# rsutormin/KmerGutsJava

Hardware: AMD Instinct MI355X
Metric: amino-acid residues/sec scanned (and hits/sec) on 1 Gbp synthetic, 1/2/4/8 MI355X (higher is better)
Workload: dtype int64; 1 GPU; 1 Gbp contig mix (0.5 kbp..1.024 Mbp, uniform ACGT) on 1 GPU, 6-frame translate + 8-mer lookup vs 1400303159-slot signature table (33.6 GB, load 0.50), -m 5 -g 200; total_bp_rank0=1000000000, contigs_rank0=6351, total_bp_all_ranks=1000000000, num_sigs=1400303159, residues_rank0=1999974596, residues_all_ranks=1999974596, hits_rank0=36744843, hits_all_ranks=36744843, calls_rank0=4, parallelism=contig shards x1, table replicated

## Files before the change

### kmergutsjava_amd/csrc/kg_device.hpp

```cpp
#pragma once

#include <hip/hip_runtime.h>
#include <stdint.h>

#include "../../include/kmerguts_hip.h"

namespace kg {

constexpr int kWave = 64;
constexpr int kWavesPerWG = 4;
constexpr int kDnaPosPerBlock = 192;
constexpr int kAaWinPerBlock = 64;
constexpr uint32_t kInvalid = 0xFFFFFFFFu;
constexpr uint32_t kTagEmpty = 0xFFu;
constexpr uint64_t kNotFound = ~0ull;
constexpr int kTagPad = 64;

struct BlockDesc {
    uint64_t soff;
    uint32_t len;
    uint32_t j;
    uint32_t nk;
    uint32_t ibase;
    uint32_t seq;
    uint32_t pad;
};
static_assert(sizeof(BlockDesc) == 32, "BlockDesc must be 32 bytes");

struct TableView {
    const uint8_t *entries;
    const uint8_t *tags;
    uint64_t limit;
    uint64_t num_sigs;
    uint64_t magic;
    uint32_t m35;
};

__device__ __forceinline__ void set_wave_prio(uint32_t p)
{
    if (p == 0) __builtin_amdgcn_s_setprio(0);
    else if (p == 1) __builtin_amdgcn_s_setprio(1);
    else if (p == 2) __builtin_amdgcn_s_setprio(2);
    else __builtin_amdgcn_s_setprio(3);
}

__device__ __forceinline__ void wave_sync()
{
    __builtin_amdgcn_fence(__ATOMIC_RELEASE, "wavefront");
    __builtin_amdgcn_wave_barrier();
    __builtin_amdgcn_fence(__ATOMIC_ACQUIRE, "wavefront");
}

__device__ __forceinline__ uint64_t split_value(uint64_t v, const TableView &t, uint64_t *q_out)
{
    uint64_t q = __umul64hi(v, t.magic);
    uint64_t r = v - q * t.num_sigs;
    if (r >= t.num_sigs) { r -= t.num_sigs; q += 1; }
    *q_out = q;
    return r;
}

__device__ __forceinline__ uint32_t split_fast(uint32_t hi, uint32_t lo, uint32_t n, uint32_t m35, uint32_t *q_out)
{
    const uint32_t vh = __umul24(hi, 20000u) + (lo >> 3);
    const uint32_t v32 = __umul24(hi, 160000u) + lo;
    uint32_t q = __umulhi(vh, m35);
    uint32_t r = v32 - q * n;
    if (r >= n) { r -= n; q += 1; }
    *q_out = q;
    return r;
}

__device__ __forceinline__ uint64_t split_halves(uint32_t hi, uint32_t lo, const TableView &t, uint64_t *q_out)
{
    if (t.m35) {
        uint32_t q;
        const uint32_t r = split_fast(hi, lo, (uint32_t)t.num_sigs, t.m35, &q);
        *q_out = q;
        return r;
    }
    return split_value((uint64_t)hi * 160000ull + lo, t, q_out);
}

__device__ __forceinline__ uint32_t mul24(uint32_t x, uint32_t c)
{
    uint32_t r;
    asm("v_mul_u32_u24 %0, %1, %2" : "=v"(r) : "s"(c), "v"(x));
    return r;
}

__device__ __forceinline__ uint32_t tag_qs(uint64_t q, uint64_t slot)
{
    const uint32_t q32 = (uint32_t)q ^ (uint32_t)(q >> 32);
    const uint32_t h = mul24((uint32_t)slot, 0x9E3779u) ^ mul24((uint32_t)(slot >> 24), 0x85EBCBu) ^
                       mul24(q32 ^ (q32 >> 19), 0xC2B2AFu);
    const uint32_t t = (h >> 16) & 0xFFu;
    return t == kTagEmpty ? 0xFEu : t;
}

__device__ __forceinline__ uint64_t home_slot(uint64_t v, const TableView &t)
{
    uint64_t q;
    return split_value(v, t, &q);
}

__device__ __forceinline__ uint32_t zero_bytes(uint32_t x)
{
    uint32_t t = (x & 0x7F7F7F7Fu) + 0x7F7F7F7Fu;
    return ~(t | x | 0x7F7F7F7Fu);
}

struct Tags16 { uint32_t w[4]; };

__device__ __forceinline__ Tags16 load_tags(const uint8_t *p)
{
    Tags16 r;
    __builtin_memcpy(&r, p, 16);
    return r;
}

__device__ __forceinline__ int first_stop(const Tags16 &x, uint32_t fp, bool *is_empty, uint32_t skip = 0)
{
    const uint32_t fpw = __builtin_amdgcn_perm(0u, fp, 0u);
    uint32_t e0 = zero_bytes(~x.w[0]), e1 = zero_bytes(~x.w[1]), e2 = zero_bytes(~x.w[2]), e3 = zero_bytes(~x.w[3]);
    uint32_t f0 = zero_bytes(x.w[0] ^ fpw), f1 = zero_bytes(x.w[1] ^ fpw), f2 = zero_bytes(x.w[2] ^ fpw), f3 = zero_bytes(x.w[3] ^ fpw);
    uint64_t elo = ((uint64_t)e1 << 32) | e0, ehi = ((uint64_t)e3 << 32) | e2;
    uint64_t slo = elo | (((uint64_t)f1 << 32) | f0), shi = ehi | (((uint64_t)f3 << 32) | f2);
    if (skip) {
        const uint64_t keep_lo = skip >= 8 ? 0ull : ~0ull << (8 * skip);
        const uint64_t keep_hi = skip <= 8 ? ~0ull : ~0ull << (8 * (skip - 8));
        slo &= keep_lo;
        shi &= keep_hi;
    }
    if (slo) {
        int b = __builtin_ctzll(slo);
        *is_empty = (elo >> b) & 1;
        return b >> 3;
    }
    if (shi) {
        int b = __builtin_ctzll(shi);
        *is_empty = (ehi >> b) & 1;
        return 8 + (b >> 3);
    }
    *is_empty = false;
    return 16;
}

__device__ __forceinline__ uint64_t probe_window(uint64_t slot, uint32_t *skip)
{
    const bool straddles = ((uint32_t)slot & 127u) > 112u;
    *skip = straddles ? ((uint32_t)slot & 15u) : 0u;
    return straddles ? (slot & ~15ull) : slot;
}

struct Entry { int64_t key; int32_t oI, avg, fI; float wt; };
struct Payload { int32_t oI, avg, fI; float wt; };

__device__ __forceinline__ Entry load_entry(const TableView &t, uint64_t slot)
{
    const uint2 *p = reinterpret_cast<const uint2 *>(t.entries + slot * 24);
    uint2 a = p[0], b = p[1], c = p[2];
    Entry e;
    e.key = (int64_t)(((uint64_t)a.y << 32) | a.x);
    e.oI = (int32_t)b.x; e.avg = (int32_t)b.y; e.fI = (int32_t)c.x; e.wt = __uint_as_float(c.y);
    return e;
}

typedef uint32_t kg_u32x4 __attribute__((ext_vector_type(4)));
typedef uint32_t kg_u32x2 __attribute__((ext_vector_type(2)));
__device__ __forceinline__ void stream_store16(void *dst, const void *src16)
{
    kg_u32x4 v;
    __builtin_memcpy(&v, src16, 16);
    __builtin_nontemporal_store(v, reinterpret_cast<kg_u32x4 *>(dst));
}
__device__ __forceinline__ void stream_store8(void *dst, uint64_t w)
{
    kg_u32x2 v; v.x = (uint32_t)w; v.y = (uint32_t)(w >> 32);
    __builtin_nontemporal_store(v, reinterpret_cast<kg_u32x2 *>(dst));
}
__device__ __forceinline__ void stream_store_hit(kg_hit *dst, const kg_hit &h)
{
    kg_u32x4 a; a.x = h.container; a.y = (uint32_t)h.from0InProt; a.z = (uint32_t)h.oI; a.w = (uint32_t)h.avgOffFromEnd;
    kg_u32x2 b; b.x = (uint32_t)h.fI; b.y = __float_as_uint(h.functionWt);
    __builtin_nontemporal_store(a, reinterpret_cast<kg_u32x4 *>(dst));
    __builtin_nontemporal_store(b, reinterpret_cast<kg_u32x2 *>(reinterpret_cast<unsigned char *>(dst) + 16));
}
__device__ __forceinline__ kg_hit stream_load_hit(const kg_hit *src)
{
    const kg_u32x4 a = __builtin_nontemporal_load(reinterpret_cast<const kg_u32x4 *>(src));
    const kg_u32x2 b = __builtin_nontemporal_load(reinterpret_cast<const kg_u32x2 *>(reinterpret_cast<const unsigned char *>(src) + 16));
    kg_hit h;
    h.container = a.x; h.from0InProt = (int32_t)a.y; h.oI = (int32_t)a.z; h.avgOffFromEnd = (int32_t)a.w;
    h.fI = (int32_t)b.x; h.functionWt = __uint_as_float(b.y);
    return h;
}

constexpr char kGeneticCode[65] = "KNKNTTTTRSRSIIMIQHQHPPPPRRRRLLLLEDEDAAAAGGGGVVVV*Y*YSSSS*CWCLFLF";
constexpr uint32_t aa_code_of(char c)
{
    const char *alpha = "ACDEFGHIKLMNPQRSTVWY";
    for (uint32_t i = 0; i < 20; i++)
        if (alpha[i] == c) return i;
    return 20;
}
__device__ __forceinline__ uint32_t aa_code_of_rt(char c)
{
    uint32_t r = 20;
#pragma unroll
    for (uint32_t i = 0; i < 20; i++)
        if ("ACDEFGHIKLMNPQRSTVWY"[i] == c) r = i;
    return r;
}
constexpr uint32_t codon16(int i)
{
    return aa_code_of(kGeneticCode[i * 4]) | (aa_code_of(kGeneticCode[i * 4 + 1]) << 5) |
           (aa_code_of(kGeneticCode[i * 4 + 2]) << 10) | (aa_code_of(kGeneticCode[i * 4 + 3]) << 15);
}
__constant__ uint32_t kCodon16[16] = {
    codon16(0), codon16(1), codon16(2), codon16(3), codon16(4), codon16(5), codon16(6), codon16(7),
    codon16(8), codon16(9), codon16(10), codon16(11), codon16(12), codon16(13), codon16(14), codon16(15)};

__device__ __forceinline__ uint32_t dna_code(uint32_t c)
{
    uint32_t u = c & 0xDFu;
    return u == 'A' ? 0u : u == 'C' ? 1u : u == 'G' ? 2u : (u == 'T' || u == 'U') ? 3u : 4u;
}

constexpr uint32_t kBadByte = 0x80u;
__device__ __forceinline__ uint32_t dot4(uint32_t bytes, uint32_t weights, uint32_t acc = 0u)
{
    return __builtin_amdgcn_udot4(bytes, weights, acc, false);
}
__device__ __forceinline__ uint2 lds_bytes8(const uint8_t *base, uint32_t at)
{
    uint2 v;
#ifdef KG_ENC_UNALIGNED
    __builtin_memcpy(&v, base + at, 8);
#else
    const uint32_t *p = reinterpret_cast<const uint32_t *>(base + (at & ~3u));
    const uint32_t w0 = p[0], w1 = p[1], w2 = p[2], sh = at & 3u;
    v.x = __builtin_amdgcn_alignbyte(w1, w0, sh);
    v.y = __builtin_amdgcn_alignbyte(w2, w1, sh);
#endif
    return v;
}
__device__ __forceinline__ uint32_t lds_bytes4(const uint8_t *base, uint32_t at)
{
#ifdef KG_ENC_UNALIGNED
    uint32_t x;
    __builtin_memcpy(&x, base + at, 4);
    return x;
#else
    const uint32_t *p = reinterpret_cast<const uint32_t *>(base + (at & ~3u));
    return __builtin_amdgcn_alignbyte(p[1], p[0], at & 3u);
#endif
}

__device__ __forceinline__ uint64_t mul24_wide(uint32_t a, uint32_t b)
{
    uint32_t lo, hi;
    asm("v_mul_u32_u24 %0, %1, %2" : "=v"(lo) : "v"(a), "v"(b));
    asm("v_mul_hi_u32_u24 %0, %1, %2" : "=v"(hi) : "v"(a), "v"(b));
    return ((uint64_t)hi << 32) | lo;
}
__device__ __forceinline__ uint32_t half_up(uint32_t w)
{
    return dot4(w, 0x01140000u, __umul24(dot4(w, 0x00000114u), 400u));
}
__device__ __forceinline__ uint32_t half_down(uint32_t w)
{
    return dot4(w, 0x00001401u, __umul24(dot4(w, 0x14010000u), 400u));
}

struct EncTablesDna {
    uint16_t codon[128];
    uint8_t base[256];
};
struct EncTablesAa {
    uint8_t code[256];
};

struct __attribute__((aligned(16))) WaveLdsDna {
    uint8_t bc[240];
    uint8_t cf[3][80];
    uint8_t cr[3][80];
};

struct __attribute__((aligned(16))) WaveLdsAa {
    uint8_t code[80];
};

template <bool AA> struct WaveLds;
template <> struct WaveLds<false> { typedef WaveLdsDna type; typedef EncTablesDna tables; };
template <> struct WaveLds<true> { typedef WaveLdsAa type; typedef EncTablesAa tables; };

template <bool AA>
__device__ __forceinline__ void encode_init(typename WaveLds<AA>::tables &t, uint32_t tid, uint32_t n_threads)
{
    if constexpr (AA) {
        for (uint32_t b = tid; b < 256; b += n_threads) {
            const uint32_t c = aa_code_of_rt((char)b);
            t.code[b] = (uint8_t)(c < 20 ? c : kBadByte);
        }
    } else {
        for (uint32_t b = tid; b < 256; b += n_threads) t.base[b] = (uint8_t)dna_code(b);
        for (uint32_t i = tid; i < 128; i += n_threads) {
            const uint32_t b0 = i / 25u, b1 = (i / 5u) % 5u, b2 = i % 5u;
            uint32_t f = kBadByte, r = kBadByte;
            if (i < 125 && b0 < 4 && b1 < 4 && b2 < 4) {
                f = (kCodon16[b0 * 4 + b1] >> (b2 * 5)) & 31u;
                r = (kCodon16[(3 - b2) * 4 + (3 - b1)] >> ((3 - b0) * 5)) & 31u;
                if (f >= 20) f = kBadByte;
                if (r >= 20) r = kBadByte;
            }
            t.codon[i] = (uint16_t)(f | (r << 8));
        }
    }
}

template <bool AA>
__device__ __forceinline__ void load_block_chars(const uint8_t *__restrict__ seq, const BlockDesc &bd, int lane, uint32_t (&raw)[4])
{
    const uint64_t soff = bd.soff;
    if constexpr (AA) {
        const uint32_t w0 = bd.j * kAaWinPerBlock;
        const uint32_t nload = min(71u, bd.len - w0);
#pragma unroll
        for (int k = 0; k < 2; k++) {
            const uint32_t q = (uint32_t)lane + 64u * k;
            raw[k] = q < nload ? seq[soff + w0 + q] : 0u;
        }
        raw[2] = raw[3] = 0;
    } else {
        const uint32_t ts = bd.j * kDnaPosPerBlock;
        const uint32_t nload = min(216u, bd.len - ts);
        const uint32_t at = 4u * (uint32_t)lane;
        uint32_t w = 0x4E4E4E4Eu;
        const uint8_t *p = seq + soff + ts + at;
        if (at + 4u <= nload) {
            __builtin_memcpy(&w, p, 4);
        } else if (at < nload) {
            for (uint32_t k = 0; at + k < nload; k++) w = (w & ~(0xFFu << (8u * k))) | ((uint32_t)p[k] << (8u * k));
        }
        raw[0] = w;
        raw[1] = raw[2] = raw[3] = 0;
    }
}

template <bool AA>
__device__ __forceinline__ void encode_chars(typename WaveLds<AA>::type &l, const typename WaveLds<AA>::tables &t,
                                             const uint32_t (&raw)[4], int lane)
{
    if constexpr (AA) {
#pragma unroll
        for (int k = 0; k < 2; k++) {
            const uint32_t q = (uint32_t)lane + 64u * k;
            const uint8_t c = t.code[raw[k] & 255u];
            if (k < 1 || q < 72) l.code[q] = c;
        }
        wave_sync();
    } else {
        {
            const uint32_t w = raw[0];
            const uint32_t c = (uint32_t)t.base[w & 255u] | ((uint32_t)t.base[(w >> 8) & 255u] << 8) |
                               ((uint32_t)t.base[(w >> 16) & 255u] << 16) | ((uint32_t)t.base[w >> 24] << 24);
            if (lane < 60) *reinterpret_cast<uint32_t *>(&l.bc[4 * lane]) = c;
        }
        wave_sync();
        {
            uint32_t idx[4];
#pragma unroll
            for (int k = 0; k < 4; k++) {
                const uint32_t q = min((uint32_t)lane + 64u * k, 212u);
                idx[k] = dot4(lds_bytes4(l.bc, q), 0x00010519u);
            }
            uint32_t cw[4];
#pragma unroll
            for (int k = 0; k < 4; k++) cw[k] = t.codon[idx[k]];
#pragma unroll
            for (int k = 0; k < 4; k++) {
                const uint32_t q = (uint32_t)lane + 64u * k;
                const uint32_t tt = (q * 171u) >> 9;
                const uint32_t f = q - 3u * tt;
                if (k < 3 || q < 213) {
                    l.cf[0][f * 80u + tt] = (uint8_t)cw[k];
                    l.cr[0][f * 80u + tt] = (uint8_t)(cw[k] >> 8);
                }
            }
        }
        wave_sync();
    }
}

template <bool AA>
__device__ __forceinline__ void encode_block(typename WaveLds<AA>::type &l, const typename WaveLds<AA>::tables &t,
                                             const uint8_t *__restrict__ seq, const BlockDesc &bd, int lane)
{
    uint32_t raw[4];
    load_block_chars<AA>(seq, bd, lane, raw);
    encode_chars<AA>(l, t, raw, lane);
}

template <bool AA>
__device__ __forceinline__ bool row_halves(const typename WaveLds<AA>::type &l, int r, int lane, const BlockDesc &bd,
                                           uint32_t *hi_out, uint32_t *lo_out)
{
    if constexpr (AA) {
        const uint2 v = lds_bytes8(l.code, (uint32_t)lane);
        const uint32_t i = bd.j * kAaWinPerBlock + lane;
        *hi_out = half_up(v.x); *lo_out = half_up(v.y);
        return (((v.x | v.y) & 0x80808080u) == 0u) & ((uint64_t)i + 8 < (uint64_t)bd.len);
    } else {
        const bool minus = r >= 3;
        const uint32_t f = (uint32_t)(minus ? r - 3 : r);
        const uint2 v = lds_bytes8(minus ? &l.cr[0][0] : &l.cf[0][0], f * 80u + (uint32_t)lane);
        if (minus) {
            *hi_out = half_down(v.y); *lo_out = half_down(v.x);
        } else {
            *hi_out = half_up(v.x); *lo_out = half_up(v.y);
        }
        return ((v.x | v.y) & 0x80808080u) == 0u;
    }
}

template <bool AA>
__device__ __forceinline__ uint32_t row_index(const BlockDesc &bd, uint32_t it, int r)
{
    if (AA) return it;
    const uint32_t vbase = 6u * bd.ibase;
    if (r < 3) return vbase + (uint32_t)r * bd.nk + bd.j;
    return vbase + (3u + (bd.len - (uint32_t)(r - 3)) % 3u) * bd.nk + (bd.nk - 1u - bd.j);
}

template <bool AA>
__device__ __forceinline__ void row_record_key(const BlockDesc &bd, int r, int lane, uint32_t *container, int32_t *pos)
{
    if (AA) {
        *container = bd.seq;
        *pos = (int32_t)(bd.j * kAaWinPerBlock + lane);
    } else if (r < 3) {
        *container = bd.seq * 6u + (uint32_t)r;
        *pos = (int32_t)(bd.j * 64u + lane);
    } else {
        const uint32_t f = (uint32_t)(r - 3);
        *container = bd.seq * 6u + 3u + (bd.len - f) % 3u;
        *pos = (int32_t)((bd.len - 24u - f - bd.j * kDnaPosPerBlock) / 3u) - (int32_t)lane;
    }
}

struct Progress {
    unsigned long long first[11];
    unsigned long long last_plus1;
    unsigned long long first_beyond;
    unsigned long long walk_ran_off;
    unsigned long long lo[11];
    unsigned long long found_upto[11];
    unsigned long long kmers_found;
    unsigned long long miss_max1[11];
};

__global__ void mark_found_kernel(const uint32_t *__restrict__ slots, uint64_t n, uint32_t *bitmap)
{
    const uint64_t stride = (uint64_t)gridDim.x * blockDim.x;
    for (uint64_t i = (uint64_t)blockIdx.x * blockDim.x + threadIdx.x; i < n; i += stride) {
        const uint32_t s = slots[i];
        atomicOr(&bitmap[s >> 5], 1u << (s & 31u));
    }
}
__global__ void count_found_kernel(const uint32_t *__restrict__ bitmap, uint64_t n_words, Progress *p)
{
    unsigned long long upto[11], all = 0;
    for (int f = 0; f <= 10; f++) upto[f] = 0;
    const uint64_t stride = (uint64_t)gridDim.x * blockDim.x;
    for (uint64_t w = (uint64_t)blockIdx.x * blockDim.x + threadIdx.x; w < n_words; w += stride) {
        const uint32_t bits = bitmap[w];
        if (!bits) continue;
        all += (unsigned long long)__popc(bits);
        const uint64_t b = w << 5;
        for (int f = 0; f <= 10; f++) {
            const unsigned long long t = p->first[f];
            if (t == ~0ull || t < b) continue;
            const uint64_t k = t - b;
            upto[f] += (unsigned long long)__popc(k >= 31 ? bits : bits & ((2u << k) - 1u));
        }
    }
    for (int f = 0; f <= 10; f++) {
        for (int off = 32; off > 0; off >>= 1) upto[f] += __shfl_down(upto[f], off);
        if ((threadIdx.x & 63) == 0 && upto[f]) atomicAdd(&p->found_upto[f], upto[f]);
    }
    for (int off = 32; off > 0; off >>= 1) all += __shfl_down(all, off);
    if ((threadIdx.x & 63) == 0 && all) atomicAdd(&p->kmers_found, all);
}

__device__ __forceinline__ void progress_note_walk(Progress *p, uint64_t home, uint64_t stop, uint64_t limit)
{
    const uint64_t last = stop < limit ? stop : limit - 1;
    if (stop >= limit) p->walk_ran_off = 1ull;
    int d = 0;
#pragma unroll
    for (int k = 1; k <= 10; k++) d += p->lo[k] <= home ? 1 : 0;
    if (home < *const_cast<volatile unsigned long long *>(&p->first[d])) atomicMin(&p->first[d], (unsigned long long)home);
    for (int k = d + 1; k <= 10 && p->lo[k] <= last; k++)
        if (p->lo[k] < *const_cast<volatile unsigned long long *>(&p->first[k])) atomicMin(&p->first[k], p->lo[k]);
    if (last + 1 > *const_cast<volatile unsigned long long *>(&p->last_plus1)) atomicMax(&p->last_plus1, (unsigned long long)(last + 1));
}
__device__ __forceinline__ void progress_note_beyond(Progress *p, uint64_t home)
{
    if (home < *const_cast<volatile unsigned long long *>(&p->first_beyond)) atomicMin(&p->first_beyond, (unsigned long long)home);
}
__device__ __forceinline__ void progress_note_homes(Progress *p, uint32_t d, uint32_t mn, uint32_t mx1)
{
#pragma unroll
    for (int off = 32; off > 0; off >>= 1) {
        mn = min(mn, (uint32_t)__shfl_xor((int)mn, off));
        mx1 = max(mx1, (uint32_t)__shfl_xor((int)mx1, off));
    }
    if ((threadIdx.x & 63) == 0) {
        if (mn != ~0u && mn < *const_cast<volatile unsigned long long *>(&p->first[d])) atomicMin(&p->first[d], (unsigned long long)mn);
        if (mx1 > *const_cast<volatile unsigned long long *>(&p->miss_max1[d])) atomicMax(&p->miss_max1[d], (unsigned long long)mx1);
    }
}

__device__ __forceinline__ void progress_note_home(Progress *p, uint32_t d_lo, uint32_t d_hi, uint32_t h, uint32_t listed)
{
    uint32_t d = d_lo;
    while (d < d_hi && p->lo[d + 1] <= h) d++;
    if (h < *const_cast<volatile unsigned long long *>(&p->first[d])) atomicMin(&p->first[d], (unsigned long long)h);
    if (!listed && h + 1u > *const_cast<volatile unsigned long long *>(&p->miss_max1[d])) atomicMax(&p->miss_max1[d], (unsigned long long)h + 1u);
}

__device__ uint64_t first_empty_block(const uint8_t *__restrict__ tags, uint64_t h, uint64_t bound)
{
    __shared__ unsigned long long s_end;
    for (uint64_t base = h; base < bound; base += 4096) {
        if (threadIdx.x == 0) s_end = ~0ull;
        __syncthreads();
        unsigned long long mine = ~0ull;
#pragma unroll
        for (int j = 0; j < 16; j++) {
            const uint64_t s = base + (uint64_t)j * 256u + threadIdx.x;
            if (s < bound && (uint32_t)tags[s] == kTagEmpty && s < mine) mine = s;
        }
        if (mine != ~0ull) atomicMin(&s_end, mine);
        __syncthreads();
        const unsigned long long e = s_end;
        __syncthreads();
        if (e != ~0ull) return e;
    }
    return bound;
}

__global__ __launch_bounds__(256) void progress_finish_kernel(Progress *p, const uint8_t *__restrict__ tags, uint64_t limit)
{
    unsigned long long m1 = 0;
    for (int k = 1; k <= 10; k++) {
        m1 = max(m1, p->miss_max1[k - 1]);
        const unsigned long long lo = p->lo[k];
        if (m1 == 0 || lo >= limit || p->first[k] <= lo) continue;
        if (first_empty_block(tags, m1 - 1, lo) == lo && threadIdx.x == 0) p->first[k] = lo;
    }
    m1 = max(m1, p->miss_max1[10]);
    if (m1 == 0) return;
    const uint64_t e = first_empty_block(tags, m1 - 1, limit);
    if (threadIdx.x == 0) {
        const uint64_t last = e < limit ? e : limit - 1;
        if (last + 1 > p->last_plus1) p->last_plus1 = last + 1;
        if (e >= limit) p->walk_ran_off = 1ull;
    }
}

template <int N, bool COUNTERS>
__device__ __forceinline__ uint32_t probe_n(const TableView &tab, const uint64_t (&val)[N], const uint64_t (&home_in)[N],
                                            const uint32_t (&fp)[N], bool (&valid)[N], Payload (&ent)[N],
                                            unsigned long long &ctr_valid, unsigned long long &ctr_slots, bool &ran_off,
                                            Progress *prog = nullptr ,
                                            uint32_t *found_slot = nullptr )
{
    uint64_t cand[N];
    uint32_t skip[N];
    Tags16 tg[N];
    uint64_t home[COUNTERS ? N : 1];
#pragma unroll
    for (int q = 0; q < N; q++) {
        cand[q] = home_in[q];
        if (COUNTERS) { home[q] = cand[q]; if (valid[q]) ctr_valid++; }
        if (valid[q] && cand[q] >= tab.limit) { ran_off = true; if (COUNTERS && prog) progress_note_beyond(prog, cand[q]); }
        valid[q] = valid[q] && cand[q] < tab.limit;
        cand[q] = probe_window(cand[q], &skip[q]);
        if (valid[q]) tg[q] = load_tags(tab.tags + cand[q]);
    }
    uint32_t st1 = 0, pend = 0;
    uint64_t stop[COUNTERS ? N : 1];
#pragma unroll
    for (int q = 0; q < N; q++) {
        if (COUNTERS) stop[q] = cand[q];
        if (valid[q]) {
            bool emp;
            int i = first_stop(tg[q], fp[q], &emp, skip[q]);
            if (i == 16) { pend |= 1u << q; cand[q] += 16; }
            else {
                cand[q] += (uint64_t)i;
                if (COUNTERS) stop[q] = cand[q];
                if (!emp) st1 |= 1u << q;
                else if (cand[q] >= tab.limit) ran_off = true;
            }
        }
    }
    uint32_t foundm = 0;
    {
        Entry full[N];
#pragma unroll
        for (int q = 0; q < N; q++)
            if (st1 & (1u << q)) full[q] = load_entry(tab, cand[q]);
#pragma unroll
        for (int q = 0; q < N; q++) {
            if (st1 & (1u << q)) {
                if (full[q].key == (int64_t)val[q]) foundm |= 1u << q;
                else { pend |= 1u << q; cand[q] += 1; }
            }
            ent[q].oI = full[q].oI; ent[q].avg = full[q].avg; ent[q].fI = full[q].fI; ent[q].wt = full[q].wt;
        }
    }
    while (__ballot(pend != 0)) {
        if (pend) {
            const int r = __builtin_ctz(pend);
            uint64_t v = val[0], s = cand[0];
            uint32_t f = fp[0];
#pragma unroll
            for (int q = 1; q < N; q++)
                if (r == q) { v = val[q]; s = cand[q]; f = fp[q]; }
            bool done = false, hit = false;
            Entry e;
            e.key = 0; e.oI = e.avg = e.fI = 0; e.wt = 0.f;
            if (s >= tab.limit) { done = true; s = tab.limit; ran_off = true; }
            else {
                Tags16 x = load_tags(tab.tags + s);
                bool emp;
                int i = first_stop(x, f, &emp);
                if (i == 16) s += 16;
                else if (emp) { done = true; s += (uint64_t)i; if (s >= tab.limit) ran_off = true; }
                else {
                    s += (uint64_t)i;
                    e = load_entry(tab, s);
                    if (e.key == (int64_t)v) done = hit = true;
                    else s += 1;
                }
            }
#pragma unroll
            for (int q = 0; q < N; q++) {
                if (r == q) {
                    cand[q] = s;
                    if (done) {
                        if (COUNTERS) stop[q] = s;
                        if (hit) { ent[q].oI = e.oI; ent[q].avg = e.avg; ent[q].fI = e.fI; ent[q].wt = e.wt; foundm |= 1u << q; }
                    }
                }
            }
            if (done) pend &= pend - 1;
        }
    }
    if (COUNTERS) {
#pragma unroll
        for (int q = 0; q < N; q++) {
            if (valid[q]) {
                uint64_t last = stop[q] < tab.limit ? stop[q] + 1 : tab.limit;
                ctr_slots += last - home[q];
                if (prog) progress_note_walk(prog, home[q], stop[q], tab.limit);
                if (found_slot) found_slot[q] = (uint32_t)stop[q];
            }
        }
    }
    return foundm;
}

__device__ __forceinline__ void flush_ran_off(bool ran_off, unsigned long long *ctr, int lane)
{
    if (__ballot(ran_off) && lane == 0) atomicOr(&ctr[3], 1ull);
}

__device__ __forceinline__ void flush_counters(unsigned long long ctr_valid, unsigned long long ctr_slots,
                                               unsigned long long *ctr, int lane)
{
    for (int off = 32; off > 0; off >>= 1) {
        ctr_valid += __shfl_down(ctr_valid, off);
        ctr_slots += __shfl_down(ctr_slots, off);
    }
    if (lane == 0) {
        atomicAdd(&ctr[0], ctr_valid);
        atomicAdd(&ctr[1], ctr_slots);
    }
}

template <bool AA, bool COUNTERS, int RPG>
__global__ __launch_bounds__(kWave *kWavesPerWG) void scan_kernel(
    const uint8_t *__restrict__ entries, const uint8_t *__restrict__ tags, uint64_t limit, uint64_t num_sigs, uint64_t magic,
    uint32_t m35, const uint8_t *__restrict__ seq, const BlockDesc *__restrict__ blocks, uint32_t n_blocks,
    uint32_t *__restrict__ counts,
    uint32_t *__restrict__ block_stage_base, kg_hit *__restrict__ stage, unsigned long long *cursor, uint64_t stage_cap,
    uint32_t stage_chunk, unsigned long long *ctr,
    Progress *prog , uint32_t *__restrict__ stage_slot ,
    const uint32_t *__restrict__ hbits , uint64_t tail_start)
{
    constexpr int ROWS = AA ? 1 : 6;
    constexpr int NG = ROWS / RPG;
    static_assert(ROWS % RPG == 0, "RPG must divide the row count");
    __shared__ typename WaveLds<AA>::type lds[kWavesPerWG];
    __shared__ typename WaveLds<AA>::tables enc_tables;
    const int lane = threadIdx.x & 63;
    const int wave = threadIdx.x >> 6;
    const uint32_t wave_global = __builtin_amdgcn_readfirstlane(blockIdx.x * kWavesPerWG + wave);
    const uint32_t n_waves = gridDim.x * kWavesPerWG;
    TableView tab;
    tab.entries = entries; tab.tags = tags; tab.limit = limit; tab.num_sigs = num_sigs; tab.magic = magic; tab.m35 = m35;

    typename WaveLds<AA>::type &l = lds[wave];
    encode_init<AA>(enc_tables, threadIdx.x, blockDim.x);
    __syncthreads();

    unsigned long long ctr_valid = 0, ctr_slots = 0;
    bool ran_off = false;
    unsigned long long res_at = 0, res_end = 0;

    for (uint32_t it_v = wave_global; it_v < n_blocks; it_v += n_waves) {
        const uint32_t it = __builtin_amdgcn_readfirstlane(it_v);
        const BlockDesc bd = blocks[it];
        encode_block<AA>(l, enc_tables, seq, bd, lane);

        for (int g = 0; g < NG; g++) {
            uint64_t val[RPG], home[RPG];
            uint32_t fp[RPG];
            bool valid[RPG];
#pragma unroll
            for (int q = 0; q < RPG; q++) {
                uint32_t hi, lo;
                uint64_t quo;
                valid[q] = row_halves<AA>(l, g * RPG + q, lane, bd, &hi, &lo);
                home[q] = split_halves(hi, lo, tab, &quo);
                fp[q] = tag_qs(quo, home[q]);
                val[q] = (uint64_t)hi * 160000ull + lo;
            }

            if (!COUNTERS && hbits) {
                uint32_t w[RPG];
#pragma unroll
                for (int q = 0; q < RPG; q++) w[q] = valid[q] && home[q] < limit ? hbits[home[q] >> 5] : ~0u;
#pragma unroll
                for (int q = 0; q < RPG; q++)
                    if (valid[q] && home[q] < limit && !((w[q] >> ((uint32_t)home[q] & 31u)) & 1u)) {
                        valid[q] = false;
                        if (home[q] >= tail_start) ran_off = true;
                    }
            }
            Payload ent[RPG];
            uint32_t fslot[RPG];
#pragma unroll
            for (int q = 0; q < RPG; q++) fslot[q] = 0;
            const uint32_t foundm = probe_n<RPG, COUNTERS>(tab, val, home, fp, valid, ent, ctr_valid, ctr_slots, ran_off,
                                                           COUNTERS ? prog : nullptr, COUNTERS && stage_slot ? fslot : nullptr);

            uint32_t cnt[RPG], rank[RPG];
            uint32_t total = 0;
#pragma unroll
            for (int q = 0; q < RPG; q++) {
                const int r = g * RPG + q;
                unsigned long long m = __ballot((foundm >> q) & 1u);
                cnt[q] = (uint32_t)__popcll(m);
                unsigned long long below = m & ((1ull << lane) - 1ull);
                unsigned long long above = lane == 63 ? 0ull : (m >> (lane + 1));
                rank[q] = (!AA && r >= 3) ? (uint32_t)__popcll(above) : (uint32_t)__popcll(below);
                total += cnt[q];
                if (lane == 0) counts[row_index<AA>(bd, it, r)] = cnt[q];
            }
            if (total > res_end - res_at) {
                unsigned long long chunk = total > stage_chunk ? total : stage_chunk;
                unsigned long long b = 0;
                if (lane == 0) b = atomicAdd(cursor, chunk);
                b = ((unsigned long long)__builtin_amdgcn_readfirstlane((uint32_t)(b >> 32)) << 32) |
                    (unsigned long long)__builtin_amdgcn_readfirstlane((uint32_t)b);
                res_at = b; res_end = b + chunk;
            }
            const unsigned long long base = res_at;
            res_at += total;
            if (lane == 0) block_stage_base[(uint64_t)it * NG + g] = (uint32_t)base;
            if (total && base + total <= stage_cap) {
                uint32_t rowbase = 0;
#pragma unroll
                for (int q = 0; q < RPG; q++) {
                    if ((foundm >> q) & 1u) {
                        kg_hit h;
                        row_record_key<AA>(bd, g * RPG + q, lane, &h.container, &h.from0InProt);
                        h.oI = ent[q].oI; h.avgOffFromEnd = ent[q].avg; h.fI = ent[q].fI; h.functionWt = ent[q].wt;
                        stage[base + rowbase + rank[q]] = h;
                        if (COUNTERS && stage_slot) stage_slot[base + rowbase + rank[q]] = fslot[q];
                    }
                    rowbase += cnt[q];
                }
            }
        }
        wave_sync();
    }

    if (COUNTERS) flush_counters(ctr_valid, ctr_slots, ctr, lane);
    flush_ran_off(ran_off, ctr, lane);
}

__global__ void build_blocks_kernel(const int64_t *seq_off, const uint32_t *ibase, uint32_t n_seqs,
                                    uint32_t n_blocks, BlockDesc *out)
{
    uint32_t i = blockIdx.x * blockDim.x + threadIdx.x;
    if (i >= n_blocks) return;
    uint32_t lo = 0, hi = n_seqs;
    while (hi - lo > 1) {
        uint32_t mid = lo + (hi - lo) / 2;
        if (ibase[mid] <= i) lo = mid; else hi = mid;
    }
    BlockDesc d;
    d.soff = (uint64_t)seq_off[lo];
    d.len = (uint32_t)(seq_off[lo + 1] - seq_off[lo]);
    d.j = i - ibase[lo];
    d.nk = ibase[lo + 1] - ibase[lo];
    d.ibase = ibase[lo];
    d.seq = lo;
    d.pad = 0;
    out[i] = d;
}

constexpr int kScanThreads = 256;
constexpr int kScanPerThread = 8;
constexpr int kScanChunk = kScanThreads * kScanPerThread;

__device__ __forceinline__ uint32_t wg_exclusive_scan(uint32_t x, uint32_t *total, uint32_t *lds )
{
    const int lane = threadIdx.x & 63, wave = threadIdx.x >> 6;
    uint32_t incl = x;
    for (int off = 1; off < 64; off <<= 1) {
        uint32_t y = __shfl_up(incl, off);
        if (lane >= off) incl += y;
    }
    if (lane == 63) lds[wave] = incl;
    __syncthreads();
    uint32_t wbase = 0, all = 0;
    for (int w = 0; w < kScanThreads / 64; w++) {
        uint32_t s = lds[w];
        if (w < wave) wbase += s;
        all += s;
    }
    __syncthreads();
    *total = all;
    return wbase + incl - x;
}

__global__ __launch_bounds__(kScanThreads) void scan_partials_kernel(const uint32_t *in, uint64_t n, uint64_t *partial)
{
    __shared__ uint64_t wsum[kScanThreads / 64];
    uint64_t base = (uint64_t)blockIdx.x * kScanChunk + (uint64_t)threadIdx.x * kScanPerThread;
    uint64_t s = 0;
    for (int k = 0; k < kScanPerThread; k++)
        if (base + k < n) s += in[base + k];
    for (int d = 32; d > 0; d >>= 1) s += __shfl_xor(s, d);
    if ((threadIdx.x & 63) == 0) wsum[threadIdx.x >> 6] = s;
    __syncthreads();
    if (threadIdx.x == 0) {
        uint64_t all = 0;
        for (int w = 0; w < kScanThreads / 64; w++) all += wsum[w];
        partial[blockIdx.x] = all;
    }
}

__global__ __launch_bounds__(kScanThreads) void scan_top_kernel(uint64_t *partial, uint32_t n_partials, uint64_t *total_out)
{
    __shared__ uint64_t carry;
    __shared__ uint64_t wsum[kScanThreads / 64];
    if (threadIdx.x == 0) carry = 0;
    __syncthreads();
    const int lane = threadIdx.x & 63, wave = threadIdx.x >> 6;
    for (uint32_t b = 0; b < n_partials; b += kScanThreads) {
        uint32_t i = b + threadIdx.x;
        uint64_t x = i < n_partials ? partial[i] : 0;
        uint64_t incl = x;
        for (int off = 1; off < 64; off <<= 1) {
            uint64_t y = __shfl_up(incl, off);
            if (lane >= off) incl += y;
        }
        if (lane == 63) wsum[wave] = incl;
        __syncthreads();
        uint64_t wbase = 0, all = 0;
        for (int w = 0; w < kScanThreads / 64; w++) {
            uint64_t s = wsum[w];
            if (w < wave) wbase += s;
            all += s;
        }
        uint64_t c = carry;
        if (i < n_partials) partial[i] = c + wbase + incl - x;
        __syncthreads();
        if (threadIdx.x == 0) carry = c + all;
        __syncthreads();
    }
    if (threadIdx.x == 0) *total_out = carry;
}

__global__ __launch_bounds__(kScanThreads) void scan_final_kernel(const uint32_t *in, uint64_t n, const uint64_t *partial,
                                                                  uint32_t *out)
{
    __shared__ uint32_t lds[8];
    uint64_t base = (uint64_t)blockIdx.x * kScanChunk + (uint64_t)threadIdx.x * kScanPerThread;
    uint32_t v[kScanPerThread];
    uint32_t s = 0;
    for (int k = 0; k < kScanPerThread; k++) {
        v[k] = base + k < n ? in[base + k] : 0;
        s += v[k];
    }
    uint32_t total;
    uint32_t excl = wg_exclusive_scan(s, &total, lds);
    uint32_t run = (uint32_t)partial[blockIdx.x] + excl;
    for (int k = 0; k < kScanPerThread; k++) {
        if (base + k < n) out[base + k] = run;
        run += v[k];
    }
}

template <bool AA>
__global__ __launch_bounds__(kWave *kWavesPerWG) void place_kernel(const BlockDesc *__restrict__ blocks, uint32_t n_blocks,
                                                                  const uint32_t *__restrict__ counts,
                                                                  const uint32_t *__restrict__ offs,
                                                                  const uint32_t *__restrict__ block_stage_base, uint32_t rpg,
                                                                  const kg_hit *__restrict__ stage, kg_hit *__restrict__ hits,
                                                                  const uint32_t *__restrict__ stage_slot, uint32_t *__restrict__ hit_slots)
{
    constexpr int ROWS = AA ? 1 : 6;
    const int lane = threadIdx.x & 63;
    const uint32_t it = __builtin_amdgcn_readfirstlane(blockIdx.x * kWavesPerWG + (threadIdx.x >> 6));
    if (it >= n_blocks) return;
    const BlockDesc bd = blocks[it];
    const uint32_t ng = (uint32_t)ROWS / rpg;
    uint32_t src = 0;
#pragma unroll
    for (int r = 0; r < ROWS; r++) {
        if ((uint32_t)r % rpg == 0) src = block_stage_base[(uint64_t)it * ng + (uint32_t)r / rpg];
        const uint32_t vrow = row_index<AA>(bd, it, r);
        uint32_t n = counts[vrow];
        if ((uint32_t)lane < n) {
            hits[(uint64_t)offs[vrow] + lane] = stage[(uint64_t)src + lane];
            if (hit_slots) hit_slots[(uint64_t)offs[vrow] + lane] = stage_slot[(uint64_t)src + lane];
        }
        src += n;
    }
}

template <bool AA>
__global__ void container_starts_kernel(const uint32_t *ibase, uint32_t n_seqs, const uint32_t *offs, uint64_t n_rows,
                                        const uint64_t *total, int64_t *chs)
{
    constexpr uint32_t PER = AA ? 1 : 6;
    uint64_t c = (uint64_t)blockIdx.x * blockDim.x + threadIdx.x;
    uint64_t n_cont = (uint64_t)n_seqs * PER;
    if (c > n_cont) return;
    if (c == n_cont) { chs[c] = (int64_t)*total; return; }
    uint32_t k = (uint32_t)(c / PER), cc = (uint32_t)(c % PER);
    uint32_t nk = ibase[k + 1] - ibase[k];
    uint64_t row = (uint64_t)PER * ibase[k] + (uint64_t)cc * nk;
    chs[c] = row < n_rows ? (int64_t)offs[row] : (int64_t)*total;
}

struct ClearList { uint32_t *p[8]; uint64_t words[8]; int n; };

__global__ __launch_bounds__(256) void clear_many_kernel(ClearList l)
{
    const uint64_t tid = (uint64_t)blockIdx.x * blockDim.x + threadIdx.x, stride = (uint64_t)gridDim.x * blockDim.x;
    for (int k = 0; k < l.n; k++) {
        uint32_t *p = l.p[k];
        const uint64_t w = l.words[k];
        const uint64_t head = min(w, (uint64_t)((16u - ((uintptr_t)p & 15u)) & 15u) / 4u);
        const uint64_t quads = (w - head) / 4;
        uint4 *q = reinterpret_cast<uint4 *>(p + head);
        for (uint64_t i = tid; i < quads; i += stride) q[i] = make_uint4(0, 0, 0, 0);
        for (uint64_t i = tid; i < head; i += stride) p[i] = 0;
        for (uint64_t i = head + quads * 4 + tid; i < w; i += stride) p[i] = 0;
    }
}

__global__ void build_tags_kernel(const uint8_t *entries, uint64_t limit, uint64_t n_tags, uint64_t num_sigs, uint64_t magic,
                                  uint8_t *tags, unsigned long long *occupied)
{
    TableView tab;
    tab.entries = entries; tab.tags = tags; tab.limit = limit; tab.num_sigs = num_sigs; tab.magic = magic; tab.m35 = 0;
    uint64_t i = (uint64_t)blockIdx.x * blockDim.x + threadIdx.x;
    uint64_t stride = (uint64_t)gridDim.x * blockDim.x;
    unsigned long long occ = 0, tail = 0;
    for (; i < n_tags; i += stride) {
        uint32_t t = kTagEmpty;
        if (i < limit) {
            const uint2 *p = reinterpret_cast<const uint2 *>(entries + i * 24);
            uint2 a = p[0];
            int64_t key = (int64_t)(((uint64_t)a.y << 32) | a.x);
            if (key <= KG_MAX_ENCODED) {
                uint64_t q;
                const uint64_t slot = split_value((uint64_t)key, tab, &q);
                t = tag_qs(q, slot);
                occ++;
            }
        }
        tags[i] = (uint8_t)t;
        if (t == kTagEmpty && i < limit) tail = i + 1;
    }
    for (int off = 32; off > 0; off >>= 1) {
        occ += __shfl_down(occ, off);
        const unsigned long long o = __shfl_down(tail, off);
        tail = o > tail ? o : tail;
    }
    if ((threadIdx.x & 63) == 0) {
        if (occ) atomicAdd(occupied, occ);
        if (tail) atomicMax(occupied + 1, tail);
    }
}

constexpr uint32_t kHomeWalkMax = 1024;
constexpr uint32_t kBidxClasses = 19, kBidxPair0 = 20, kBidxHash0 = 191, kBidxMore = 255;
constexpr uint32_t kBidxInexact = 0x80000000u;

__host__ __device__ constexpr uint32_t bidx_pair_code(uint32_t c1, uint32_t c2)
{
    return kBidxPair0 + c1 * 19u - c1 * (c1 + 1u) / 2u + (c2 - c1 - 1u);
}
static_assert(bidx_pair_code(0, 1) == 20 && bidx_pair_code(0, 18) == 37 && bidx_pair_code(1, 2) == 38 && bidx_pair_code(17, 18) == 190,
              "pair codes must fill 20..190");

__device__ __forceinline__ uint32_t bidx_decode(uint32_t code)
{
    if (code == 0) return 0u;
    if (code < kBidxPair0) return 1u << (code - 1u);
    if (code < kBidxHash0) {
        uint32_t c1 = 0;
        while (code >= bidx_pair_code(c1, c1 + 1u) + (18u - c1)) c1++;
        const uint32_t c2 = c1 + 1u + (code - bidx_pair_code(c1, c1 + 1u));
        return (1u << c1) | (1u << c2);
    }
    if (code == kBidxMore) return 0x7FFFFu | kBidxInexact;
    const uint32_t m6 = code - kBidxHash0;
    uint32_t m = 0;
    for (uint32_t c = 0; c < kBidxClasses; c++) m |= ((m6 >> (c % 6u)) & 1u) << c;
    return m | kBidxInexact;
}

__device__ __forceinline__ uint32_t bidx_encode(uint32_t class_mask, bool complete)
{
    if (!complete) return kBidxMore;
    const uint32_t n = (uint32_t)__popc(class_mask);
    if (n == 0) return 0u;
    const uint32_t c1 = (uint32_t)__builtin_ctz(class_mask);
    if (n == 1) return 1u + c1;
    if (n == 2) return bidx_pair_code(c1, 31u - (uint32_t)__builtin_clz(class_mask));
    const uint32_t m6 = (class_mask | (class_mask >> 6) | (class_mask >> 12) | (class_mask >> 18)) & 63u;
    return kBidxHash0 + m6;
}

__global__ void build_bidx_kernel(const uint8_t *entries, const uint8_t *tags, uint64_t limit, uint64_t n_idx, uint64_t num_sigs,
                                  uint64_t magic, uint8_t *idx)
{
    TableView tab;
    tab.entries = entries; tab.tags = tags; tab.limit = limit; tab.num_sigs = num_sigs; tab.magic = magic; tab.m35 = 0;
    const uint64_t stride = (uint64_t)gridDim.x * blockDim.x;
    for (uint64_t h = (uint64_t)blockIdx.x * blockDim.x + threadIdx.x; h < n_idx; h += stride) {
        uint32_t mask = 0;
        bool complete = true;
        if (h < limit && tags[h] != kTagEmpty) {
            uint64_t j = h;
            for (; j < limit && j - h < kHomeWalkMax; j++) {
                if (tags[j] == kTagEmpty) break;
                const uint2 a = *reinterpret_cast<const uint2 *>(entries + j * 24);
                const int64_t key = (int64_t)(((uint64_t)a.y << 32) | a.x);
                if (key < 0) continue;
                uint64_t q;
                if (split_value((uint64_t)key, tab, &q) != h) continue;
                mask |= 1u << (uint32_t)(q % kBidxClasses);
            }
            if (j < limit && j - h >= kHomeWalkMax) complete = false;
        }
        idx[h] = (uint8_t)bidx_encode(mask, complete);
    }
}

__global__ void build_hbits_kernel(const uint8_t *__restrict__ idx, uint64_t n_idx, uint32_t *__restrict__ bits, uint64_t n_words)
{
    const uint64_t stride = (uint64_t)gridDim.x * blockDim.x;
    for (uint64_t w = (uint64_t)blockIdx.x * blockDim.x + threadIdx.x; w < n_words; w += stride) {
        uint32_t out = 0;
        const uint64_t s0 = w * 32;
        if (s0 + 32 <= n_idx) {
            const uint4 a = *reinterpret_cast<const uint4 *>(idx + s0), b = *reinterpret_cast<const uint4 *>(idx + s0 + 16);
            const uint32_t v[8] = {a.x, a.y, a.z, a.w, b.x, b.y, b.z, b.w};
#pragma unroll
            for (int k = 0; k < 8; k++)
#pragma unroll
                for (int j = 0; j < 4; j++) out |= (((v[k] >> (8 * j)) & 0xFFu) != 0u ? 1u : 0u) << (4 * k + j);
        } else {
            for (uint32_t j = 0; j < 32 && s0 + j < n_idx; j++) out |= (idx[s0 + j] != 0 ? 1u : 0u) << j;
        }
        bits[w] = out;
    }
}

}
```

### kmergutsjava_amd/csrc/kg_host_plan.hpp

```cpp
#pragma once

namespace {


template <typename T, T V, T... Vs, typename F>
void dispatch(T x, F &&f)
{
    if constexpr (sizeof...(Vs) == 0) f(std::integral_constant<T, V>{});
    else if (x == V) f(std::integral_constant<T, V>{});
    else dispatch<T, Vs...>(x, f);
}

struct BatchPlan {
    std::vector<uint32_t> ibase;
    uint64_t nblocks = 0, windows = 0, residues = 0;
    uint64_t n_rows = 0, n_cont = 0;
    int64_t longest = 0;
};

template <bool AA>
int plan_batch(const int64_t *offsets, int64_t n_seqs, BatchPlan &b)
{
    constexpr uint32_t PER = AA ? 1 : 6;
    b.ibase.resize((size_t)n_seqs + 1);
    for (int64_t k = 0; k < n_seqs; k++) {
        int64_t L = offsets[k + 1] - offsets[k];
        if (L < 0) return fail(KG_ERR_ARG, "offsets must be non-decreasing");
        b.longest = std::max(b.longest, L);
        if (L > 0xFFFFFFF0ll) return fail(KG_ERR_LIMIT, "a single sequence longer than 2^32-16 characters");
        b.ibase[(size_t)k] = (uint32_t)b.nblocks;
        uint64_t nb;
        if (AA) {
            uint64_t nwin = L >= 9 ? (uint64_t)L - 8 : 0;
            b.windows += nwin;
            b.residues += (uint64_t)L;
            nb = (nwin + kg::kAaWinPerBlock - 1) / kg::kAaWinPerBlock;
        } else {
            uint64_t npos = L >= 24 ? (uint64_t)L - 23 : 0;
            b.windows += 2 * npos;
            for (int f = 0; f < 3; f++)
                if (L - f >= 3) b.residues += 2 * (uint64_t)((L - f) / 3);
            nb = (npos + kg::kDnaPosPerBlock - 1) / kg::kDnaPosPerBlock;
        }
        b.nblocks += nb;
        if (b.nblocks > 0x7FFFFFFFull / PER) return fail(KG_ERR_LIMIT, "batch too large: more than 2^31-1 window rows; split the batch");
    }
    b.ibase[(size_t)n_seqs] = (uint32_t)b.nblocks;
    if (b.windows > 0xFFFFFF00ull) return fail(KG_ERR_LIMIT, "batch too large: more than 2^32-256 windows; split the batch");
    b.n_rows = b.nblocks * PER;
    b.n_cont = (uint64_t)n_seqs * PER;
    return KG_OK;
}

uint64_t bucket_count(uint64_t limit, uint32_t shift) { return (limit + (1ull << shift) - 1) >> shift; }

struct PartPlan {
    bool applicable = false;
    uint32_t shift = 0, buckets = 0;
    uint32_t n_chunks = 0;
    std::vector<uint64_t> clo;
    std::vector<int64_t> cseq;
    uint64_t max_chunk = 0;
    uint32_t n_wg = 0, cap = 0;
    uint64_t n_regions = 0;
    uint32_t ovf_cap = 0;
    uint32_t gshift = 10, groups_stride = 0;
    size_t next_stride = 0;
    size_t scatter_lds = 0;
    bool use_bidx = false, part_counters = false, prog_index = false;
    uint32_t probe_grid = 0, index_grid = 0, verify_grid = 0, lowc_grid = 0, ovf_grid = 0, order_grid = 0;
    uint32_t scatter_prio = 0, index_prio = 0, verify_prio = 0, index_r = 1, probe_grab = 0;
    uint32_t flush_list = 0;
    uint64_t list_slack = 0, ucap = 0, ccap = 0;
    uint32_t n_os = 0;
    bool early_totals = false, place_staged = false, debug = false;
};

template <bool AA>
int plan_partition(const kg_table *t, const BatchPlan &b, bool progress, bool counters_req, PartPlan &pl)
{
    constexpr uint32_t PER = AA ? 1 : 6;
    const uint64_t nblocks = b.nblocks;
    uint32_t shift = env_knob("KG_PART_SHIFT", 21u, 4u, 31u);
    const uint64_t qmax = (uint64_t)KG_MAX_ENCODED / (uint64_t)t->num_sigs + 1;
    while (shift > 4 && qmax >= (1ull << (32 - shift))) shift--;
    while (bucket_count(t->limit, shift) > (uint64_t)kg::kMaxBuckets) shift++;
    while (kg::scatter_lds_bytes<AA>((uint32_t)bucket_count(t->limit, shift)) > 160u * 1024) shift++;
    const bool fits = shift < 32 && qmax < (1ull << (32 - shift)) && nblocks <= (1ull << 23) && t->m35 != 0 &&
                      t->limit < (1ull << 32) - 64;
    const uint32_t mode = env_u32("KG_PARTITION", 2u);
    const bool worth = t->limit >= (64ull << 20) && b.windows >= (1ull << 27);
    if (!(fits && nblocks > 0 && (mode == 1 || (mode == 2 && worth)))) return KG_OK;
    pl.shift = shift;
    pl.buckets = (uint32_t)bucket_count(t->limit, shift);

    constexpr uint32_t WIN = AA ? 64u : 384u;
    uint32_t want = env_u32("KG_PART_CHUNKS", 4u);
    if (want < 1) want = 1;
    if (want > kMaxChunks) want = kMaxChunks;
    if (getenv("KG_PART_MIN_CHUNK_BLOCKS")) {
        const uint64_t min_chunk = std::max(1u, env_u32("KG_PART_MIN_CHUNK_BLOCKS", 600000u));
        while (want > 1 && nblocks / want < min_chunk) want--;
    } else {
        const uint32_t by_size = nblocks < 450000 ? 1u : std::max(2u, (uint32_t)std::lround(std::sqrt((double)nblocks / 325000.0)));
        want = std::min(want, std::max(1u, by_size));
    }
    pl.clo.push_back(0); pl.cseq.push_back(0);
    std::vector<double> cum;
    if (const char *tp = getenv("KG_PART_TAPER")) {
        double acc = 0;
        for (const char *q = tp; *q;) {
            char *endp = nullptr;
            const double v = strtod(q, &endp);
            if (endp == q) break;
            acc += v; cum.push_back(acc);
            q = *endp == ',' ? endp + 1 : endp;
        }
        if (cum.size() >= 2 && cum.size() <= kMaxChunks && acc > 0) { for (auto &x : cum) x /= acc; want = (uint32_t)cum.size(); }
        else cum.clear();
    }
    for (uint32_t c = 1; c < want; c++) {
        const uint64_t target = cum.empty() ? nblocks * c / want : (uint64_t)((double)nblocks * cum[c - 1]);
        const auto it = std::lower_bound(b.ibase.begin(), b.ibase.end(), (uint32_t)target);
        const uint64_t cut = *it;
        if (cut > pl.clo.back() && cut < nblocks) { pl.clo.push_back(cut); pl.cseq.push_back((int64_t)(it - b.ibase.begin())); }
    }
    pl.clo.push_back(nblocks); pl.cseq.push_back((int64_t)b.ibase.size() - 1);
    pl.n_chunks = (uint32_t)pl.clo.size() - 1;
    for (uint32_t c = 0; c < pl.n_chunks; c++) pl.max_chunk = std::max(pl.max_chunk, pl.clo[c + 1] - pl.clo[c]);
    const uint64_t max_chunk = pl.max_chunk;
    const uint64_t chunk_blocks = (max_chunk + kg::kScatterWaves - 1) / kg::kScatterWaves * kg::kScatterWaves;
    const double max_frac = (double)max_chunk / (double)nblocks;
    uint32_t n_wg = env_knob("KG_PART_WGS", 256u, 1u, kMaxGrid);
    if ((uint64_t)n_wg * kg::kScatterWaves > chunk_blocks) n_wg = (uint32_t)((chunk_blocks + kg::kScatterWaves - 1) / kg::kScatterWaves);
    const uint64_t blocks_per_wg = ((chunk_blocks + (uint64_t)n_wg * kg::kScatterWaves - 1) / ((uint64_t)n_wg * kg::kScatterWaves)) * kg::kScatterWaves;
    const double mean = (double)blocks_per_wg * WIN / (double)pl.buckets * (env_u32("KG_PART_SLACK", 100u) / 100.0);
    const uint64_t cap64 = ((uint64_t)(mean + 6.0 * std::sqrt(mean) + 32.0) + 15) / 16 * 16;
    if (cap64 >= (1ull << 24) || (uint64_t)pl.buckets * n_wg >= (1ull << 24)) return KG_OK;
    pl.n_wg = n_wg;
    pl.cap = (uint32_t)cap64;
    pl.n_regions = (uint64_t)pl.buckets * n_wg;
    pl.ovf_cap = env_u32("KG_PART_OVF_GROUPS", (uint32_t)std::min<uint64_t>(1u << 23, std::max<uint64_t>(65536, pl.n_regions * pl.cap / 16 / 8)));
    while (pl.gshift < 12 && ((max_chunk * PER) >> pl.gshift) + 2 > 8192) pl.gshift++;
    pl.groups_stride = (uint32_t)(((max_chunk * PER) >> pl.gshift) + 2);
    if (pl.groups_stride > kg::kMaxGroups) return fail(KG_ERR_LIMIT, "a chunk of the batch holds more than 2^26 window rows");
    pl.next_stride = std::max<size_t>((size_t)pl.buckets + 8, 256);
    pl.use_bidx = t->d_bidx != nullptr && !counters_req && env_u32("KG_BIDX", 1u) != 0;
    pl.part_counters = (counters_req || progress) && !pl.use_bidx;
    pl.prog_index = progress && pl.use_bidx;
    pl.scatter_lds = kg::scatter_lds_bytes<AA>(pl.buckets);
    pl.flush_list = env_knob("KG_SCATTER_FLUSH_LIST", kg::scatter_flush_list_max<AA>(), 1u, kg::scatter_flush_list_max<AA>());
    pl.probe_grid = env_knob("KG_PROBE_GRID", 256u * 8u, 8u, kMaxGrid, 8u);
    pl.index_grid = env_knob("KG_INDEX_GRID", 256u * 4u, 8u, kMaxGrid, 8u);
    pl.scatter_prio = std::min(3u, env_u32("KG_SCATTER_PRIO", 1u));
    pl.index_prio = std::min(3u, env_u32("KG_INDEX_PRIO", 2u));
    pl.verify_prio = std::min(3u, env_u32("KG_VERIFY_PRIO", pl.n_chunks == 1 ? 2u : 0u));
    uint32_t index_r = env_u32("KG_INDEX_R", 0u);
    if (index_r == 0) index_r = mean * 0.7 >= 640.0 ? 1u : mean * 0.7 >= 320.0 ? 2u : 4u;
    if (index_r != 1 && index_r != 2) index_r = 4;
    while (index_r > 1 && (n_wg % index_r != 0 || kg::kIndexN % index_r != 0)) index_r /= 2;
    pl.index_r = index_r;
    pl.verify_grid = env_knob("KG_VERIFY_GRID", 256u * 2u, 1u, kMaxGrid);
    pl.lowc_grid = env_knob("KG_LOWC_GRID", 256u, 1u, kMaxGrid);
    pl.ovf_grid = env_knob("KG_OVF_GRID", 256u, 1u, kMaxGrid);
    pl.list_slack = (uint64_t)(std::max(std::max(pl.probe_grid, pl.index_grid), pl.verify_grid) + 64) * 4 * kg::kUChunk + 4096;
    pl.ucap = ((uint64_t)((double)b.windows * t->stage_ratio * max_frac) + pl.list_slack + kg::kUChunk - 1) / kg::kUChunk * kg::kUChunk;
    pl.ccap = ((uint64_t)((double)b.windows * (t->stage_ratio * 1.25 + 0.03) * max_frac) + pl.list_slack + kg::kUChunk - 1) /
              kg::kUChunk * kg::kUChunk;
    if (test_hook("KG_TEST_TINY_LISTS")) pl.ucap = pl.ccap = kg::kUChunk;
    const uint32_t grab_unit = 256u * (uint32_t)std::max(kg::kProbeN, kg::kIndexN);
    pl.probe_grab = env_knob("KG_PROBE_GRAB", pl.cap, grab_unit, 1u << 24, grab_unit);
    pl.n_os = pl.n_chunks < 2 ? 0u : std::min(env_u32("KG_ORDER_STREAMS", 0u), kMaxOrderStreams);
    pl.early_totals = pl.n_os == 0 && env_u32("KG_EARLY_TOTALS", 1u) != 0;
    pl.order_grid = env_knob("KG_ORDER_GRID", 256u * 3u, 1u, kMaxGrid);
    pl.place_staged = pl.gshift == 10 && env_u32("KG_PLACE_STAGED", 1u) != 0;
    pl.debug = getenv("KG_DEBUG") != nullptr;
    pl.applicable = true;
    return KG_OK;
}

struct DirectPlan {
    uint32_t scan_grid, stage_chunk;
    const uint32_t *d_hbits;
    uint32_t rpg;
    uint64_t stage_cap;
};

template <bool AA>
DirectPlan plan_direct(const kg_table *t, const BatchPlan &b, bool counters)
{
    DirectPlan pl;
    pl.scan_grid = env_knob("KG_SCAN_GRID", 256u * 8u, 1u, kMaxGrid);
    pl.stage_chunk = env_knob("KG_STAGE_CHUNK", 256u, 1u, 1u << 12);
    const uint32_t filter_mode = env_u32("KG_DIRECT_FILTER", 1u);
    pl.d_hbits = (counters || filter_mode == 0 || (filter_mode == 1 && t->limit <= (4ull << 20))) ? nullptr : t->d_hbits;
    pl.rpg = AA ? 1u : env_u32("KG_SCAN_RPG", pl.d_hbits ? 6u : 3u);
    if (pl.rpg != 1 && pl.rpg != 2 && pl.rpg != 3 && pl.rpg != 6) pl.rpg = 3;
    pl.stage_cap = (uint64_t)((double)b.windows * t->stage_ratio) + 4096 + (uint64_t)pl.scan_grid * kg::kWavesPerWG * pl.stage_chunk;
    if (pl.stage_cap > 0xFFFFFF00ull) pl.stage_cap = 0xFFFFFF00ull;
    if (test_hook("KG_TEST_TINY_LISTS")) pl.stage_cap = 256;
    return pl;
}

struct AggPlan {
    uint32_t pshift;
    bool pieces_on;
    uint32_t agg_pairs;
};

AggPlan plan_aggregate()
{
    AggPlan pl;
    pl.pshift = std::min(20u, std::max(6u, env_u32("KG_AGG_BLOCK_SHIFT", 9u)));
    pl.pieces_on = env_u32("KG_AGG_PIECES", 1u) != 0;
    pl.agg_pairs = env_u32("KG_AGG_PAIRS", 1u);
    return pl;
}

}
```

### kmergutsjava_amd/csrc/kg_host_scan.hpp

```cpp
#pragma once

namespace {

struct ScanCtx {
    kg_table *t;
    kg_result *res;
    Scratch &sc;
    const BatchPlan &b;
    const uint8_t *d_seq, *h_seq;
    const int64_t *offsets;
    int64_t n_seqs;
    bool progress, counters;
    bool seq_uploaded;
    uint64_t n_hits = 0;
    int64_t *d_off = nullptr;
    uint32_t *d_ibase = nullptr;
    kg::BlockDesc *d_blocks = nullptr;
    uint32_t *d_counts = nullptr, *d_offs = nullptr, *d_bsb = nullptr;
    uint64_t *d_partial = nullptr, *d_totals = nullptr;
    kg::Progress *d_prog = nullptr;
};

int upload_seq(const ScanCtx &cx, int64_t a, int64_t b)
{
    if (cx.h_seq && b > a)
        HIP_TRY(hipMemcpyAsync(const_cast<uint8_t *>(cx.d_seq) + a, cx.h_seq + a, (size_t)(b - a), hipMemcpyHostToDevice, cx.t->stream));
    return KG_OK;
}

template <int N>
struct BlockGuard {
    Scratch &sc;
    void **slot[N];
    void release() { for (void **q : slot) { dfree(sc.t, *q); *q = nullptr; } }
    ~BlockGuard() { for (void **q : slot) if (*q) { sc.adopt(*q); *q = nullptr; } }
};

void drop_hits(kg_table *t, kg_result *res)
{
    dfree(t, res->d_hits); dfree(t, res->d_hit_slots);
    res->d_hits = nullptr; res->d_hit_slots = nullptr;
}

int send_counters(kg_table *t, const uint64_t *d_pc, const uint32_t *d_ovfc, const uint64_t *d_totals, hipStream_t s)
{
    if (d_pc) {
        HIP_TRY(hipMemcpyAsync(t->h_pin + kPinPc, d_pc, kPcWords * 8, hipMemcpyDeviceToHost, s));
        HIP_TRY(hipMemcpyAsync(t->h_pin + kPinOvf, d_ovfc, kOvfWords * kMaxChunks * 4, hipMemcpyDeviceToHost, s));
    }
    HIP_TRY(hipMemcpyAsync(t->h_pin + kPinTotals, d_totals, kTotSent * 8, hipMemcpyDeviceToHost, s));
    return KG_OK;
}

void note_totals(ScanCtx &cx, uint64_t n_hits, bool counted)
{
    kg_table *t = cx.t;
    kg_stats &st = cx.res->st;
    const uint64_t *h_tot = t->h_pin + kPinTotals;
    st.windows_valid = counted ? (int64_t)h_tot[kTotValid] : -1;
    st.slots_inspected = counted ? (int64_t)h_tot[kTotSlots] : -1;
    st.lookup_ran_off = h_tot[kTotRanOff] ? 1 : 0;
    if (cx.b.windows) {
        double ratio = (double)n_hits / (double)cx.b.windows * 1.1 + 1e-3;
        if (ratio > t->stage_ratio) t->stage_ratio = ratio > 1.0 ? 1.0 : ratio;
    }
    cx.n_hits = n_hits;
    st.n_hits = (int64_t)n_hits;
}

int progress_begin(ScanCtx &cx)
{
    kg_table *t = cx.t;
    int rc;
    if (t->limit > 0xFFFFFFFFull) return fail(KG_ERR_UNSUPPORTED, "KG_F_PROGRESS: table streams of 2^32 records or more");
    if ((rc = cx.sc.get(&cx.d_prog, 1))) return rc;
    kg::Progress h;
    for (auto &x : h.first) x = ~0ull;
    h.last_plus1 = 0; h.first_beyond = ~0ull; h.walk_ran_off = 0;
    for (auto &x : h.found_upto) x = 0;
    h.kmers_found = 0;
    for (auto &x : h.miss_max1) x = 0;
    const double n = (double)t->num_sigs;
    auto tenth = [&](uint64_t s) { return (int)(10.0 * ((double)(s + 1) / n)); };
    for (int f = 0; f <= 10; f++) {
        const unsigned __int128 num = (unsigned __int128)(uint64_t)t->num_sigs * (unsigned)f;
        uint64_t s = (uint64_t)((num + 9) / 10);
        s = s > 3 ? s - 3 : 0;
        while (tenth(s) < f) s++;
        h.lo[f] = s;
    }
    HIP_TRY(hipMemcpyAsync(cx.d_prog, &h, sizeof h, hipMemcpyHostToDevice, t->stream));
    HIP_TRY(hipStreamSynchronize(t->stream));
    return KG_OK;
}

int progress_finish(ScanCtx &cx, bool index_walks)
{
    kg_table *t = cx.t;
    int rc;
    if (index_walks)
        hipLaunchKernelGGL(kg::progress_finish_kernel, dim3(1), dim3(256), 0, t->stream, cx.d_prog, t->d_tags, t->limit);
    uint32_t *d_bitmap = nullptr;
    const uint64_t n_words = (t->limit + 31) / 32 + 1;
    if ((rc = cx.sc.get(&d_bitmap, (size_t)n_words))) return rc;
    HIP_TRY(hipMemsetAsync(d_bitmap, 0, n_words * 4, t->stream));
    if (cx.n_hits)
        hipLaunchKernelGGL(kg::mark_found_kernel, dim3((uint32_t)std::min<uint64_t>(2048, (cx.n_hits + 255) / 256)), dim3(256), 0, t->stream,
                           cx.res->d_hit_slots, cx.n_hits, d_bitmap);
    hipLaunchKernelGGL(kg::count_found_kernel, dim3((uint32_t)std::min<uint64_t>(2048, (n_words + 255) / 256)), dim3(256), 0, t->stream,
                       d_bitmap, n_words, cx.d_prog);
    return KG_OK;
}

int progress_fetch(ScanCtx &cx)
{
    kg::Progress h;
    HIP_TRY(hipMemcpy(&h, cx.d_prog, sizeof h, hipMemcpyDeviceToHost));
    kg_progress &g = cx.res->progress;
    for (int f = 0; f <= 10; f++) g.first_visited[f] = h.first[f] == ~0ull ? -1 : (int64_t)h.first[f];
    g.last_visited = (int64_t)h.last_plus1 - 1;
    g.first_beyond = h.first_beyond == ~0ull ? -1 : (int64_t)h.first_beyond;
    g.walk_ran_off = h.walk_ran_off ? 1 : 0;
    g.stream_slots = (int64_t)cx.t->limit;
    for (int f = 0; f <= 10; f++) g.found_upto[f] = g.first_visited[f] < 0 ? 0 : (int64_t)h.found_upto[f];
    g.kmers_found = (int64_t)h.kmers_found;
    cx.res->has_progress = true;
    return KG_OK;
}

struct PartBuffers {
    uint64_t *d_ent = nullptr, *d_ovf_ent = nullptr;
    uint32_t *d_fill = nullptr, *d_ovf_bucket = nullptr, *d_next = nullptr;
    uint32_t *d_ovfc = nullptr;
    uint32_t *d_lowc = nullptr;
    kg::RowGeo *d_geo = nullptr;
    uint64_t *d_pc = nullptr;
    uint32_t *d_ghist = nullptr, *d_gbase = nullptr, *d_gcur1 = nullptr, *d_gcur2 = nullptr, *d_gtile = nullptr;
    uint64_t ucap = 0, ccap = 0;
    size_t cused_stride = 0, candused_stride = 0;
    kg_hit *d_ulist = nullptr, *d_sortA = nullptr, *d_sortB = nullptr;
    uint32_t *d_cused = nullptr, *d_candused = nullptr;
    kg::CandRec *d_cand = nullptr;
};

struct ChunkView {
    uint32_t c, lo, nb;
    uint64_t *ent, *ovf_ent;
    uint32_t *fill, *next, *ovfc, *ovf_bucket;
    kg_hit *ulist, *sortA, *sortB;
    uint32_t *cused, *candused;
    kg::CandRec *cand;
    unsigned long long *ucur, *ccur;
    uint64_t *base, *ctot;
    uint32_t *ghist, *gbase, *gcur1, *gcur2, *gtile;
};

ChunkView chunk_view(const PartPlan &pl, const PartBuffers &pb, uint32_t c)
{
    ChunkView v;
    v.c = c; v.lo = (uint32_t)pl.clo[c]; v.nb = (uint32_t)(pl.clo[c + 1] - pl.clo[c]);
    v.ent = pb.d_ent + (uint64_t)c * pl.n_regions * pl.cap;
    v.fill = pb.d_fill + (uint64_t)c * pl.n_regions;
    v.next = pb.d_next + (size_t)c * pl.next_stride;
    v.ovfc = pb.d_ovfc + kOvfWords * c; v.ovf_bucket = pb.d_ovf_bucket + (size_t)c * pl.ovf_cap;
    v.ovf_ent = pb.d_ovf_ent + (size_t)c * pl.ovf_cap * kg::kGroup;
    v.ulist = pb.d_ulist + (uint64_t)c * pb.ucap;
    v.cused = pb.d_cused + c * pb.cused_stride; v.candused = pb.d_candused + c * pb.candused_stride;
    v.cand = pb.d_cand + (uint64_t)c * pb.ccap;
    v.ucur = (unsigned long long *)(pb.d_pc + kPcUcur + c); v.ccur = (unsigned long long *)(pb.d_pc + kPcCcur + c);
    v.base = pb.d_pc + kPcBase + c; v.ctot = pb.d_pc + kPcCtot + c;
    v.ghist = pb.d_ghist + (size_t)c * pl.groups_stride; v.gbase = pb.d_gbase + (size_t)c * (pl.groups_stride + 1);
    v.gcur1 = pb.d_gcur1 + (size_t)c * (kg::kHDigits + 1); v.gcur2 = pb.d_gcur2 + (size_t)c * pl.groups_stride;
    v.gtile = pb.d_gtile + (size_t)c * (kg::kHDigits + 1);
    v.sortA = pb.d_sortA + (uint64_t)c * pb.ucap; v.sortB = pb.d_sortB + (uint64_t)c * pb.ucap;
    return v;
}

int scatter_variant_of(const ScanCtx &cx)
{
    return cx.t->limit >= (uint64_t)cx.t->num_sigs ? 0 : cx.d_prog ? 2 : 1;
}
template <typename F>
void scatter_variant(int variant, F &&f)
{
    if (variant == 0) f(std::false_type{}, std::false_type{});
    else if (variant == 1) f(std::true_type{}, std::false_type{});
    else f(std::true_type{}, std::true_type{});
}

int upload_scatter_cold(const ScanCtx &cx, const PartPlan &pl, const PartBuffers &pb)
{
    kg_table *t = cx.t;
    kg::ScatterCold h[kMaxChunks] = {};
    for (uint32_t c = 0; c < pl.n_chunks; c++) {
        uint32_t *ovfc = pb.d_ovfc + kOvfWords * c;
        h[c].ovf_cursor = ovfc; h[c].ovf_bucket = pb.d_ovf_bucket + (size_t)c * pl.ovf_cap;
        h[c].ovf_ent = pb.d_ovf_ent + (size_t)c * pl.ovf_cap * kg::kGroup;
        h[c].lowc_cursor = ovfc + kOvfLowc; h[c].lowc_blocks = pb.d_lowc + pl.clo[c];
        h[c].ctr = (unsigned long long *)(cx.d_totals + kTotValid); h[c].prog = cx.d_prog;
        h[c].ovf_cap = pl.ovf_cap;
    }
    if (!t->d_cold) HIP_TRY(hipMalloc((void **)&t->d_cold, sizeof h));
    else if (!memcmp(h, t->h_cold, sizeof h)) return KG_OK;
    memcpy(t->h_cold, h, sizeof h);
    HIP_TRY(hipMemcpyAsync(t->d_cold, t->h_cold, sizeof h, hipMemcpyHostToDevice, t->stream));
    return KG_OK;
}

template <bool AA>
int chunk_passes(const ScanCtx &cx, const PartPlan &pl, const PartBuffers &pb, const ChunkView &v)
{
    kg_table *t = cx.t;
    kg::Progress *d_prog = cx.d_prog;
    unsigned long long *d_ctr = (unsigned long long *)(cx.d_totals + kTotValid);
    const hipStream_t s2 = t->stream2, s3 = t->stream3;
    uint32_t *lowc_cursor = v.ovfc + kOvfLowc, *lowc = pb.d_lowc + v.lo;
    const uint32_t limit32 = (uint32_t)std::min<uint64_t>(t->limit, 0xFFFFFFFFull);
    scatter_variant(scatter_variant_of(cx), [&](auto is_short, auto prog) {
        constexpr bool SHORT = decltype(is_short)::value, PROG = decltype(prog)::value;
        hipLaunchKernelGGL((kg::part_scatter_kernel<AA, SHORT, PROG>), dim3(pl.n_wg), dim3(kg::kWave * kg::kScatterWaves), pl.scatter_lds,
                           t->stream, cx.d_seq, cx.d_blocks, v.lo, v.nb, limit32, (uint32_t)t->num_sigs, t->m35, pl.shift, pl.buckets, pl.cap,
                           v.ent, v.fill, t->d_cold + v.c, pl.scatter_prio, pl.flush_list);
    });
    HIP_TRY(hipEventRecord(t->pev[kPevChunk + 2 * v.c], t->stream));
    HIP_TRY(hipStreamWaitEvent(s2, t->pev[kPevChunk + 2 * v.c], 0));
    hipLaunchKernelGGL((kg::lowc_blocks_kernel<AA>), dim3(pl.lowc_grid), dim3(64 * kg::kLowcWaves), 0, s2, cx.d_seq, cx.d_blocks, lowc_cursor, lowc,
                       t->limit, (uint32_t)t->num_sigs, t->m35, pl.shift, pl.n_wg, pl.cap, v.ent, v.fill, v.ovfc, pl.ovf_cap,
                       v.ovf_bucket, v.ovf_ent, d_ctr, d_prog);
    if (pl.use_bidx) {
        const uint32_t tail_start = (uint32_t)std::min<uint64_t>(t->tail_start, 0xFFFFFFFFull);
        dispatch<int, 1, 2, 4>((int)pl.index_r, [&](auto r) {
            dispatch<bool, true, false>(t->bidx_exact, [&](auto exact) {
                dispatch<bool, true, false>(pl.prog_index, [&](auto prog) {
                    constexpr int R = decltype(r)::value;
                    constexpr bool EXACT = decltype(exact)::value, PROG = decltype(prog)::value;
                    hipLaunchKernelGGL((kg::bucket_index_kernel<kg::kIndexN, R, EXACT, PROG>), dim3(pl.index_grid), dim3(256), 0, s2,
                                       t->d_bidx, tail_start, v.ent, v.fill, pl.n_wg, pl.cap, pl.buckets, pl.shift, pl.probe_grab, v.next,
                                       v.cand, v.candused, v.ccur, pb.ccap, d_ctr, pl.index_prio, PROG ? d_prog : (kg::Progress *)nullptr);
                });
            });
        });
    } else {
        dispatch<bool, true, false>(pl.part_counters, [&](auto counters) {
            constexpr bool COUNTERS = decltype(counters)::value;
            hipLaunchKernelGGL((kg::bucket_tag_kernel<COUNTERS>), dim3(pl.probe_grid), dim3(256), 0, s2, t->d_tags, t->limit,
                               (uint64_t)t->num_sigs, v.ent, v.fill, pl.n_wg, pl.cap, pl.buckets, pl.shift, pl.probe_grab, v.next, v.cand,
                               v.candused, v.ccur, pb.ccap, d_ctr, COUNTERS ? d_prog : (kg::Progress *)nullptr);
        });
    }
    HIP_TRY(hipEventRecord(t->pev[kPevChunk + 2 * v.c + 1], s2));
    HIP_TRY(hipStreamWaitEvent(s3, t->pev[kPevChunk + 2 * v.c + 1], 0));
    dispatch<int, 1, 2, 0>(pl.part_counters ? 1 : pl.prog_index ? 2 : 0, [&](auto walks) {
        constexpr bool COUNTERS = decltype(walks)::value == 1, PROG = decltype(walks)::value == 2;
        hipLaunchKernelGGL((kg::verify_kernel<AA, COUNTERS, PROG>), dim3(pl.verify_grid), dim3(256), 0, s3, t->d_entries, t->d_tags, t->limit,
                           (uint64_t)t->num_sigs, t->magic, v.cand, v.candused, v.ccur, pb.ccap, v.ulist, v.cused, v.ucur, pb.ucap, d_ctr,
                           d_prog, pl.verify_prio);
        hipLaunchKernelGGL((kg::overflow_probe_kernel<AA, COUNTERS, PROG>), dim3(pl.ovf_grid), dim3(256), 0, s3, t->d_entries, t->d_tags,
                           t->limit, (uint64_t)t->num_sigs, t->magic, v.ovf_bucket, v.ovf_ent, v.ovfc, pl.ovf_cap, pl.shift, v.ulist,
                           v.cused, v.ucur, pb.ucap, d_ctr, d_prog);
    });
    HIP_TRY(hipEventRecord(t->pev[kPevVerified + v.c], s3));
    HIP_TRY(hipGetLastError());
    return KG_OK;
}

template <bool AA>
int chunk_order(const ScanCtx &cx, const PartPlan &pl, const PartBuffers &pb, const ChunkView &v, uint64_t hits_cap)
{
    constexpr uint32_t PER = AA ? 1 : 6;
    kg_table *t = cx.t;
    kg_result *res = cx.res;
    const uint32_t c = v.c, gshift = pl.gshift;
    const bool last = c + 1 == pl.n_chunks;
    hipStream_t s = t->stream;
    if (pl.n_os) {
        s = t->ostream[c % pl.n_os];
        HIP_TRY(hipStreamWaitEvent(s, t->ev[kEvScattered], 0));
    }
    HIP_TRY(hipStreamWaitEvent(s, t->pev[kPevVerified + c], 0));
    const uint64_t row_lo = (uint64_t)v.lo * PER, row_hi = row_lo + (uint64_t)v.nb * PER;
    const uint32_t g0 = (uint32_t)(row_lo >> gshift);
    const uint32_t n_groups = v.nb ? (uint32_t)(((row_hi - 1) >> gshift) - g0 + 1) : 1u;
    hipLaunchKernelGGL(kg::hit_hist_kernel, dim3(pl.order_grid), dim3(kg::kHThreads), (size_t)n_groups * 4, s, v.ulist, v.cused, v.ucur, pb.ucap,
                       g0, 6u + gshift, n_groups, v.ghist);
    hipLaunchKernelGGL(kg::group_scan_kernel, dim3(1), dim3(kg::kGsThreads), 0, s, v.ghist, n_groups, v.gbase, v.gcur1, v.gcur2, v.ctot, v.gtile);
    if (pl.n_os && c) HIP_TRY(hipStreamWaitEvent(s, t->pev[kPevBase + c - 1], 0));
    hipLaunchKernelGGL(kg::chunk_base_kernel, dim3(1), dim3(1), 0, s, v.ctot, v.base, last ? cx.d_totals : (uint64_t *)nullptr);
    if (pl.n_os) HIP_TRY(hipEventRecord(t->pev[kPevBase + c], s));
    if (pl.early_totals && last) {
        int rc;
        if ((rc = send_counters(t, pb.d_pc, pb.d_ovfc, cx.d_totals, s))) return rc;
        HIP_TRY(hipEventRecord(t->pev[kPevTotals], s));
    }
    hipLaunchKernelGGL((kg::hit_partition_kernel<true>), dim3(pl.order_grid), dim3(kg::kHThreads), 0, s, v.ulist, v.cused, v.ucur, pb.ucap,
                       v.gbase, n_groups, g0, 6u + gshift, v.gcur1, v.sortA, pb.ucap, v.gtile);
    hipLaunchKernelGGL((kg::hit_partition_kernel<false>), dim3(pl.order_grid), dim3(kg::kHThreads), 0, s, v.sortA, v.cused, v.ucur, pb.ucap,
                       v.gbase, n_groups, g0, 6u + gshift, v.gcur2, v.sortB, pb.ucap, v.gtile);
    hipLaunchKernelGGL((kg::group_place_kernel<AA>), dim3(std::min(n_groups, 256u * 8u)), dim3(kg::kHThreads),
                       kg::group_place_lds(gshift, pl.place_staged), s,
                       v.sortB, v.gbase, n_groups, g0, gshift, (uint32_t)row_lo, (uint32_t)row_hi, pb.d_geo, (uint64_t)cx.b.n_rows,
                       pl.place_staged ? 1u : 0u, v.base, res->d_hits, hits_cap, cx.d_offs, res->d_hit_slots);
    HIP_TRY(hipGetLastError());
    return KG_OK;
}

template <bool AA>
int part_allocate(ScanCtx &cx, const PartPlan &pl, PartBuffers &pb)
{
    kg_table *t = cx.t;
    Scratch &sc = cx.sc;
    const uint32_t n_chunks = pl.n_chunks, groups_stride = pl.groups_stride;
    int rc;
    if ((rc = sc.get(&pb.d_ent, (size_t)(pl.n_regions * pl.cap * n_chunks)))) return rc;
    if ((rc = sc.get(&pb.d_fill, (size_t)pl.n_regions * n_chunks))) return rc;
    if ((rc = sc.get(&pb.d_ovf_ent, (size_t)pl.ovf_cap * kg::kGroup * n_chunks))) return rc;
    if ((rc = sc.get(&pb.d_ovf_bucket, (size_t)pl.ovf_cap * n_chunks))) return rc;
    if ((rc = sc.get(&pb.d_next, pl.next_stride * n_chunks))) return rc;
    if ((rc = sc.get(&pb.d_ovfc, kOvfWords * kMaxChunks))) return rc;
    if ((rc = sc.get(&pb.d_lowc, (size_t)cx.b.nblocks + 1))) return rc;
    if ((rc = sc.get(&pb.d_geo, (size_t)cx.b.n_rows))) return rc;
    if ((rc = sc.get(&pb.d_ghist, (size_t)groups_stride * n_chunks))) return rc;
    if ((rc = sc.get(&pb.d_gbase, (size_t)(groups_stride + 1) * n_chunks))) return rc;
    if ((rc = sc.get(&pb.d_gcur1, (size_t)(kg::kHDigits + 1) * n_chunks))) return rc;
    if ((rc = sc.get(&pb.d_gcur2, (size_t)groups_stride * n_chunks))) return rc;
    if ((rc = sc.get(&pb.d_gtile, (size_t)(kg::kHDigits + 1) * n_chunks))) return rc;
    if (kg::group_place_lds(pl.gshift, pl.gshift == 10) > t->place_lds[AA ? 1 : 0]) {
        const size_t want_lds = kg::group_place_lds(pl.gshift, pl.gshift == 10);
        HIP_TRY(hipFuncSetAttribute((const void *)kg::group_place_kernel<AA>, hipFuncAttributeMaxDynamicSharedMemorySize, (int)want_lds));
        t->place_lds[AA ? 1 : 0] = want_lds;
    }
    if (groups_stride * 4u > t->hist_lds) {
        HIP_TRY(hipFuncSetAttribute((const void *)kg::hit_hist_kernel, hipFuncAttributeMaxDynamicSharedMemorySize, (int)(groups_stride * 4u)));
        t->hist_lds = groups_stride * 4u;
    }
    if ((rc = sc.get(&pb.d_pc, kPcWords))) return rc;
    const int sv = scatter_variant_of(cx);
    if (t->scatter_lds[AA ? 1 : 0][sv] < pl.scatter_lds) {
        hipError_t e = hipSuccess;
        scatter_variant(sv, [&](auto is_short, auto prog) {
            e = hipFuncSetAttribute((const void *)kg::part_scatter_kernel<AA, decltype(is_short)::value, decltype(prog)::value>,
                                    hipFuncAttributeMaxDynamicSharedMemorySize, (int)pl.scatter_lds);
        });
        HIP_TRY(e);
        t->scatter_lds[AA ? 1 : 0][sv] = pl.scatter_lds;
    }
    return KG_OK;
}

template <bool AA>
int scan_partitioned(ScanCtx &cx, const PartPlan &pl, bool &done)
{
    constexpr uint32_t PER = AA ? 1 : 6;
    kg_table *t = cx.t;
    kg_result *res = cx.res;
    kg_stats &st = res->st;
    const uint32_t n_chunks = pl.n_chunks;
    const uint64_t nblocks = cx.b.nblocks;
    int rc;
    PartBuffers pb;
    if ((rc = part_allocate<AA>(cx, pl, pb))) return rc;
    BlockGuard<6> lists{cx.sc, {(void **)&pb.d_ulist, (void **)&pb.d_cused, (void **)&pb.d_cand, (void **)&pb.d_candused,
                                (void **)&pb.d_sortA, (void **)&pb.d_sortB}};
    pb.ucap = pl.ucap; pb.ccap = pl.ccap;
    HIP_TRY(hipEventRecord(t->ev[kEvScanBegin], t->stream));
    for (int attempt = 0; attempt < 3; attempt++) {
        const uint64_t ucap = pb.ucap, ccap = pb.ccap;
        const uint64_t hits_cap = ucap * n_chunks;
        pb.cused_stride = (size_t)(ucap / kg::kUChunk + 1); pb.candused_stride = (size_t)(ccap / kg::kUChunk + 1);
        if ((rc = dalloc(t, (void **)&res->d_hits, hits_cap * sizeof(kg_hit)))) return rc;
        if (cx.progress && (rc = dalloc(t, (void **)&res->d_hit_slots, hits_cap * 4))) return rc;
        if ((rc = dalloc(t, (void **)&pb.d_ulist, ucap * n_chunks * sizeof(kg_hit)))) return rc;
        if ((rc = dalloc(t, (void **)&pb.d_cused, pb.cused_stride * n_chunks * 4))) return rc;
        if ((rc = dalloc(t, (void **)&pb.d_cand, ccap * n_chunks * sizeof(kg::CandRec)))) return rc;
        if ((rc = dalloc(t, (void **)&pb.d_candused, pb.candused_stride * n_chunks * 4))) return rc;
        if ((rc = dalloc(t, (void **)&pb.d_sortA, ucap * n_chunks * sizeof(kg_hit)))) return rc;
        if ((rc = dalloc(t, (void **)&pb.d_sortB, ucap * n_chunks * sizeof(kg_hit)))) return rc;
        if ((rc = clear_words(t->stream, [](uint64_t most) { return (uint32_t)std::min<uint64_t>(4096, (most / 4 + 255) / 256 + 1); },
                              {{pb.d_cused, (uint64_t)pb.cused_stride * n_chunks},
                               {pb.d_candused, (uint64_t)pb.candused_stride * n_chunks},
                               {pb.d_pc, kPcWords * 2},
                               {cx.d_totals, kTotWords * 2},
                               {pb.d_ovfc, kOvfWords * kMaxChunks},
                               {pb.d_next, (uint64_t)pl.next_stride * n_chunks},
                               {pb.d_ghist, (uint64_t)pl.groups_stride * n_chunks}})))
            return rc;
        if ((rc = upload_scatter_cold(cx, pl, pb))) return rc;
        HIP_TRY(hipEventRecord(t->pev[kPevFork], t->stream));
        HIP_TRY(hipStreamWaitEvent(t->stream2, t->pev[kPevFork], 0));
        HIP_TRY(hipStreamWaitEvent(t->stream3, t->pev[kPevFork], 0));
        hipLaunchKernelGGL((kg::row_geo_kernel<AA>), dim3((uint32_t)((nblocks * PER + 255) / 256)), dim3(256), 0, t->stream3, cx.d_blocks,
                           (uint32_t)nblocks, pb.d_geo);
        for (uint32_t c = 0; c < n_chunks; c++) {
            if (!cx.seq_uploaded && (rc = upload_seq(cx, cx.offsets[pl.cseq[c]], cx.offsets[pl.cseq[c + 1]]))) return rc;
            if ((rc = chunk_passes<AA>(cx, pl, pb, chunk_view(pl, pb, c)))) return rc;
        }
        HIP_TRY(hipEventRecord(t->ev[kEvScattered], t->stream));
        cx.seq_uploaded = true;
        for (uint32_t k = 0; k < pl.n_os; k++)
            if (!t->ostream[k]) {
                int pr_least = 0, pr_greatest = 0;
                HIP_TRY(hipDeviceGetStreamPriorityRange(&pr_least, &pr_greatest));
                HIP_TRY(hipStreamCreateWithPriority(&t->ostream[k], hipStreamNonBlocking, pr_least));
            }
        for (uint32_t c = 0; c < n_chunks; c++)
            if ((rc = chunk_order<AA>(cx, pl, pb, chunk_view(pl, pb, c), hits_cap))) return rc;

        for (uint32_t k = 0; k < pl.n_os; k++) {
            HIP_TRY(hipEventRecord(t->pev[kPevOrdered + k], t->ostream[k]));
            HIP_TRY(hipStreamWaitEvent(t->stream, t->pev[kPevOrdered + k], 0));
        }
        HIP_TRY(hipEventRecord(t->pev[kPevJoin2], t->stream2));
        HIP_TRY(hipStreamWaitEvent(t->stream, t->pev[kPevJoin2], 0));
        HIP_TRY(hipEventRecord(t->pev[kPevJoin3], t->stream3));
        HIP_TRY(hipStreamWaitEvent(t->stream, t->pev[kPevJoin3], 0));
        HIP_TRY(hipEventRecord(t->ev[kEvJoined], t->stream));
        st.scan_launches++;
        HIP_TRY(hipEventRecord(t->ev[kEvScanEnd], t->stream));
        if (pl.early_totals) {
            HIP_TRY(hipEventSynchronize(t->pev[kPevTotals]));
        } else {
            if ((rc = send_counters(t, pb.d_pc, pb.d_ovfc, cx.d_totals, t->stream))) return rc;
            HIP_TRY(hipStreamSynchronize(t->stream));
        }
        const uint64_t *h_pc = t->h_pin + kPinPc;
        const uint32_t *h_ovf = reinterpret_cast<const uint32_t *>(t->h_pin + kPinOvf);
        uint64_t need_u = 0, need_c = 0;
        uint32_t max_ovf = 0, guard = 0;
        for (uint32_t c = 0; c < n_chunks; c++) {
            need_u = std::max(need_u, h_pc[kPcUcur + c]); need_c = std::max(need_c, h_pc[kPcCcur + c]);
            max_ovf = std::max(max_ovf, h_ovf[kOvfWords * c + kOvfGroups]);
            guard |= h_ovf[kOvfWords * c + kOvfGuard];
        }
        const uint64_t n_hits = h_pc[kPcBase + n_chunks];
        if (pl.debug)
            fprintf(stderr, "[kg] partition attempt %d: %u chunks (largest %llu of %llu blocks), overflow groups <= %u (cap %u), hit list <= %llu "
                            "(cap %llu), candidates <= %llu (cap %llu), regions/chunk %llu x %u entries, %u buckets, shift %u, %u scatter "
                            "workgroups, hits %llu, %s\n",
                    attempt, n_chunks, (unsigned long long)pl.max_chunk, (unsigned long long)nblocks, max_ovf, pl.ovf_cap,
                    (unsigned long long)need_u, (unsigned long long)ucap, (unsigned long long)need_c, (unsigned long long)ccap,
                    (unsigned long long)pl.n_regions, pl.cap, pl.buckets, pl.shift, pl.n_wg, (unsigned long long)n_hits, pl.use_bidx ? "byte home index" : "tags");
        const bool redo = guard || max_ovf > pl.ovf_cap || need_u > ucap || need_c > ccap;
        if (redo && pl.early_totals) HIP_TRY(hipStreamSynchronize(t->stream));
        if (guard || max_ovf > pl.ovf_cap) {
            st.fallback = guard ? 2 : 1;
            lists.release();
            drop_hits(t, res);
            return KG_OK;
        }
        if (!redo) {
            note_totals(cx, n_hits, pl.part_counters);
            st.partitioned = 1;
            st.part_chunks = (int32_t)n_chunks; st.part_buckets = (int32_t)pl.buckets; st.part_shift = (int32_t)pl.shift;
            st.part_levels = pl.use_bidx ? 4 : 1;
            done = true;
            return KG_OK;
        }
        lists.release();
        drop_hits(t, res);
        if (attempt == 2) break;
        if (need_c > ccap) { pb.ccap = (need_c + pl.list_slack + kg::kUChunk - 1) / kg::kUChunk * kg::kUChunk; pb.ucap = std::max(ucap, pb.ccap); }
        else pb.ucap = (need_u + pl.list_slack + kg::kUChunk - 1) / kg::kUChunk * kg::kUChunk;
    }
    return fail(KG_ERR_DEVICE, "hit list overflow after resize (internal error)");
}

template <bool AA>
int scan_direct(ScanCtx &cx, const DirectPlan &pl)
{
    kg_table *t = cx.t;
    kg_result *res = cx.res;
    kg_stats &st = res->st;
    const uint64_t nblocks = cx.b.nblocks, n_rows = cx.b.n_rows;
    int rc;
    st.scan_launches = 0;
    if (!cx.seq_uploaded) { if ((rc = upload_seq(cx, cx.offsets[0], cx.offsets[cx.n_seqs]))) return rc; cx.seq_uploaded = true; }
    uint64_t stage_cap = pl.stage_cap;
    kg_hit *d_stage = nullptr;
    uint32_t *d_stage_slot = nullptr;
    BlockGuard<2> stage{cx.sc, {(void **)&d_stage, (void **)&d_stage_slot}};
    unsigned long long *d_cursor = (unsigned long long *)(cx.d_totals + kTotCursor);
    unsigned long long *d_ctr = (unsigned long long *)(cx.d_totals + kTotValid);
    for (int attempt = 0;; attempt++) {
        if ((rc = dalloc(t, (void **)&d_stage, stage_cap * sizeof(kg_hit)))) return rc;
        if (cx.progress && (rc = dalloc(t, (void **)&d_stage_slot, stage_cap * 4))) return rc;
        HIP_TRY(hipMemsetAsync(cx.d_totals, 0, kTotWords * 8, t->stream));
        HIP_TRY(hipEventRecord(t->ev[kEvScanBegin], t->stream));
        if (nblocks) {
            const uint64_t wgs = (nblocks + kg::kWavesPerWG - 1) / kg::kWavesPerWG;
            const uint32_t grid = (uint32_t)(wgs < pl.scan_grid ? wgs : pl.scan_grid);
            dispatch<bool, true, false>(cx.counters, [&](auto counters) {
                dispatch<int, 1, 2, 3, 6>((int)pl.rpg, [&](auto rpg) {
                    constexpr bool COUNTERS = decltype(counters)::value;
                    constexpr int RPG = AA ? 1 : decltype(rpg)::value;
                    hipLaunchKernelGGL((kg::scan_kernel<AA, COUNTERS, RPG>), dim3(grid), dim3(kg::kWave * kg::kWavesPerWG), 0, t->stream,
                                       t->d_entries, t->d_tags, t->limit, (uint64_t)t->num_sigs, t->magic, t->m35, cx.d_seq, cx.d_blocks,
                                       (uint32_t)nblocks, cx.d_counts, cx.d_bsb, d_stage, d_cursor, stage_cap, pl.stage_chunk, d_ctr, cx.d_prog,
                                       d_stage_slot, pl.d_hbits, t->tail_start);
                });
            });
            HIP_TRY(hipGetLastError());
        }
        HIP_TRY(hipEventRecord(t->ev[kEvScanEnd], t->stream));
        st.scan_launches++;
        if ((rc = prefix_sum(t, cx.d_counts, n_rows, cx.d_offs, cx.d_partial, cx.d_totals + kTotHits))) return rc;
        if ((rc = send_counters(t, nullptr, nullptr, cx.d_totals, t->stream))) return rc;
        HIP_TRY(hipStreamSynchronize(t->stream));
        const uint64_t need = t->h_pin[kPinTotals + kTotCursor];
        if (need <= stage_cap) break;
        stage.release();
        if (attempt == 1) return fail(KG_ERR_DEVICE, "staging overflow after resize (internal error)");
        stage_cap = need;
    }
    const uint64_t n_hits = n_rows ? t->h_pin[kPinTotals + kTotHits] : 0;
    note_totals(cx, n_hits, cx.counters);

    if ((rc = dalloc(t, (void **)&res->d_hits, n_hits * sizeof(kg_hit)))) return rc;
    if (cx.progress && (rc = dalloc(t, (void **)&res->d_hit_slots, (n_hits ? n_hits : 1) * 4))) return rc;
    if (nblocks) {
        const uint32_t grid = (uint32_t)((nblocks + kg::kWavesPerWG - 1) / kg::kWavesPerWG);
        hipLaunchKernelGGL((kg::place_kernel<AA>), dim3(grid), dim3(kg::kWave * kg::kWavesPerWG), 0, t->stream, cx.d_blocks,
                           (uint32_t)nblocks, cx.d_counts, cx.d_offs, cx.d_bsb, pl.rpg, d_stage, res->d_hits, d_stage_slot, res->d_hit_slots);
    }
    return KG_OK;
}

template <bool AA>
int scan_impl(kg_table *t, const kg_params *p, const uint8_t *d_seq, const uint8_t *h_seq ,
              const int64_t *offsets, int64_t n_seqs, kg_result *res)
{
    constexpr uint32_t PER = AA ? 1 : 6;
    const bool progress = (p->flags & KG_F_PROGRESS) != 0;
    const bool counters_req = (p->flags & KG_F_COUNTERS) != 0;
    const bool aggregate = !(p->flags & KG_F_SKIP_AGGREGATE);
    kg_stats &st = res->st;
    res->per = PER;
    int rc;

    BatchPlan b;
    if ((rc = plan_batch<AA>(offsets, n_seqs, b))) return rc;
    const uint64_t nblocks = b.nblocks, n_rows = b.n_rows, n_cont = b.n_cont;
    st.n_seqs = n_seqs; st.n_containers = (int64_t)n_cont; st.n_blocks = (int64_t)nblocks;
    st.residues = (int64_t)b.residues; st.windows = (int64_t)b.windows;
    st.table_bytes = t->num_sigs * (int64_t)KG_TABLE_ENTRY_SIZE;

    Scratch sc(t);
    ScanCtx cx{t, res, sc, b, d_seq, h_seq, offsets, n_seqs, progress, counters_req || progress, h_seq == nullptr};
    if ((rc = sc.get(&cx.d_off, (size_t)n_seqs + 1))) return rc;
    if ((rc = sc.get(&cx.d_ibase, (size_t)n_seqs + 1))) return rc;
    HIP_TRY(hipMemcpyAsync(cx.d_off, offsets, ((size_t)n_seqs + 1) * 8, hipMemcpyHostToDevice, t->stream));
    HIP_TRY(hipMemcpyAsync(cx.d_ibase, b.ibase.data(), ((size_t)n_seqs + 1) * 4, hipMemcpyHostToDevice, t->stream));
    if ((rc = sc.get(&cx.d_blocks, nblocks))) return rc;
    if ((rc = sc.get(&cx.d_counts, n_rows))) return rc;
    if ((rc = sc.get(&cx.d_offs, n_rows))) return rc;
    if ((rc = sc.get(&cx.d_bsb, nblocks * 6))) return rc;
    if ((rc = sc.get(&cx.d_partial, (size_t)(std::max(n_rows, n_cont) / kg::kScanChunk + 2)))) return rc;
    if ((rc = sc.get(&cx.d_totals, kTotWords))) return rc;
    HIP_TRY(hipMemsetAsync(cx.d_totals, 0, kTotWords * 8, t->stream));
    if ((rc = dalloc(t, (void **)&res->d_chs, (n_cont + 1) * 8))) return rc;
    if (progress && (rc = progress_begin(cx))) return rc;
    HIP_TRY(hipEventRecord(t->ev[kEvBegin], t->stream));
    if (nblocks) {
        hipLaunchKernelGGL(kg::build_blocks_kernel, dim3((uint32_t)((nblocks + 255) / 256)), dim3(256), 0, t->stream,
                           cx.d_off, cx.d_ibase, (uint32_t)n_seqs, (uint32_t)nblocks, cx.d_blocks);
        HIP_TRY(hipGetLastError());
    }

    st.scan_launches = 0;
    PartPlan part;
    if ((rc = plan_partition<AA>(t, b, progress, counters_req, part))) return rc;
    bool part_done = false;
    if (part.applicable && (rc = scan_partitioned<AA>(cx, part, part_done))) return rc;
    if (!part_done && (rc = scan_direct<AA>(cx, plan_direct<AA>(t, b, cx.counters)))) return rc;

    if (progress && (rc = progress_finish(cx, part_done && part.prog_index))) return rc;
    hipLaunchKernelGGL((kg::container_starts_kernel<AA>), dim3((uint32_t)((n_cont + 1 + 255) / 256)), dim3(256), 0, t->stream,
                       cx.d_ibase, (uint32_t)n_seqs, cx.d_offs, n_rows, cx.d_totals, res->d_chs);
    HIP_TRY(hipGetLastError());
    HIP_TRY(hipEventRecord(t->ev[kEvOrderEnd], t->stream));

    if (aggregate && (rc = aggregate_stage(t, p, res, sc, n_seqs, n_cont, cx.n_hits, PER, cx.d_partial, cx.d_totals, nullptr, b.longest < (1ll << 30),
                                         plan_aggregate())))
        return rc;
    HIP_TRY(hipEventRecord(t->ev[kEvAggEnd], t->stream));
    HIP_TRY(hipStreamSynchronize(t->stream));
    st.n_calls = aggregate ? (int64_t)t->h_pin[kPinCalls] : 0;
    if (progress && (rc = progress_fetch(cx))) return rc;
    st.agg_pieces = aggregate ? (int32_t)std::min<uint64_t>(t->h_pin[kPinPieces], 0x7FFFFFFF) : 0;
    float ms = 0;
    HIP_TRY(hipEventElapsedTime(&ms, t->ev[kEvScanBegin], t->ev[kEvScanEnd])); st.ms_scan = ms;
    HIP_TRY(hipEventElapsedTime(&ms, t->ev[kEvScanEnd], t->ev[kEvOrderEnd])); st.ms_order = ms;
    HIP_TRY(hipEventElapsedTime(&ms, t->ev[kEvOrderEnd], t->ev[kEvAggEnd])); st.ms_aggregate = ms;
    HIP_TRY(hipEventElapsedTime(&ms, t->ev[kEvBegin], t->ev[kEvAggEnd])); st.ms_total = ms;
    if (st.partitioned) {
        HIP_TRY(hipEventElapsedTime(&ms, t->ev[kEvScanBegin], t->ev[kEvScattered])); st.ms_part_scatter = ms;
        st.ms_part_tag = 0;
        HIP_TRY(hipEventElapsedTime(&ms, t->ev[kEvScattered], t->ev[kEvJoined])); st.ms_part_verify = ms;
    }
    return KG_OK;
}

int scan_entry(kg_table *t, const kg_params *p, const uint8_t *seq, bool on_device, const int64_t *offsets, int64_t n_seqs,
               kg_result **out)
{
    if (!t || !p || !offsets || !out || n_seqs < 0) return fail(KG_ERR_ARG, "null or negative argument");
    if (n_seqs > 0x7FFFFFF0ll / 6) return fail(KG_ERR_LIMIT, "too many sequences in one batch");
    if (p->min_hits < 2)
        return fail(KG_ERR_UNSUPPORTED, "minHits < 2: the reference throws in processSetOfHits (KGJ:442); refusing");
    CallScope cs(t, "another kg_scan* is in flight on this kg_table (one scan at a time per table; open a second table "
                    "object for concurrent scans)");
    if (cs.rc) return cs.rc;
    int64_t total = offsets[n_seqs] - offsets[0];
    if (total < 0) return fail(KG_ERR_ARG, "offsets must be non-decreasing");
    if (!seq && total > 0) return fail(KG_ERR_ARG, "null sequence buffer");
    kg_result *r = new (std::nothrow) kg_result();
    if (!r) return fail(KG_ERR_NOMEM, "out of host memory");
    r->tab = t;
    uint8_t *d_seq = nullptr;
    int rc = KG_OK;
    if (!on_device) {
        size_t end = (size_t)offsets[n_seqs];
        rc = dalloc(t, (void **)&d_seq, end + 16);
    }
    if (rc == KG_OK) {
        const uint8_t *s = on_device ? seq : d_seq;
        const uint8_t *h = on_device ? nullptr : seq;
        rc = p->aa ? scan_impl<true>(t, p, s, h, offsets, n_seqs, r) : scan_impl<false>(t, p, s, h, offsets, n_seqs, r);
    }
    (void)hipStreamSynchronize(t->stream);
    if (d_seq) dfree(t, d_seq);
    if (rc != KG_OK) return fail_and_free(r, rc);
    *out = r;
    return KG_OK;
}

}

extern "C" {

int kg_scan(kg_table *t, const kg_params *p, const uint8_t *seq, const int64_t *offsets, int64_t n_seqs, kg_result **out)
{
    return scan_entry(t, p, seq, false, offsets, n_seqs, out);
}

int kg_scan_device(kg_table *t, const kg_params *p, const uint8_t *d_seq, const int64_t *offsets, int64_t n_seqs,
                   kg_result **out)
{
    return scan_entry(t, p, d_seq, true, offsets, n_seqs, out);
}

}
```

### kmergutsjava_amd/csrc/kg_order.hpp

```cpp
#pragma once

#include "kg_device.hpp"
#include "kg_partition.hpp"

namespace kg {

constexpr uint32_t kHThreads = 512;
constexpr uint32_t kHPer = 4;
constexpr uint32_t kHTile = kHThreads * kHPer;
constexpr uint32_t kHDigits = 128;
constexpr uint32_t kMaxGroups = kHDigits * kHDigits;

struct RowGeo { uint32_t container; int32_t pos_first; };

template <bool AA>
__global__ void row_geo_kernel(const BlockDesc *__restrict__ blocks, uint32_t n_blocks, RowGeo *__restrict__ geo)
{
    constexpr uint32_t ROWS = AA ? 1 : 6;
    const uint64_t tl = (uint64_t)blockIdx.x * blockDim.x + threadIdx.x;
    if (tl >= (uint64_t)n_blocks * ROWS) return;
    const uint32_t r = (uint32_t)(tl / n_blocks), it = (uint32_t)(tl % n_blocks);
    const BlockDesc bd = blocks[it];
    RowGeo g;
    int32_t pos0;
    row_record_key<AA>(bd, (int)r, 0, &g.container, &pos0);
    g.pos_first = (!AA && r >= 3) ? pos0 - 63 : pos0;
    geo[row_index<AA>(bd, it, (int)r)] = g;
}

__global__ __launch_bounds__(kHThreads) void hit_hist_kernel(const kg_hit *__restrict__ ulist, const uint32_t *__restrict__ chunk_used,
                                                             const unsigned long long *__restrict__ cursor, uint64_t ulist_cap,
                                                             uint32_t g0, uint32_t gs , uint32_t n_groups,
                                                             uint32_t *ghist )
{
    extern __shared__ uint32_t h_lds[];
    for (uint32_t g = threadIdx.x; g < n_groups; g += kHThreads) h_lds[g] = 0;
    __syncthreads();
    const unsigned long long cur = *cursor;
    const uint32_t n_chunks = (uint32_t)((cur < ulist_cap ? cur : ulist_cap) / kUChunk);
    for (uint32_t c = blockIdx.x; c < n_chunks; c += gridDim.x) {
        const uint32_t used = chunk_used[c];
        for (uint32_t k = threadIdx.x; k < used; k += kHThreads) {
            const uint32_t g = (ulist[(uint64_t)c * kUChunk + k].container >> gs) - g0;
            if (g < n_groups) atomicAdd(&h_lds[g], 1u);
        }
    }
    __syncthreads();
    for (uint32_t g = threadIdx.x; g < n_groups; g += kHThreads)
        if (h_lds[g]) atomicAdd(&ghist[g], h_lds[g]);
}

constexpr uint32_t kGsThreads = 256, kGsPer = 4;
__global__ __launch_bounds__(kGsThreads) void group_scan_kernel(const uint32_t *__restrict__ ghist, uint32_t n_groups, uint32_t *__restrict__ gbase,
                                                                uint32_t *__restrict__ cur1, uint32_t *__restrict__ cur2, uint64_t *total_out,
                                                                uint32_t *__restrict__ tile_start)
{
    __shared__ uint32_t wsum[kGsThreads / 64];
    __shared__ uint32_t carry;
    if (threadIdx.x == 0) carry = 0;
    __syncthreads();
    const int lane = threadIdx.x & 63, wave = threadIdx.x >> 6;
    for (uint32_t b = 0; b < n_groups; b += kGsThreads * kGsPer) {
        const uint32_t i0 = b + threadIdx.x * kGsPer;
        uint32_t x[kGsPer], mine = 0;
#pragma unroll
        for (uint32_t k = 0; k < kGsPer; k++) {
            x[k] = i0 + k < n_groups ? ghist[i0 + k] : 0u;
            mine += x[k];
        }
        uint32_t incl = mine;
        for (int off = 1; off < 64; off <<= 1) {
            const uint32_t y = __shfl_up(incl, off);
            if (lane >= off) incl += y;
        }
        if (lane == 63) wsum[wave] = incl;
        __syncthreads();
        uint32_t wbase = 0, all = 0;
        for (int w = 0; w < (int)(kGsThreads / 64); w++) {
            const uint32_t sw = wsum[w];
            if (w < wave) wbase += sw;
            all += sw;
        }
        const uint32_t c = carry;
        uint32_t e = c + wbase + incl - mine;
#pragma unroll
        for (uint32_t k = 0; k < kGsPer; k++) {
            const uint32_t i = i0 + k;
            if (i < n_groups) {
                gbase[i] = e;
                cur2[i] = e;
                if ((i & (kHDigits - 1)) == 0) cur1[i / kHDigits] = e;
            }
            e += x[k];
        }
        __syncthreads();
        if (threadIdx.x == 0) carry = c + all;
        __syncthreads();
    }
    const uint32_t n_d1 = (n_groups + kHDigits - 1) / kHDigits;
    if (threadIdx.x == 0) {
        gbase[n_groups] = carry;
        cur1[n_d1] = carry;
        *total_out = carry;
    }
    __syncthreads();
    const uint32_t d = threadIdx.x;
    const uint32_t t = d < n_d1 ? (cur1[d + 1] - cur1[d] + kHTile - 1) / kHTile : 0u;
    uint32_t incl = t;
    for (int off = 1; off < 64; off <<= 1) {
        const uint32_t y = __shfl_up(incl, off);
        if (lane >= off) incl += y;
    }
    if (d == 63) wsum[0] = incl;
    __syncthreads();
    if (d < kHDigits) {
        const uint32_t before = d >= 64 ? wsum[0] : 0u;
        tile_start[d] = before + incl - t;
        if (d == kHDigits - 1) tile_start[kHDigits] = before + incl;
    }
}

template <bool FIRST>
__global__ __launch_bounds__(kHThreads) void hit_partition_kernel(const kg_hit *__restrict__ in, const uint32_t *__restrict__ chunk_used,
                                                                  const unsigned long long *__restrict__ cursor, uint64_t in_cap,
                                                                  const uint32_t *__restrict__ gbase, uint32_t n_groups, uint32_t g0, uint32_t gs,
                                                                  uint32_t *cur, kg_hit *__restrict__ out, uint64_t out_cap,
                                                                  const uint32_t *__restrict__ tile_start)
{
    __shared__ __attribute__((aligned(16))) kg_hit stage[kHTile];
    __shared__ uint32_t hist[kHDigits], cnt[kHDigits], sbase[kHDigits], gb[kHDigits];
    const uint32_t tid = threadIdx.x, lane = tid & 63u, wave = tid >> 6;
    if (tid < kHDigits) hist[tid] = 0;
    const uint32_t n_d1 = (n_groups + kHDigits - 1) / kHDigits;
    uint32_t n_res = 0;
    if (FIRST) {
        const unsigned long long cc = *cursor;
        n_res = (uint32_t)((cc < in_cap ? cc : in_cap) / kUChunk);
    }
    __shared__ uint32_t tstart[kHDigits + 1];
    if (!FIRST) {
        if (tid <= kHDigits) tstart[tid] = tile_start[tid];
        __syncthreads();
    }
    const uint32_t n_items = FIRST ? (n_res + kHTile / kUChunk - 1) / (kHTile / kUChunk) : tstart[kHDigits];
    {
        for (uint32_t item = blockIdx.x; item < n_items; item += gridDim.x) {
            uint32_t d1 = 0, tile = item;
            if (!FIRST) {
                uint32_t lo_d = 0, hi_d = n_d1;
                while (hi_d - lo_d > 1) {
                    const uint32_t mid = (lo_d + hi_d) / 2;
                    if (tstart[mid] <= item) lo_d = mid; else hi_d = mid;
                }
                d1 = lo_d;
                tile = item - tstart[d1];
            }
            const uint32_t seg_lo = FIRST ? 0u : gbase[d1 * kHDigits];
            const uint32_t seg_hi = FIRST ? 0u : gbase[min((d1 + 1) * kHDigits, n_groups)];
            kg_hit rec[kHPer];
            uint32_t dr[kHPer];
#pragma unroll
            for (uint32_t k = 0; k < kHPer; k++) {
                const uint32_t i = k * kHThreads + tid;
                bool ok;
                uint64_t at;
                if (FIRST) {
                    const uint32_t c = tile * (kHTile / kUChunk) + i / kUChunk;
                    ok = c < n_res && (i % kUChunk) < chunk_used[c];
                    at = (uint64_t)c * kUChunk + (i % kUChunk);
                } else {
                    at = (uint64_t)seg_lo + (uint64_t)tile * kHTile + i;
                    ok = at < seg_hi;
                }
                dr[k] = ~0u;
                if (ok) {
                    rec[k] = stream_load_hit(in + at);
                    const uint32_t g = (rec[k].container >> gs) - g0;
                    if (g < n_groups) {
                        const uint32_t d = FIRST ? g / kHDigits : g % kHDigits;
                        dr[k] = (d << 16) | atomicAdd(&hist[d], 1u);
                    }
                }
            }
            __syncthreads();
            if (tid < kHDigits) {
                const uint32_t c = hist[tid];
                uint32_t incl = c;
                for (int off = 1; off < 64; off <<= 1) {
                    const uint32_t y = __shfl_up(incl, off);
                    if ((int)lane >= off) incl += y;
                }
                cnt[tid] = c;
                sbase[tid] = incl - c;
                gb[tid] = c ? atomicAdd(&cur[FIRST ? tid : d1 * kHDigits + tid], c) : 0u;
                hist[tid] = 0;
            }
            __syncthreads();
            const uint32_t first_half = sbase[63] + cnt[63];
#pragma unroll
            for (uint32_t k = 0; k < kHPer; k++)
                if (dr[k] != ~0u) {
                    const uint32_t d = dr[k] >> 16;
                    stage[sbase[d] + (d >= 64 ? first_half : 0u) + (dr[k] & 0xFFFFu)] = rec[k];
                }
            __syncthreads();
            const uint64_t *stage64 = reinterpret_cast<const uint64_t *>(stage);
            uint64_t *out64 = reinterpret_cast<uint64_t *>(out);
            for (uint32_t d = wave; d < kHDigits; d += kHThreads / 64u) {
                const uint32_t n = cnt[d];
                if (n == 0) continue;
                const uint32_t s0 = sbase[d] + (d >= 64 ? first_half : 0u);
                const uint64_t o0 = gb[d];
                const uint32_t n_ok = o0 >= out_cap ? 0u : (uint32_t)min((uint64_t)n, out_cap - o0);
                for (uint32_t i = lane; i < 3u * n_ok; i += 64u) stream_store8(out64 + o0 * 3u + i, stage64[(uint64_t)s0 * 3u + i]);
            }
            __syncthreads();
        }
    }
}

constexpr uint32_t kPlaceOut = 1536;
__host__ __device__ inline size_t group_place_lds(uint32_t gshift, bool staged)
{
    return staged ? ((size_t)20 << gshift) + (size_t)kPlaceOut * sizeof(kg_hit) : ((size_t)12 << gshift);
}
template <bool AA>
__global__ __launch_bounds__(kHThreads) void group_place_kernel(const kg_hit *__restrict__ in, const uint32_t *__restrict__ gbase, uint32_t n_groups,
                                                                uint32_t g0, uint32_t gshift, uint32_t row_lo, uint32_t row_hi ,
                                                                const RowGeo *__restrict__ geo, uint64_t n_rows_all, uint32_t staged,
                                                                const uint64_t *__restrict__ base,
                                                                kg_hit *__restrict__ hits, uint64_t hits_cap, uint32_t *__restrict__ offs,
                                                                uint32_t *__restrict__ hit_slots )
{
    extern __shared__ __attribute__((aligned(16))) unsigned char p_lds[];
    const uint32_t R = 1u << gshift;
    unsigned long long *masks = reinterpret_cast<unsigned long long *>(p_lds);
    uint32_t *pre = reinterpret_cast<uint32_t *>(masks + R);
    RowGeo *lgeo = reinterpret_cast<RowGeo *>(pre + R);
    uint64_t *lout = reinterpret_cast<uint64_t *>(lgeo + R);
    __shared__ uint32_t wsum[kHThreads / 64];
    const uint32_t tid = threadIdx.x, lane = tid & 63u, wave = tid >> 6;
    const uint64_t chunk_base = *base;
    const uint32_t per = R / kHThreads > 0 ? R / kHThreads : 1u;
    for (uint32_t g = blockIdx.x; g < n_groups; g += gridDim.x) {
        const uint32_t lo = gbase[g], n = gbase[g + 1] - lo;
        const uint64_t row0 = (uint64_t)(g0 + g) << gshift;
        const bool to_lds = staged && n <= kPlaceOut;
        for (uint32_t i = tid; i < R; i += kHThreads) {
            masks[i] = 0ull;
            if (staged && n && row0 + i < n_rows_all) lgeo[i] = geo[row0 + i];
        }
        __syncthreads();
        constexpr uint32_t kKeep = 4;
        const bool keep = n <= kHThreads * kKeep;
        kg_hit rk[kKeep];
        if (keep) {
#pragma unroll
            for (uint32_t j = 0; j < kKeep; j++) {
                const uint32_t k = j * kHThreads + tid;
                if (k < n) {
                    rk[j] = stream_load_hit(in + lo + k);
                    atomicOr(&masks[(rk[j].container >> 6) & (R - 1u)], 1ull << (rk[j].container & 63u));
                }
            }
        } else {
            for (uint32_t k = tid; k < n; k += kHThreads) {
                const uint32_t key = in[lo + k].container;
                atomicOr(&masks[(key >> 6) & (R - 1u)], 1ull << (key & 63u));
            }
        }
        __syncthreads();
        uint32_t mine = 0;
        const uint32_t r_lo = tid * per;
        if (r_lo < R)
            for (uint32_t i = 0; i < per; i++) mine += (uint32_t)__popcll(masks[r_lo + i]);
        uint32_t incl = mine;
        for (int off = 1; off < 64; off <<= 1) {
            const uint32_t y = __shfl_up(incl, off);
            if ((int)lane >= off) incl += y;
        }
        if (lane == 63) wsum[wave] = incl;
        __syncthreads();
        uint32_t run = incl - mine;
        for (uint32_t w = 0; w < wave; w++) run += wsum[w];
        if (r_lo < R)
            for (uint32_t i = 0; i < per; i++) {
                pre[r_lo + i] = run;
                const uint64_t row = row0 + r_lo + i;
                if (row >= row_lo && row < row_hi) offs[row] = (uint32_t)(chunk_base + lo + run);
                run += (uint32_t)__popcll(masks[r_lo + i]);
            }
        __syncthreads();
        auto place = [&](kg_hit h) {
            const uint32_t key = h.container, rl = (key >> 6) & (R - 1u), ol = key & 63u;
            const RowGeo gr = staged ? lgeo[rl] : geo[key >> 6];
            const uint32_t rank = pre[rl] + (uint32_t)__popcll(masks[rl] & ((1ull << ol) - 1ull));
            if (hit_slots && chunk_base + lo + rank < hits_cap)
                hit_slots[chunk_base + lo + rank] = (uint32_t)h.from0InProt;
            h.container = gr.container;
            h.from0InProt = gr.pos_first + (int32_t)ol;
            if (to_lds) {
                uint64_t w3[3];
                __builtin_memcpy(w3, &h, 24);
                lout[3u * rank] = w3[0]; lout[3u * rank + 1] = w3[1]; lout[3u * rank + 2] = w3[2];
            } else {
                const uint64_t dst = chunk_base + lo + rank;
                if (dst < hits_cap) hits[dst] = h;
            }
        };
        if (keep) {
#pragma unroll
            for (uint32_t j = 0; j < kKeep; j++)
                if (j * kHThreads + tid < n) place(rk[j]);
        } else {
            for (uint32_t k = tid; k < n; k += kHThreads) place(in[lo + k]);
        }
        __syncthreads();
        if (to_lds) {
            const uint64_t dst0 = chunk_base + lo;
            const uint32_t n_ok = dst0 >= hits_cap ? 0u : (uint32_t)min((uint64_t)n, hits_cap - dst0);
            uint64_t *out64 = reinterpret_cast<uint64_t *>(hits) + dst0 * 3u;
            for (uint32_t i = tid; i < 3u * n_ok; i += kHThreads) stream_store8(out64 + i, lout[i]);
            __syncthreads();
        }
    }
}

__global__ __launch_bounds__(256) void restore_hits_kernel(const kg_hit *__restrict__ src, uint64_t n_hits, const int64_t *__restrict__ seq_first,
                                                           uint64_t n_seqs, const int64_t *__restrict__ dst_first,
                                                           const int32_t *__restrict__ container_shift, kg_hit *__restrict__ dst)
{
    __shared__ uint64_t k_first;
    constexpr uint64_t kTile = 1024;
    const uint64_t n_tiles = (n_hits + kTile - 1) / kTile;
    for (uint64_t tile = blockIdx.x; tile < n_tiles; tile += gridDim.x) {
        __syncthreads();
        if (threadIdx.x == 0) {
            const uint64_t i0 = tile * kTile;
            uint64_t lo = 0, hi = n_seqs;
            while (hi - lo > 1) {
                const uint64_t mid = lo + (hi - lo) / 2;
                if ((uint64_t)seq_first[mid] <= i0) lo = mid; else hi = mid;
            }
            k_first = lo;
        }
        __syncthreads();
        uint64_t k = k_first;
#pragma unroll
        for (int j = 0; j < 4; j++) {
            const uint64_t i = tile * kTile + (uint64_t)j * 256 + threadIdx.x;
            if (i < n_hits) {
                while (k + 1 < n_seqs && (uint64_t)seq_first[k + 1] <= i) k++;
                kg_hit h = src[i];
                h.container += (uint32_t)container_shift[k];
                dst[(uint64_t)dst_first[k] + (i - (uint64_t)seq_first[k])] = h;
            }
        }
    }
}

}
```

### kmergutsjava_amd/csrc/kg_partition.hpp

```cpp
#pragma once

#include "kg_device.hpp"

namespace kg {

constexpr int kMaxBuckets = 1024;
#ifndef KG_PROBE_N
#define KG_PROBE_N 4
#endif
#ifndef KG_SCATTER_WPE
#define KG_SCATTER_WPE 5
#endif
#ifndef KG_TAG_WPE
#define KG_TAG_WPE 8
#endif
#if KG_SCATTER_WPE
#define KG_SCATTER_REGS __attribute__((amdgpu_waves_per_eu(KG_SCATTER_WPE)))
#else
#define KG_SCATTER_REGS
#endif
#if KG_TAG_WPE
#define KG_TAG_REGS __attribute__((amdgpu_waves_per_eu(KG_TAG_WPE)))
#else
#define KG_TAG_REGS
#endif
#ifndef KG_STAGE_FLUSH
#define KG_STAGE_FLUSH 64
#endif
#ifndef KG_SCATTER_RG
#define KG_SCATTER_RG 6
#endif

#ifndef KG_SCAN_FULL
#define KG_SCAN_FULL 1
#endif

constexpr uint32_t kStageFlush = KG_STAGE_FLUSH;
constexpr int kProbeN = KG_PROBE_N;
#ifndef KG_INDEX_N
#define KG_INDEX_N KG_PROBE_N
#endif
constexpr int kIndexN = KG_INDEX_N;
constexpr uint32_t kUChunk = 512;

constexpr uint64_t kEntInvalid = ~0ull;

template <bool AA>
__device__ __forceinline__ uint32_t window_key(const BlockDesc &bd, uint32_t it, int r, int lane)
{
    const uint32_t ol = (!AA && r >= 3) ? 63u - (uint32_t)lane : (uint32_t)lane;
    return (row_index<AA>(bd, it, r) << 6) | ol;
}
#ifndef KG_SCATTER_WAVES
#define KG_SCATTER_WAVES 16
#endif
constexpr int kScatterWaves = KG_SCATTER_WAVES;
constexpr uint32_t kGroup = 16;

template <bool AA>
inline size_t scatter_lds_bytes(uint32_t n_buckets)
{
    size_t enc = (sizeof(typename WaveLds<AA>::type) + 15) & ~(size_t)15;
    size_t tab = (sizeof(typename WaveLds<AA>::tables) + 15) & ~(size_t)15;
    return enc * kScatterWaves + tab + (size_t)n_buckets * (kGroup * 8 + 8);
}
template <bool AA>
constexpr uint32_t scatter_flush_list_max()
{
    constexpr size_t idle = AA ? sizeof(WaveLdsAa) : KG_SCATTER_RG == 6 ? sizeof(WaveLdsDna) : sizeof(WaveLdsDna::bc);
    return idle / 4 < 64 ? (uint32_t)(idle / 4) : 64u;
}

#ifndef KG_SCATTER_NT
#define KG_SCATTER_NT 1
#endif
__device__ __forceinline__ void store_entry_pair(uint64_t *dst, const ulonglong2 &v)
{
#if KG_SCATTER_NT
    typedef uint64_t u64x2 __attribute__((ext_vector_type(2)));
    u64x2 x; x.x = v.x; x.y = v.y;
    __builtin_nontemporal_store(x, reinterpret_cast<u64x2 *>(dst));
#else
    *reinterpret_cast<ulonglong2 *>(dst) = v;
#endif
}

struct ScatterCold {
    uint32_t *ovf_cursor;
    uint32_t *ovf_bucket;
    uint64_t *ovf_ent;
    uint32_t *lowc_cursor;
    uint32_t *lowc_blocks;
    unsigned long long *ctr;
    Progress *prog;
    uint32_t ovf_cap, pad;
};
static_assert(sizeof(ScatterCold) == 64, "ScatterCold is one 64-byte line");

constexpr unsigned long long kDstOvf = 1ull << 62, kDstNone = ~0ull, kDstDropped = ~0ull - 1;

__device__ __forceinline__ unsigned long long overflow_reserve(const ScatterCold *__restrict__ cold, unsigned long long movf, bool to_ovf,
                                                               uint32_t b, unsigned long long dst)
{
    const int lane = threadIdx.x & 63;
    uint32_t og = 0;
    if (lane == 0) og = atomicAdd(cold->ovf_cursor, (uint32_t)__popcll(movf));
    og = (uint32_t)__builtin_amdgcn_readfirstlane((int)og);
    if (to_ovf) {
        const uint32_t g = og + (uint32_t)__popcll(movf & ((1ull << lane) - 1ull));
        if (g < cold->ovf_cap) { cold->ovf_bucket[g] = b; dst = kDstOvf | ((uint64_t)g * kGroup); }
        else dst = kDstDropped;
    }
    return dst;
}
__device__ __attribute__((noinline, cold)) unsigned long long scatter_overflow_groups(const ScatterCold *__restrict__ cold,
                                                                                     unsigned long long movf, bool to_ovf, uint32_t b,
                                                                                     unsigned long long dst)
{
    return overflow_reserve(cold, movf, to_ovf, b, dst);
}
__device__ __attribute__((noinline, cold)) void scatter_overflow_octets(const ScatterCold *__restrict__ cold, bool full, uint32_t b,
                                                                        uint64_t lo, uint64_t hi)
{
    const int lane = threadIdx.x & 63;
    const bool lead = full && (lane & 7) == 0;
    unsigned long long dst = overflow_reserve(cold, __ballot(lead), lead, b, kDstNone);
    dst = __shfl(dst, lane & ~7);
    if (full && dst != kDstDropped) {
        ulonglong2 v; v.x = lo; v.y = hi;
        store_entry_pair(cold->ovf_ent + (dst & ~kDstOvf) + 2 * ((uint32_t)lane & 7u), v);
    }
}
__device__ __attribute__((noinline, cold)) void scatter_store_overflow(const ScatterCold *__restrict__ cold, unsigned long long to,
                                                                       uint32_t sub, uint64_t lo, uint64_t hi)
{
    ulonglong2 v; v.x = lo; v.y = hi;
    store_entry_pair(cold->ovf_ent + (to & ~kDstOvf) + 2 * sub, v);
}
__device__ __attribute__((noinline, cold)) void scatter_set_aside(const ScatterCold *__restrict__ cold, uint32_t block)
{
    if ((threadIdx.x & 63) == 0) cold->lowc_blocks[atomicAdd(cold->lowc_cursor, 1u)] = block;
}
__device__ __attribute__((noinline, cold)) void scatter_protocol_failure(const ScatterCold *__restrict__ cold)
{
    if ((threadIdx.x & 63) == 0) atomicOr(cold->ovf_cursor + 2, 1u);
}
__device__ __attribute__((noinline, cold)) void scatter_note_beyond(const ScatterCold *__restrict__ cold, uint32_t slot)
{
    progress_note_beyond(cold->prog, slot);
}

struct BlockRows { uint32_t len, j, nk, ibase; };
__device__ __forceinline__ BlockRows rows_of(const BlockDesc &bd) { return BlockRows{bd.len, bd.j, bd.nk, bd.ibase}; }
__device__ __forceinline__ BlockDesc desc_of(const BlockRows &r)
{
    BlockDesc bd;
    bd.soff = 0; bd.len = r.len; bd.j = r.j; bd.nk = r.nk; bd.ibase = r.ibase; bd.seq = 0; bd.pad = 0;
    return bd;
}

template <bool AA, bool SHORT = false, bool PROG = false>
__global__ __launch_bounds__(kWave *kScatterWaves) KG_SCATTER_REGS void part_scatter_kernel(
    const uint8_t *__restrict__ seq, const BlockDesc *__restrict__ blocks, uint32_t block_lo, uint32_t n_blocks ,
    uint32_t limit32 , uint32_t num_sigs , uint32_t m35, uint32_t shift,
    uint32_t n_buckets, uint32_t cap, uint64_t *__restrict__ ent, uint32_t *__restrict__ fill, const ScatterCold *__restrict__ cold,
    uint32_t insert_prio , uint32_t flush_list )
{
    static_assert(SHORT || !PROG, "PROG implies SHORT");
    constexpr int ROWS = AA ? 1 : 6;
    typedef typename WaveLds<AA>::type Enc;
    constexpr size_t enc_bytes = (sizeof(Enc) + 15) & ~(size_t)15;
    extern __shared__ __attribute__((aligned(16))) unsigned char part_lds[];
    const int lane = threadIdx.x & 63, wave = __builtin_amdgcn_readfirstlane((int)(threadIdx.x >> 6));
    Enc &l = *reinterpret_cast<Enc *>(part_lds + enc_bytes * wave);
    typedef typename WaveLds<AA>::tables Tables;
    constexpr size_t tab_bytes = (sizeof(Tables) + 15) & ~(size_t)15;
    Tables &enc_tables = *reinterpret_cast<Tables *>(part_lds + enc_bytes * kScatterWaves);
    uint64_t *buf = reinterpret_cast<uint64_t *>(part_lds + enc_bytes * kScatterWaves + tab_bytes);
    uint32_t *cnt = reinterpret_cast<uint32_t *>(buf + (size_t)n_buckets * kGroup);
    uint32_t *written = cnt + n_buckets;
    uint32_t *flist = reinterpret_cast<uint32_t *>(&l);
    const uint32_t w = blockIdx.x, n_wg = gridDim.x;
    const uint32_t gcap = cap >> 4;
    const uint32_t list_cap = max(min(flush_list, scatter_flush_list_max<AA>()), 1u);
    for (uint32_t b = threadIdx.x; b < n_buckets; b += blockDim.x) { cnt[b] = 0; written[b] = 0; }
    encode_init<AA>(enc_tables, threadIdx.x, blockDim.x);
    __syncthreads();

    uint32_t n_valid = 0;
    bool ran_off = false;
    const uint32_t n_iter = (n_blocks + n_wg * kScatterWaves - 1) / (n_wg * kScatterWaves);
    BlockRows rows_next = {0, 0, 0, 0};
    uint32_t raw_next[4] = {0, 0, 0, 0};
    {
        const uint32_t it0 = w * kScatterWaves + (uint32_t)wave;
        if (it0 < n_blocks) {
            const BlockDesc bd0 = blocks[block_lo + it0];
            load_block_chars<AA>(seq, bd0, lane, raw_next);
            rows_next = rows_of(bd0);
        }
    }
    constexpr int RG = AA ? 1 : KG_SCATTER_RG;
    static_assert(ROWS % RG == 0, "KG_SCATTER_RG must divide 6");
    for (uint32_t iter = 0; iter < n_iter; iter++) {
        const uint32_t it = (iter * n_wg + w) * kScatterWaves + (uint32_t)wave;
        const BlockDesc bd = desc_of(rows_next);
        const bool have = it < n_blocks;
        if (have) {
            uint32_t raw[4] = {raw_next[0], raw_next[1], raw_next[2], raw_next[3]};
            const uint32_t itn = it + n_wg * kScatterWaves;
            if (itn < n_blocks) {
                const BlockDesc bdn = blocks[block_lo + itn];
                load_block_chars<AA>(seq, bdn, lane, raw_next);
                rows_next = rows_of(bdn);
            }
            encode_chars<AA>(l, enc_tables, raw, lane);
        }
        bool lowc = false;
#pragma unroll
        for (int g0 = 0; g0 < ROWS; g0 += RG) {
        uint64_t e[RG];
        uint32_t bk[RG];
        uint32_t pend = 0, nv = 0;
        if (have && !lowc) {
#pragma unroll
            for (int k = 0; k < RG; k++) {
                const int r = g0 + k;
                uint32_t hi, lo, q;
                bool valid = row_halves<AA>(l, r, lane, bd, &hi, &lo);
                const uint32_t slot = split_fast(hi, lo, num_sigs, m35, &q);
                if (valid) nv++;
                if constexpr (SHORT) {
                    if (valid && slot >= limit32) {
                        ran_off = true;
                        if constexpr (PROG) scatter_note_beyond(cold, slot);
                    }
                    valid = valid && slot < limit32;
                }
                bk[k] = slot >> shift;
                const uint32_t low = (q << shift) | (slot & ((1u << shift) - 1u));
                const uint32_t id = window_key<AA>(bd, block_lo + it, r, lane);
                e[k] = ((uint64_t)id << 32) | low;
                if (valid) pend |= 1u << k;
            }
            if (g0 + RG == ROWS) wave_sync();
            if (g0 == 0) {
                const unsigned long long m0 = __ballot((pend & 1u) != 0);
                if (__popcll(m0) >= 32) {
                    const uint32_t lead0 = (uint32_t)__builtin_amdgcn_readlane((int)bk[0], __builtin_ctzll(m0));
                    if (__builtin_expect(__popcll(__ballot((pend & 1u) && bk[0] == lead0)) >= 24, 0)) {
                        scatter_set_aside(cold, block_lo + it);
                        nv = 0;
                        pend = 0;
                        lowc = true;
                        if (RG != ROWS) wave_sync();
                    }
                }
            }
        }
        n_valid += nv;
        uint32_t spins = 0;
        if (insert_prio) set_wave_prio(insert_prio);
        for (;;) {
            uint32_t at[RG], old[RG];
#pragma unroll
            for (int r = 0; r < RG; r++)
                at[r] = (pend & (1u << r)) ? atomicAdd(&cnt[bk[r]], 1u) : kGroup;
#pragma unroll
            for (int r = 0; r < RG; r++) {
                old[r] = 0;
                if (at[r] < kGroup) {
                    buf[(size_t)bk[r] * kGroup + at[r]] = e[r];
                    __builtin_amdgcn_fence(__ATOMIC_RELEASE, "wavefront");
                    old[r] = atomicAdd(&written[bk[r]], 1u);
                }
            }
            __builtin_amdgcn_fence(__ATOMIC_ACQUIRE, "wavefront");
#pragma unroll
            for (int r = 0; r < RG; r++) pend &= ~((uint32_t)(at[r] < kGroup) << r);
            uint32_t at_max = at[0];
#pragma unroll
            for (int r = 1; r < RG; r++) at_max = max(at_max, at[r]);
            uint32_t left = 0;
            auto list_rows = [&](auto again) -> uint32_t {
                uint32_t n = 0;
#pragma unroll
                for (int r = 0; r < RG; r++) {
                    const bool own = decltype(again)::value ? ((left >> r) & 1u) != 0 : (old[r] & 15u) == 15u;
                    const unsigned long long m = __ballot(own);
                    if (m) {
                        const uint32_t rank = __builtin_amdgcn_mbcnt_hi((uint32_t)(m >> 32), __builtin_amdgcn_mbcnt_lo((uint32_t)m, n));
                        if (own && rank < list_cap) {
                            const uint32_t g = decltype(again)::value ? (written[bk[r]] >> 4) - 1u : old[r] >> 4;
                            flist[rank] = (min(g, gcap) << 10) | bk[r];
                            if (decltype(again)::value) left &= ~(1u << r);
                        }
                        n += (uint32_t)__popcll(m);
                    }
                }
                return n;
            };
            uint32_t n_own = list_rows(std::false_type{});
            if (__builtin_expect(n_own > list_cap, 0)) {
                uint32_t k = 0;
#pragma unroll
                for (int r = 0; r < RG; r++) {
                    const bool own = (old[r] & 15u) == 15u;
                    const unsigned long long m = __ballot(own);
                    const uint32_t rank = __builtin_amdgcn_mbcnt_hi((uint32_t)(m >> 32), __builtin_amdgcn_mbcnt_lo((uint32_t)m, k));
                    if (own && rank >= list_cap) left |= 1u << r;
                    k += (uint32_t)__popcll(m);
                }
            }
            while (n_own) {
                const uint32_t n_list = min(n_own, list_cap);
                wave_sync();
                for (uint32_t p0 = 0; p0 < n_list; p0 += 8) {
                    const uint32_t want = p0 + ((uint32_t)lane >> 3), sub = (uint32_t)lane & 7u;
                    if (want < n_list) {
                        const uint32_t d = flist[want];
                        const uint32_t fb = d & (uint32_t)(kMaxBuckets - 1), g = d >> 10;
                        const ulonglong2 v = *reinterpret_cast<const ulonglong2 *>(buf + (size_t)fb * kGroup + 2 * sub);
                        __builtin_amdgcn_fence(__ATOMIC_RELEASE, "wavefront");
                        if (sub == 0) cnt[fb] = 0;
                        const bool full = g >= gcap;
                        if (!full) {
                            unsigned char *to = reinterpret_cast<unsigned char *>(ent) + (mul24_wide(__umul24(fb, n_wg) + w, cap) << 3);
                            store_entry_pair(reinterpret_cast<uint64_t *>(to + ((g << 7) | (sub << 4))), v);
                        }
                        if (__builtin_expect(__ballot(full) != 0, 0)) scatter_overflow_octets(cold, full, fb, v.x, v.y);
                    }
                }
                wave_sync();
                if (__builtin_expect(n_own <= list_cap, 1)) break;
                n_own = list_rows(std::true_type{});
            }
            if (!__ballot(pend != 0)) break;
            {
                const int rp = pend ? __builtin_ctz(pend) : 0;
                uint32_t pb = bk[0];
#pragma unroll
                for (int r = 1; r < RG; r++)
                    if (rp == r) pb = bk[r];
                for (uint32_t polls = 0; polls < 64; polls++) {
                    if (__ballot(pend != 0 && __hip_atomic_load(&cnt[pb], __ATOMIC_RELAXED, __HIP_MEMORY_SCOPE_WORKGROUP) < kGroup)) break;
                    __builtin_amdgcn_s_sleep(2);
                }
            }
            if (__builtin_expect(++spins > (1u << 20) || __ballot(at_max >= (1u << 28)), 0)) {
                scatter_protocol_failure(cold);
                break;
            }
        }
        if (insert_prio) set_wave_prio(0);
        }
    }
    __syncthreads();
    const uint32_t per_wave = (n_buckets + kScatterWaves - 1) / kScatterWaves;
    const uint32_t b_end = min((uint32_t)(wave + 1) * per_wave, n_buckets);
    for (uint32_t b0 = (uint32_t)wave * per_wave; b0 < b_end; b0 += 64) {
        const uint32_t b = b0 + (uint32_t)lane;
        const uint32_t wr = b < b_end ? written[b] : 0u;
        const uint32_t c = wr & 15u, g = wr >> 4;
        unsigned long long dst = kDstNone;
        bool to_ovf = false;
        if (c > 0) {
            for (uint32_t k = c; k < kGroup; k++) buf[(size_t)b * kGroup + k] = kEntInvalid;
            if (g < gcap) dst = ((uint64_t)b * n_wg + w) * cap + ((uint64_t)g << 4);
            else to_ovf = true;
        }
        const unsigned long long movf = __ballot(to_ovf);
        if (movf) dst = scatter_overflow_groups(cold, movf, to_ovf, b, dst);
        unsigned long long m = __ballot(dst != kDstNone);
        wave_sync();
        while (m) {
            int src_lane = -1;
            unsigned long long mm = m;
#pragma unroll
            for (int o = 0; o < 8; o++) {
                const int ln = mm ? __builtin_ctzll(mm) : -1;
                if (mm) mm &= mm - 1;
                if ((lane >> 3) == o) src_lane = ln;
            }
            m = mm;
            const int sl = src_lane < 0 ? 0 : src_lane;
            const uint32_t fb = (uint32_t)__shfl((int)b, sl);
            const unsigned long long to = __shfl(dst, sl);
            if (src_lane >= 0) {
                const uint32_t sub = (uint32_t)lane & 7u;
                const ulonglong2 v = *reinterpret_cast<const ulonglong2 *>(buf + (size_t)fb * kGroup + 2 * sub);
                if (__builtin_expect((to & kDstOvf) != 0, 0)) {
                    if (to != kDstDropped) scatter_store_overflow(cold, to, sub, v.x, v.y);
                } else {
                    store_entry_pair(ent + to + 2 * sub, v);
                }
            }
        }
    }
    for (uint32_t b = threadIdx.x; b < n_buckets; b += blockDim.x)
        fill[(uint64_t)b * n_wg + w] = min((written[b] + 15u) >> 4, gcap) << 4;
    for (int off = 32; off > 0; off >>= 1) n_valid += __shfl_down(n_valid, off);
    unsigned long long *ctr = cold->ctr;
    if (lane == 0 && n_valid) atomicAdd(&ctr[0], (unsigned long long)n_valid);
    if constexpr (SHORT) flush_ran_off(ran_off, ctr, lane);
}

constexpr int kLowcWaves = 4;
template <bool AA>
__global__ __launch_bounds__(64 * kLowcWaves) void lowc_blocks_kernel(
    const uint8_t *__restrict__ seq, const BlockDesc *__restrict__ blocks, const uint32_t *__restrict__ lowc_cursor,
    const uint32_t *__restrict__ lowc_blocks, uint64_t limit, uint32_t num_sigs, uint32_t m35, uint32_t shift, uint32_t n_regions,
    uint32_t cap, uint64_t *__restrict__ ent, uint32_t *__restrict__ fill, uint32_t *ovf_cursor, uint32_t ovf_cap,
    uint32_t *__restrict__ ovf_bucket, uint64_t *__restrict__ ovf_ent, unsigned long long *ctr, Progress *prog)
{
    constexpr int ROWS = AA ? 1 : 6;
    __shared__ typename WaveLds<AA>::type lds[kLowcWaves];
    __shared__ typename WaveLds<AA>::tables enc_tables;
    const int lane = threadIdx.x & 63, wave = threadIdx.x >> 6;
    typename WaveLds<AA>::type &l = lds[wave];
    const uint32_t n_list = *lowc_cursor;
    if (n_list == 0) return;
    encode_init<AA>(enc_tables, threadIdx.x, blockDim.x);
    __syncthreads();
    const uint32_t limit32 = limit < 0xFFFFFFFFull ? (uint32_t)limit : 0xFFFFFFFFu;
    unsigned long long n_valid = 0;
    bool ran_off = false;
    uint32_t pool_at = 0, pool_end = 0;
    auto pool_flush = [&]() {
        for (uint32_t g = pool_at + ((uint32_t)lane >> 4); g < pool_end && g < ovf_cap; g += 4) {
            if ((lane & 15) == 0) ovf_bucket[g] = 0;
            ovf_ent[(uint64_t)g * kGroup + ((uint32_t)lane & 15u)] = kEntInvalid;
        }
        pool_at = pool_end;
    };
    auto ovf_groups = [&](uint32_t lead, uint32_t ng) -> uint64_t * {
        if (pool_end - pool_at < ng) {
            pool_flush();
            const uint32_t want = ng > 32u ? ng : 32u;
            uint32_t g0 = 0;
            if (lane == 0) g0 = atomicAdd(ovf_cursor, want);
            g0 = (uint32_t)__builtin_amdgcn_readfirstlane((int)g0);
            pool_at = g0; pool_end = g0 + want;
        }
        const uint32_t g = pool_at;
        pool_at += ng;
        if (g + ng > ovf_cap) return nullptr;
        if ((uint32_t)lane < ng) ovf_bucket[g + lane] = lead;
        return ovf_ent + (uint64_t)g * kGroup;
    };
    for (uint32_t i = blockIdx.x * kLowcWaves + (uint32_t)wave; i < n_list; i += gridDim.x * kLowcWaves) {
        const uint32_t it = (uint32_t)__builtin_amdgcn_readfirstlane((int)lowc_blocks[i]);
        const BlockDesc bd = blocks[it];
        encode_block<AA>(l, enc_tables, seq, bd, lane);
        const uint32_t region_w = it % n_regions;
        for (int r = 0; r < ROWS; r++) {
            uint32_t hi, lo, q;
            bool valid = row_halves<AA>(l, r, lane, bd, &hi, &lo);
            const uint32_t slot = split_fast(hi, lo, num_sigs, m35, &q);
            if (valid) n_valid++;
            if (valid && slot >= limit32) { ran_off = true; if (prog) progress_note_beyond(prog, slot); }
            bool pend = valid && slot < limit32;
            const uint32_t bkt = slot >> shift;
            const uint64_t e = ((uint64_t)window_key<AA>(bd, it, r, lane) << 32) | ((q << shift) | (slot & ((1u << shift) - 1u)));
            for (int pass = 0; pass < 4; pass++) {
                const unsigned long long mp = __ballot(pend);
                if (__popcll(mp) < 16) break;
                const uint32_t lead = (uint32_t)__builtin_amdgcn_readlane((int)bkt, __builtin_ctzll(mp));
                const bool mine = pend && bkt == lead;
                const unsigned long long same = __ballot(mine);
                const uint32_t n = (uint32_t)__popcll(same);
                if (n < 8) break;
                const uint32_t rank = (uint32_t)__popcll(same & ((1ull << lane) - 1ull));
                const uint64_t region = (uint64_t)lead * n_regions + region_w;
                uint32_t rel = cap;
                if (lane == 0 && *const_cast<volatile uint32_t *>(&fill[region]) < cap) rel = atomicAdd(&fill[region], n);
                rel = (uint32_t)__builtin_amdgcn_readfirstlane((int)rel);
                if (rel + n <= cap) {
                    if (mine) ent[region * cap + rel + rank] = e;
                } else {
                    if (rel < cap && (uint32_t)lane < cap - rel) ent[region * cap + rel + lane] = kEntInvalid;
                    const uint32_t npad = (n + kGroup - 1) & ~(kGroup - 1);
                    uint64_t *dst = ovf_groups(lead, npad / kGroup);
                    if (dst) {
                        if (mine) dst[rank] = e;
                        if ((uint32_t)lane < npad - n) dst[n + lane] = kEntInvalid;
                    }
                }
                if (mine) pend = false;
            }
            if (pend) {
                const uint64_t region = (uint64_t)bkt * n_regions + region_w;
                const uint32_t rel = atomicAdd(&fill[region], 1u);
                if (rel < cap) { ent[region * cap + rel] = e; pend = false; }
            }
            for (;;) {
                const unsigned long long mp = __ballot(pend);
                if (!mp) break;
                const uint32_t lead = (uint32_t)__builtin_amdgcn_readlane((int)bkt, __builtin_ctzll(mp));
                const bool mine = pend && bkt == lead;
                const unsigned long long same = __ballot(mine);
                const uint32_t n = (uint32_t)__popcll(same);
                const uint32_t npad = (n + kGroup - 1) & ~(kGroup - 1);
                const uint32_t rank = (uint32_t)__popcll(same & ((1ull << lane) - 1ull));
                uint64_t *dst = ovf_groups(lead, npad / kGroup);
                if (dst) {
                    if (mine) dst[rank] = e;
                    if ((uint32_t)lane < npad - n) dst[n + lane] = kEntInvalid;
                }
                if (mine) pend = false;
            }
        }
        wave_sync();
    }
    pool_flush();
    for (int off = 32; off > 0; off >>= 1) n_valid += __shfl_down(n_valid, off);
    if (lane == 0 && n_valid) atomicAdd(&ctr[0], n_valid);
    flush_ran_off(ran_off, ctr, lane);
}

struct UListState { unsigned long long base; uint32_t used; bool have; };

template <bool AA, int N, bool COUNTERS>
__device__ __forceinline__ void probe_entries(const TableView &tab, uint32_t b, uint32_t shift, const uint64_t (&e)[N],
                                              kg_hit *__restrict__ ulist, uint32_t *__restrict__ chunk_used,
                                              unsigned long long *cursor, uint64_t ulist_cap, UListState &u,
                                              unsigned long long &ctr_slots, bool &ran_off, int lane, Progress *prog)
{
    uint64_t val[N], slot[N];
    bool valid[N];
    uint32_t id[N], fp[N];
#pragma unroll
    for (int k = 0; k < N; k++) {
        valid[k] = e[k] != kEntInvalid;
        const uint32_t low = (uint32_t)e[k];
        id[k] = (uint32_t)(e[k] >> 32);
        slot[k] = ((uint64_t)b << shift) | (low & ((1u << shift) - 1u));
        val[k] = (uint64_t)(low >> shift) * tab.num_sigs + slot[k];
        fp[k] = tag_qs(low >> shift, slot[k]);
    }
    Payload pay[N];
    unsigned long long ctr_dummy = 0;
    uint32_t fslot[N];
#pragma unroll
    for (int k = 0; k < N; k++) fslot[k] = 0;
    const uint32_t foundm = probe_n<N, COUNTERS>(tab, val, slot, fp, valid, pay, ctr_dummy, ctr_slots, ran_off, COUNTERS ? prog : nullptr,
                                                 COUNTERS ? fslot : nullptr);
    uint32_t cnt[N], rank[N], total = 0;
#pragma unroll
    for (int k = 0; k < N; k++) {
        const bool f = (foundm >> k) & 1u;
        const unsigned long long m = __ballot(f);
        cnt[k] = (uint32_t)__popcll(m);
        rank[k] = (uint32_t)__popcll(m & ((1ull << lane) - 1ull));
        total += cnt[k];
    }
    if (total) {
        if (u.used + total > kUChunk) {
            if (lane == 0 && u.have && u.base + kUChunk <= ulist_cap) chunk_used[u.base / kUChunk] = u.used;
            unsigned long long nb = 0;
            if (lane == 0) nb = atomicAdd(cursor, (unsigned long long)kUChunk);
            nb = ((unsigned long long)__builtin_amdgcn_readfirstlane((uint32_t)(nb >> 32)) << 32) |
                 (unsigned long long)__builtin_amdgcn_readfirstlane((uint32_t)nb);
            u.base = nb; u.used = 0; u.have = true;
        }
        if (u.base + kUChunk <= ulist_cap) {
            uint32_t at = u.used;
#pragma unroll
            for (int k = 0; k < N; k++) {
                if ((foundm >> k) & 1u) {
                    kg_hit h;
                    h.container = id[k];
                    h.from0InProt = (int32_t)fslot[k];
                    h.oI = pay[k].oI; h.avgOffFromEnd = pay[k].avg; h.fI = pay[k].fI; h.functionWt = pay[k].wt;
                    ulist[u.base + at + rank[k]] = h;
                }
                at += cnt[k];
            }
        }
        u.used += total;
    }
}

struct CandRec { uint32_t home, quo, id, walked; };
constexpr uint32_t kWalkOn = 0x80000000u;
constexpr uint32_t kScanOn = 0x40000000u;
constexpr uint32_t kWalkedMask = 0x3FFFFFFFu;
static_assert(sizeof(CandRec) == 16, "CandRec must be 16 bytes");

__device__ __forceinline__ unsigned long long chunk_reserve(UListState &u, uint32_t total, uint32_t *__restrict__ chunk_used,
                                                            unsigned long long *cursor, uint64_t cap, int lane)
{
    if (u.used + total > kUChunk) {
        if (lane == 0 && u.have && u.base + kUChunk <= cap) chunk_used[u.base / kUChunk] = u.used;
        unsigned long long nb = 0;
        if (lane == 0) nb = atomicAdd(cursor, (unsigned long long)kUChunk);
        nb = ((unsigned long long)__builtin_amdgcn_readfirstlane((uint32_t)(nb >> 32)) << 32) |
             (unsigned long long)__builtin_amdgcn_readfirstlane((uint32_t)nb);
        u.base = nb; u.used = 0; u.have = true;
    }
    const unsigned long long at = u.base + u.used;
    u.used += total;
    return u.base + kUChunk <= cap ? at : ~0ull;
}

__device__ __forceinline__ void chunk_finish(const UListState &u, uint32_t *__restrict__ chunk_used, uint64_t cap, int lane)
{
    if (lane == 0 && u.have && u.base + kUChunk <= cap) chunk_used[u.base / kUChunk] = u.used;
}

template <bool COUNTERS>
__global__ __launch_bounds__(256) KG_TAG_REGS void bucket_tag_kernel(
    const uint8_t *__restrict__ tags, uint64_t limit, uint64_t num_sigs, const uint64_t *__restrict__ ent,
    const uint32_t *__restrict__ fill, uint32_t n_regions, uint32_t cap, uint32_t n_buckets, uint32_t shift,
    uint32_t grab ,
    uint32_t *next_region ,
    CandRec *__restrict__ cand, uint32_t *__restrict__ cand_used, unsigned long long *cand_cursor, uint64_t cand_cap,
    unsigned long long *ctr, Progress *prog )
{
    constexpr int N = kProbeN;
    const uint32_t lim32 = (uint32_t)limit;
    __shared__ uint32_t s_region;
    __shared__ __attribute__((aligned(16))) CandRec s_stage[4][kStageFlush + 64];
    CandRec *stage = s_stage[__builtin_amdgcn_readfirstlane((int)(threadIdx.x >> 6))];
    uint32_t sfill = 0;
    const int lane = threadIdx.x & 63;
    unsigned long long ctr_slots = 0;
    bool ran_off = false;
    UListState u;
    u.base = 0; u.used = kUChunk; u.have = false;

    const uint32_t kGrab = grab;
    const uint32_t grabs_per_region = (cap + kGrab - 1) / kGrab;
    const uint32_t n_grabs = n_regions * grabs_per_region;
    const uint32_t xg = blockIdx.x & 7u;
    const uint32_t n_tickets = xg < n_buckets ? ((n_buckets - xg + 7u) / 8u) * n_grabs : 0u;
    for (;;) {
        __syncthreads();
        if (threadIdx.x == 0) s_region = atomicAdd(&next_region[xg * 32u], 1u);
        __syncthreads();
        const uint32_t tk = s_region;
        if (tk >= n_tickets) break;
        const uint32_t b = xg + 8u * (tk / n_grabs), g = tk % n_grabs;
        const uint32_t w = g / grabs_per_region, g0 = (g % grabs_per_region) * kGrab;
        const uint32_t fraw = fill[(uint64_t)b * n_regions + w];
        uint32_t n = cap;
        const uint64_t *src = ent + ((uint64_t)b * n_regions + w) * cap;
        for (uint32_t c0 = g0; c0 < n && c0 < g0 + kGrab; c0 += 256u * N) {
            const uint32_t bound = n;
            uint32_t low[N], id[N], fp[N], skip[N], walked[N];
            uint32_t vmask = 0;
            Tags16 tg[N];
            const uint32_t smask = (1u << shift) - 1u, bbase = b << shift;
            uint64_t ev[N];
#pragma unroll
            for (int k = 0; k < N; k++) {
                const uint32_t i = c0 + (uint32_t)k * 256u + threadIdx.x;
                ev[k] = i < bound ? __builtin_nontemporal_load(src + i) : kEntInvalid;
            }
            if (c0 == g0) {
                uint32_t f = fraw;
                asm volatile("; fill first used here" : "+s"(f));
                n = min(f, cap);
            }
#pragma unroll
            for (int k = 0; k < N; k++) {
                const uint64_t e = c0 + (uint32_t)k * 256u + threadIdx.x < n ? ev[k] : kEntInvalid;
                if (e != kEntInvalid) vmask |= 1u << k;
                low[k] = (uint32_t)e;
                id[k] = (uint32_t)(e >> 32);
                const uint32_t home = bbase | (low[k] & smask);
                fp[k] = tag_qs(low[k] >> shift, home);
                const uint32_t cur = (uint32_t)probe_window(home, &skip[k]);
                if ((vmask >> k) & 1u) tg[k] = load_tags(tags + cur);
            }
            uint32_t candm = 0, walkm = 0;
#pragma unroll
            for (int k = 0; k < N; k++) {
                walked[k] = 0;
                if ((vmask >> k) & 1u) {
                    bool emp;
                    const int i = first_stop(tg[k], fp[k], &emp, skip[k]);
                    walked[k] = (uint32_t)i - skip[k];
                    if (i == 16) { candm |= 1u << k; walkm |= 1u << k; }
                    else if (!emp) candm |= 1u << k;
                    else {
                        const uint32_t home = bbase | (low[k] & smask), at = home + walked[k];
                        if (at >= lim32) ran_off = true;
                        if (COUNTERS) {
                            ctr_slots += (at < lim32 ? at + 1u : lim32) - home;
                            if (prog) progress_note_walk(prog, home, at, lim32);
                        }
                    }
                }
            }
#pragma unroll
            for (int k = 0; k < N; k++) {
                const unsigned long long m = __ballot((candm >> k) & 1u);
                if (!m) continue;
                if ((candm >> k) & 1u) {
                    CandRec c;
                    c.home = bbase | (low[k] & smask); c.quo = low[k] >> shift;
                    c.id = id[k]; c.walked = walked[k] | (((walkm >> k) & 1u) ? kWalkOn : 0u);
                    stage[sfill + (uint32_t)__popcll(m & ((1ull << lane) - 1ull))] = c;
                }
                sfill += (uint32_t)__popcll(m);
                while (sfill >= kStageFlush) {
                    wave_sync();
                    const unsigned long long at = chunk_reserve(u, kStageFlush, cand_used, cand_cursor, cand_cap, lane);
                    if ((uint32_t)lane < kStageFlush) {
                        const ulonglong2 out = *reinterpret_cast<const ulonglong2 *>(stage + lane);
                        if (at != ~0ull) stream_store16(cand + at + (uint32_t)lane, &out);
                    }
                    sfill -= kStageFlush;
                    wave_sync();
                    if ((uint32_t)lane < sfill) {
                        const ulonglong2 rest = *reinterpret_cast<const ulonglong2 *>(stage + kStageFlush + lane);
                        *reinterpret_cast<ulonglong2 *>(stage + lane) = rest;
                    }
                    wave_sync();
                }
            }
        }
    }
    if (sfill) {
        wave_sync();
        const CandRec out = stage[(uint32_t)lane < sfill ? lane : 0];
        const unsigned long long at = chunk_reserve(u, sfill, cand_used, cand_cursor, cand_cap, lane);
        if (at != ~0ull && (uint32_t)lane < sfill) stream_store16(cand + at + (uint32_t)lane, &out);
    }
    chunk_finish(u, cand_used, cand_cap, lane);
    flush_ran_off(ran_off, ctr, lane);
    if (COUNTERS) {
        for (int off = 32; off > 0; off >>= 1) ctr_slots += __shfl_down(ctr_slots, off);
        if (lane == 0) atomicAdd(&ctr[1], ctr_slots);
    }
}

template <int N, int R, bool EXACT, bool PROG = false>
__global__ __launch_bounds__(256) KG_TAG_REGS void bucket_index_kernel(
    const uint8_t *__restrict__ bidx, uint32_t tail_start,
    const uint64_t *__restrict__ ent, const uint32_t *__restrict__ fill, uint32_t n_regions , uint32_t cap, uint32_t n_buckets,
    uint32_t shift, uint32_t grab ,
    uint32_t *next_region ,
    CandRec *__restrict__ cand, uint32_t *__restrict__ cand_used, unsigned long long *cand_cursor, uint64_t cand_cap,
    unsigned long long *ctr, uint32_t prio , Progress *prog )
{
    static_assert(N % R == 0, "R must divide N");
    constexpr int PER = N / R;
    __shared__ uint32_t s_region;
    __shared__ uint32_t s_lut[256];
    __shared__ __attribute__((aligned(16))) CandRec s_stage[4][kStageFlush + 64];
    CandRec *stage = s_stage[__builtin_amdgcn_readfirstlane((int)(threadIdx.x >> 6))];
    uint32_t sfill = 0;
    const int lane = threadIdx.x & 63;
    bool ran_off = false;
    UListState u;
    u.base = 0; u.used = kUChunk; u.have = false;
    s_lut[threadIdx.x] = bidx_decode(threadIdx.x);
    if (prio) set_wave_prio(prio);

    const uint32_t kGrab = grab;
    const uint32_t grabs_per_region = (cap + kGrab - 1) / kGrab;
    const uint32_t n_grabs = (n_regions / R) * grabs_per_region;
    const uint32_t xg = blockIdx.x & 7u;
    const uint32_t n_tickets = xg < n_buckets ? ((n_buckets - xg + 7u) / 8u) * n_grabs : 0u;
    constexpr uint32_t all_walk = EXACT ? 0u : kBidxInexact;
    for (;;) {
        __syncthreads();
        if (threadIdx.x == 0) s_region = atomicAdd(&next_region[xg * 32u], 1u);
        __syncthreads();
        const uint32_t tk = s_region;
        if (tk >= n_tickets) break;
        const uint32_t b = xg + 8u * (tk / n_grabs), g = tk % n_grabs;
        const uint32_t w = (g / grabs_per_region) * R, g0 = (g % grabs_per_region) * kGrab;
        uint32_t fraw[R], n[R], nmax = cap;
#pragma unroll
        for (int r = 0; r < R; r++) { fraw[r] = fill[(uint64_t)b * n_regions + w + r]; n[r] = cap; }
        const uint64_t *src = ent + ((uint64_t)b * n_regions + w) * cap;
        const uint32_t smask = (1u << shift) - 1u, bbase = b << shift;
        uint32_t d_lo = 0, d_hi = 0, pmin = ~0u, pmax1 = 0;
        if (PROG) {
            const uint64_t s0 = (uint64_t)b << shift, s1 = (((uint64_t)b + 1) << shift) - 1;
#pragma unroll
            for (int k = 1; k <= 10; k++) { d_lo += prog->lo[k] <= s0 ? 1u : 0u; d_hi += prog->lo[k] <= s1 ? 1u : 0u; }
        }
        for (uint32_t c0 = g0; c0 < nmax && c0 < g0 + kGrab; c0 += 256u * PER) {
            uint64_t ev[N];
#pragma unroll
            for (int k = 0; k < N; k++) {
                const int r = k / PER;
                const uint32_t i = c0 + (uint32_t)(k % PER) * 256u + threadIdx.x;
                ev[k] = i < n[r] ? __builtin_nontemporal_load(src + (uint64_t)r * cap + i) : kEntInvalid;
            }
            if (c0 == g0) {
                nmax = 0;
#pragma unroll
                for (int r = 0; r < R; r++) {
                    uint32_t f = fraw[r];
                    asm volatile("; fill first used here" : "+s"(f));
                    n[r] = min(f, cap);
                    nmax = max(nmax, n[r]);
                }
            }
            uint32_t code[N], vmask = 0;
#pragma unroll
            for (int k = 0; k < N; k++) {
                if (c0 + (uint32_t)(k % PER) * 256u + threadIdx.x >= n[k / PER]) ev[k] = kEntInvalid;
                code[k] = 0;
                if (ev[k] != kEntInvalid) {
                    vmask |= 1u << k;
                    code[k] = bidx[bbase | ((uint32_t)ev[k] & smask)];
                }
            }
            uint32_t candm = 0, walkm = 0, wd[N];
#pragma unroll
            for (int k = 0; k < N; k++) wd[k] = s_lut[code[k]];
#pragma unroll
            for (int k = 0; k < N; k++) {
                const uint32_t q = (uint32_t)ev[k] >> shift;
                const uint32_t c = EXACT ? q : q % kBidxClasses;
                const uint32_t listed = (wd[k] >> c) & 1u;
                candm |= listed << k;
                walkm |= (listed & ((wd[k] | all_walk) >> 31)) << k;
                ran_off = ran_off || (((vmask >> k) & 1u) && !listed && (bbase | ((uint32_t)ev[k] & smask)) >= tail_start);
            }
            if (PROG) {
                if (d_lo == d_hi) {
#pragma unroll
                    for (int k = 0; k < N; k++) {
                        const uint32_t h = bbase | ((uint32_t)ev[k] & smask);
                        if ((vmask >> k) & 1u) pmin = min(pmin, h);
                        if (((vmask & ~candm) >> k) & 1u) pmax1 = max(pmax1, h + 1u);
                    }
                } else {
                    for (int k = 0; k < N; k++)
                        if ((vmask >> k) & 1u) progress_note_home(prog, d_lo, d_hi, bbase | ((uint32_t)ev[k] & smask), (candm >> k) & 1u);
                }
            }
#pragma unroll
            for (int k = 0; k < N; k++) {
                const unsigned long long m = __ballot((candm >> k) & 1u);
                if (!m) continue;
                if ((candm >> k) & 1u) {
                    CandRec c;
                    c.home = bbase | ((uint32_t)ev[k] & smask); c.quo = (uint32_t)ev[k] >> shift;
                    c.id = (uint32_t)(ev[k] >> 32); c.walked = ((walkm >> k) & 1u) ? kWalkOn : kScanOn;
                    stage[sfill + (uint32_t)__popcll(m & ((1ull << lane) - 1ull))] = c;
                }
                sfill += (uint32_t)__popcll(m);
                while (sfill >= kStageFlush) {
                    wave_sync();
                    const unsigned long long at = chunk_reserve(u, kStageFlush, cand_used, cand_cursor, cand_cap, lane);
                    if ((uint32_t)lane < kStageFlush) {
                        const ulonglong2 out = *reinterpret_cast<const ulonglong2 *>(stage + lane);
                        if (at != ~0ull) stream_store16(cand + at + (uint32_t)lane, &out);
                    }
                    sfill -= kStageFlush;
                    wave_sync();
                    if ((uint32_t)lane < sfill) {
                        const ulonglong2 rest = *reinterpret_cast<const ulonglong2 *>(stage + kStageFlush + lane);
                        *reinterpret_cast<ulonglong2 *>(stage + lane) = rest;
                    }
                    wave_sync();
                }
            }
        }
        if (PROG && d_lo == d_hi) progress_note_homes(prog, d_lo, pmin, pmax1);
    }
    if (sfill) {
        wave_sync();
        const CandRec out = stage[(uint32_t)lane < sfill ? lane : 0];
        const unsigned long long at = chunk_reserve(u, sfill, cand_used, cand_cursor, cand_cap, lane);
        if (at != ~0ull && (uint32_t)lane < sfill) stream_store16(cand + at + (uint32_t)lane, &out);
    }
    chunk_finish(u, cand_used, cand_cap, lane);
    flush_ran_off(ran_off, ctr, lane);
}

template <bool AA, bool COUNTERS, bool PROG = false>
__global__ __launch_bounds__(256) void verify_kernel(
    const uint8_t *__restrict__ entries, const uint8_t *__restrict__ tags, uint64_t limit, uint64_t num_sigs, uint64_t magic,
    const CandRec *__restrict__ cand, const uint32_t *__restrict__ cand_used, const unsigned long long *cand_cursor,
    uint64_t cand_cap, kg_hit *__restrict__ ulist, uint32_t *__restrict__ chunk_used, unsigned long long *cursor,
    uint64_t ulist_cap, unsigned long long *ctr, Progress *prog ,
    uint32_t prio )
{
    const int lane = threadIdx.x & 63;
    const uint32_t wave_global = __builtin_amdgcn_readfirstlane(blockIdx.x * 4 + (threadIdx.x >> 6));
    const uint32_t n_waves = gridDim.x * 4;
    if (prio) set_wave_prio(prio);
    TableView tab;
    tab.entries = entries; tab.tags = tags; tab.limit = limit; tab.num_sigs = num_sigs; tab.magic = magic; tab.m35 = 0;
    const unsigned long long cur = *cand_cursor;
    const uint32_t n_chunks = (uint32_t)((cur < cand_cap ? cur : cand_cap) / kUChunk);
    unsigned long long ctr_slots = 0;
    bool ran_off = false;
    UListState u;
    u.base = 0; u.used = kUChunk; u.have = false;
    for (uint32_t c = wave_global; c < n_chunks; c += n_waves) {
        const uint32_t used = cand_used[c];
        for (uint32_t k0 = 0; k0 < used; k0 += 64) {
            const bool act = k0 + (uint32_t)lane < used;
            CandRec r;
            r.home = 0; r.quo = 0; r.id = 0; r.walked = 0;
            if (act) {
                const kg_u32x4 cv = __builtin_nontemporal_load(reinterpret_cast<const kg_u32x4 *>(cand + (uint64_t)c * kUChunk + k0 + lane));
                r.home = cv.x; r.quo = cv.y; r.id = cv.z; r.walked = cv.w;
            }
            const uint64_t quo = r.quo, home = r.home;
            const uint64_t val = quo * num_sigs + home;
            uint64_t s = home + (r.walked & kWalkedMask);
            bool found = false;
            Entry e;
            e.key = 0; e.oI = e.avg = e.fI = 0; e.wt = 0.f;
            if (act && (r.walked & kScanOn)) {
#if KG_SCAN_FULL
                if (s < limit) {
                    const uint64_t s1 = s + 1 < limit ? s + 1 : s, s2 = s + 2 < limit ? s + 2 : s;
                    const Entry e0 = load_entry(tab, s);
                    const uint2 k1 = *reinterpret_cast<const uint2 *>(tab.entries + s1 * 24);
                    const uint2 k2 = *reinterpret_cast<const uint2 *>(tab.entries + s2 * 24);
                    const uint32_t vlo = (uint32_t)val, vhi = (uint32_t)(val >> 32);
                    if (e0.key == (int64_t)val) { found = true; e = e0; }
                    else if (s + 1 < limit && k1.x == vlo && k1.y == vhi) { found = true; s += 1; e = load_entry(tab, s); }
                    else if (s + 2 < limit && k2.x == vlo && k2.y == vhi) { found = true; s += 2; e = load_entry(tab, s); }
                    else s += 3;
                }
#endif
                while (!found) {
                    if (s >= limit) { s = limit; ran_off = true; break; }
                    const uint64_t s1 = s + 1 < limit ? s + 1 : s, s2 = s + 2 < limit ? s + 2 : s;
                    const uint2 k0 = *reinterpret_cast<const uint2 *>(tab.entries + s * 24);
                    const uint2 k1 = *reinterpret_cast<const uint2 *>(tab.entries + s1 * 24);
                    const uint2 k2 = *reinterpret_cast<const uint2 *>(tab.entries + s2 * 24);
                    const uint32_t vlo = (uint32_t)val, vhi = (uint32_t)(val >> 32);
                    if (k0.x == vlo && k0.y == vhi) found = true;
                    else if (s + 1 < limit && k1.x == vlo && k1.y == vhi) { found = true; s += 1; }
                    else if (s + 2 < limit && k2.x == vlo && k2.y == vhi) { found = true; s += 2; }
                    if (found) { e = load_entry(tab, s); break; }
                    s += 3;
                }
                if (COUNTERS) {
                    ctr_slots += (s < limit ? s + 1 : limit) - home;
                    if (prog) progress_note_walk(prog, home, s, limit);
                } else if (PROG) {
                    progress_note_walk(prog, home, s, limit);
                }
            } else if (act) {
                if (!(r.walked & kWalkOn)) {
                    e = load_entry(tab, s);
                    found = e.key == (int64_t)val;
                    if (!found) s += 1;
                }
                if (!found) {
                    const uint32_t f = tag_qs(quo, home);
                    for (;;) {
                        if (s >= limit) { s = limit; ran_off = true; break; }
                        const Tags16 x = load_tags(tab.tags + s);
                        bool emp;
                        const int i = first_stop(x, f, &emp);
                        if (i == 16) { s += 16; continue; }
                        s += (uint64_t)i;
                        if (emp) { if (s >= limit) ran_off = true; break; }
                        e = load_entry(tab, s);
                        if (e.key == (int64_t)val) { found = true; break; }
                        s += 1;
                    }
                }
                if (COUNTERS) {
                    ctr_slots += (s < limit ? s + 1 : limit) - home;
                    if (prog) progress_note_walk(prog, home, s, limit);
                } else if (PROG) {
                    progress_note_walk(prog, home, s, limit);
                }
            }
            const unsigned long long m = __ballot(found);
            const uint32_t total = (uint32_t)__popcll(m);
            if (total) {
                const unsigned long long at = chunk_reserve(u, total, chunk_used, cursor, ulist_cap, lane);
                if (at != ~0ull && found) {
                    kg_hit h;
                    h.container = r.id;
                    h.from0InProt = (int32_t)(uint32_t)s;
                    h.oI = e.oI; h.avgOffFromEnd = e.avg; h.fI = e.fI; h.functionWt = e.wt;
                    stream_store_hit(ulist + at + (uint32_t)__popcll(m & ((1ull << lane) - 1ull)), h);
                }
            }
        }
    }
    chunk_finish(u, chunk_used, ulist_cap, lane);
    flush_ran_off(ran_off, ctr, lane);
    if (COUNTERS) {
        for (int off = 32; off > 0; off >>= 1) ctr_slots += __shfl_down(ctr_slots, off);
        if (lane == 0) atomicAdd(&ctr[1], ctr_slots);
    }
}

template <bool AA, bool COUNTERS, bool PROG = false>
__global__ __launch_bounds__(256) void overflow_probe_kernel(
    const uint8_t *__restrict__ entries, const uint8_t *__restrict__ tags, uint64_t limit, uint64_t num_sigs, uint64_t magic,
    const uint32_t *__restrict__ ovf_bucket, const uint64_t *__restrict__ ovf_ent, const uint32_t *__restrict__ ovf_cursor,
    uint32_t ovf_cap, uint32_t shift, kg_hit *__restrict__ ulist, uint32_t *__restrict__ chunk_used, unsigned long long *cursor, uint64_t ulist_cap,
    unsigned long long *ctr, Progress *prog)
{
    const int lane = threadIdx.x & 63;
    const uint32_t wave_global = __builtin_amdgcn_readfirstlane(blockIdx.x * 4 + (threadIdx.x >> 6));
    const uint32_t n_waves = gridDim.x * 4;
    TableView tab;
    tab.entries = entries; tab.tags = tags; tab.limit = limit; tab.num_sigs = num_sigs; tab.magic = magic; tab.m35 = 0;
    unsigned long long ctr_slots = 0;
    bool ran_off = false;
    UListState u;
    u.base = 0; u.used = kUChunk; u.have = false;
    const uint32_t n_groups = min(*ovf_cursor, ovf_cap);
    for (uint32_t g = wave_global; g < n_groups; g += n_waves) {
        const uint32_t b = ovf_bucket[g];
        uint64_t e[1];
        e[0] = lane < (int)kGroup ? ovf_ent[(uint64_t)g * kGroup + lane] : kEntInvalid;
        probe_entries<AA, 1, COUNTERS || PROG>(tab, b, shift, e, ulist, chunk_used, cursor, ulist_cap, u, ctr_slots, ran_off, lane, prog);
    }
    if (lane == 0 && u.have && u.base + kUChunk <= ulist_cap) chunk_used[u.base / kUChunk] = u.used;
    flush_ran_off(ran_off, ctr, lane);
    if (COUNTERS) {
        for (int off = 32; off > 0; off >>= 1) ctr_slots += __shfl_down(ctr_slots, off);
        if (lane == 0) atomicAdd(&ctr[1], ctr_slots);
    }
}

__global__ void chunk_base_kernel(const uint64_t *chunk_total, uint64_t *base, uint64_t *grand_total)
{
    const uint64_t b = base[0] + *chunk_total;
    base[1] = b;
    if (grand_total) *grand_total = b;
}

}
```

Before: 131.4 billion residues/s.

## Split hit keys into a compact array and derive row geometry per sequence

```diff
diff --git a/kmergutsjava_amd/csrc/kg_device.hpp b/kmergutsjava_amd/csrc/kg_device.hpp
--- a/kmergutsjava_amd/csrc/kg_device.hpp
+++ b/kmergutsjava_amd/csrc/kg_device.hpp
@@ -4,6 +4,7 @@
 #include <stdint.h>
 
 #include "../../include/kmerguts_hip.h"
+#include "kg_rows.hpp"
 
 namespace kg {
 
@@ -11,21 +12,12 @@
 constexpr int kWavesPerWG = 4;
 constexpr int kDnaPosPerBlock = 192;
 constexpr int kAaWinPerBlock = 64;
+static_assert(kDnaPosPerBlock == kRowDnaPos && kAaWinPerBlock == kRowAaWin, "kg_rows.hpp restates the blocks' sizes");
 constexpr uint32_t kInvalid = 0xFFFFFFFFu;
 constexpr uint32_t kTagEmpty = 0xFFu;
 constexpr uint64_t kNotFound = ~0ull;
 constexpr int kTagPad = 64;
 
-struct BlockDesc {
-    uint64_t soff;
-    uint32_t len;
-    uint32_t j;
-    uint32_t nk;
-    uint32_t ibase;
-    uint32_t seq;
-    uint32_t pad;
-};
-static_assert(sizeof(BlockDesc) == 32, "BlockDesc must be 32 bytes");
 
 struct TableView {
     const uint8_t *entries;
@@ -185,6 +177,11 @@
     kg_u32x2 b; b.x = (uint32_t)h.fI; b.y = __float_as_uint(h.functionWt);
     __builtin_nontemporal_store(a, reinterpret_cast<kg_u32x4 *>(dst));
     __builtin_nontemporal_store(b, reinterpret_cast<kg_u32x2 *>(reinterpret_cast<unsigned char *>(dst) + 16));
+}
+__device__ __forceinline__ void ulist_append(kg_hit *__restrict__ ulist, uint32_t *__restrict__ ukeys, uint64_t at, const kg_hit &h)
+{
+    stream_store_hit(ulist + at, h);
+    __builtin_nontemporal_store(h.container, ukeys + at);
 }
 __device__ __forceinline__ kg_hit stream_load_hit(const kg_hit *src)
 {
@@ -424,30 +421,6 @@
     }
 }
 
-template <bool AA>
-__device__ __forceinline__ uint32_t row_index(const BlockDesc &bd, uint32_t it, int r)
-{
-    if (AA) return it;
-    const uint32_t vbase = 6u * bd.ibase;
-    if (r < 3) return vbase + (uint32_t)r * bd.nk + bd.j;
-    return vbase + (3u + (bd.len - (uint32_t)(r - 3)) % 3u) * bd.nk + (bd.nk - 1u - bd.j);
-}
-
-template <bool AA>
-__device__ __forceinline__ void row_record_key(const BlockDesc &bd, int r, int lane, uint32_t *container, int32_t *pos)
-{
-    if (AA) {
-        *container = bd.seq;
-        *pos = (int32_t)(bd.j * kAaWinPerBlock + lane);
-    } else if (r < 3) {
-        *container = bd.seq * 6u + (uint32_t)r;
-        *pos = (int32_t)(bd.j * 64u + lane);
-    } else {
-        const uint32_t f = (uint32_t)(r - 3);
-        *container = bd.seq * 6u + 3u + (bd.len - f) % 3u;
-        *pos = (int32_t)((bd.len - 24u - f - bd.j * kDnaPosPerBlock) / 3u) - (int32_t)lane;
-    }
-}
 
 struct Progress {
     unsigned long long first[11];
diff --git a/kmergutsjava_amd/csrc/kg_host_plan.hpp b/kmergutsjava_amd/csrc/kg_host_plan.hpp
--- a/kmergutsjava_amd/csrc/kg_host_plan.hpp
+++ b/kmergutsjava_amd/csrc/kg_host_plan.hpp
@@ -179,6 +179,12 @@
     return KG_OK;
 }
 
+template <bool AA>
+uint32_t plan_row_owners(const BatchPlan &b, const int64_t *offsets, int64_t n_seqs, uint32_t gshift, std::vector<uint32_t> &words)
+{
+    return kg::row_owner_words<AA>(b.ibase.data(), offsets, n_seqs, gshift, words);
+}
+
 struct DirectPlan {
     uint32_t scan_grid, stage_chunk;
     const uint32_t *d_hbits;
diff --git a/kmergutsjava_amd/csrc/kg_host_scan.hpp b/kmergutsjava_amd/csrc/kg_host_scan.hpp
--- a/kmergutsjava_amd/csrc/kg_host_scan.hpp
+++ b/kmergutsjava_amd/csrc/kg_host_scan.hpp
@@ -133,12 +133,14 @@
     uint32_t *d_fill = nullptr, *d_ovf_bucket = nullptr, *d_next = nullptr;
     uint32_t *d_ovfc = nullptr;
     uint32_t *d_lowc = nullptr;
-    kg::RowGeo *d_geo = nullptr;
+    uint32_t *d_owners = nullptr;
+    uint32_t n_listed = 0;
     uint64_t *d_pc = nullptr;
     uint32_t *d_ghist = nullptr, *d_gbase = nullptr, *d_gcur1 = nullptr, *d_gcur2 = nullptr, *d_gtile = nullptr;
     uint64_t ucap = 0, ccap = 0;
     size_t cused_stride = 0, candused_stride = 0;
     kg_hit *d_ulist = nullptr, *d_sortA = nullptr, *d_sortB = nullptr;
+    uint32_t *d_ukeys = nullptr;
     uint32_t *d_cused = nullptr, *d_candused = nullptr;
     kg::CandRec *d_cand = nullptr;
 };
@@ -148,6 +150,7 @@
     uint64_t *ent, *ovf_ent;
     uint32_t *fill, *next, *ovfc, *ovf_bucket;
     kg_hit *ulist, *sortA, *sortB;
+    uint32_t *ukeys;
     uint32_t *cused, *candused;
     kg::CandRec *cand;
     unsigned long long *ucur, *ccur;
@@ -164,7 +167,7 @@
     v.next = pb.d_next + (size_t)c * pl.next_stride;
     v.ovfc = pb.d_ovfc + kOvfWords * c; v.ovf_bucket = pb.d_ovf_bucket + (size_t)c * pl.ovf_cap;
     v.ovf_ent = pb.d_ovf_ent + (size_t)c * pl.ovf_cap * kg::kGroup;
-    v.ulist = pb.d_ulist + (uint64_t)c * pb.ucap;
+    v.ulist = pb.d_ulist + (uint64_t)c * pb.ucap; v.ukeys = pb.d_ukeys + (uint64_t)c * pb.ucap;
     v.cused = pb.d_cused + c * pb.cused_stride; v.candused = pb.d_candused + c * pb.candused_stride;
     v.cand = pb.d_cand + (uint64_t)c * pb.ccap;
     v.ucur = (unsigned long long *)(pb.d_pc + kPcUcur + c); v.ccur = (unsigned long long *)(pb.d_pc + kPcCcur + c);
@@ -253,11 +256,11 @@
     dispatch<int, 1, 2, 0>(pl.part_counters ? 1 : pl.prog_index ? 2 : 0, [&](auto walks) {
         constexpr bool COUNTERS = decltype(walks)::value == 1, PROG = decltype(walks)::value == 2;
         hipLaunchKernelGGL((kg::verify_kernel<AA, COUNTERS, PROG>), dim3(pl.verify_grid), dim3(256), 0, s3, t->d_entries, t->d_tags, t->limit,
-                           (uint64_t)t->num_sigs, t->magic, v.cand, v.candused, v.ccur, pb.ccap, v.ulist, v.cused, v.ucur, pb.ucap, d_ctr,
+                           (uint64_t)t->num_sigs, t->magic, v.cand, v.candused, v.ccur, pb.ccap, v.ulist, v.ukeys, v.cused, v.ucur, pb.ucap, d_ctr,
                            d_prog, pl.verify_prio);
         hipLaunchKernelGGL((kg::overflow_probe_kernel<AA, COUNTERS, PROG>), dim3(pl.ovf_grid), dim3(256), 0, s3, t->d_entries, t->d_tags,
                            t->limit, (uint64_t)t->num_sigs, t->magic, v.ovf_bucket, v.ovf_ent, v.ovfc, pl.ovf_cap, pl.shift, v.ulist,
-                           v.cused, v.ucur, pb.ucap, d_ctr, d_prog);
+                           v.ukeys, v.cused, v.ucur, pb.ucap, d_ctr, d_prog);
     });
     HIP_TRY(hipEventRecord(t->pev[kPevVerified + v.c], s3));
     HIP_TRY(hipGetLastError());
@@ -281,7 +284,7 @@
     const uint64_t row_lo = (uint64_t)v.lo * PER, row_hi = row_lo + (uint64_t)v.nb * PER;
     const uint32_t g0 = (uint32_t)(row_lo >> gshift);
     const uint32_t n_groups = v.nb ? (uint32_t)(((row_hi - 1) >> gshift) - g0 + 1) : 1u;
-    hipLaunchKernelGGL(kg::hit_hist_kernel, dim3(pl.order_grid), dim3(kg::kHThreads), (size_t)n_groups * 4, s, v.ulist, v.cused, v.ucur, pb.ucap,
+    hipLaunchKernelGGL(kg::hit_hist_kernel, dim3(pl.order_grid), dim3(kg::kHThreads), (size_t)n_groups * 4, s, v.ukeys, v.cused, v.ucur, pb.ucap,
                        g0, 6u + gshift, n_groups, v.ghist);
     hipLaunchKernelGGL(kg::group_scan_kernel, dim3(1), dim3(kg::kGsThreads), 0, s, v.ghist, n_groups, v.gbase, v.gcur1, v.gcur2, v.ctot, v.gtile);
     if (pl.n_os && c) HIP_TRY(hipStreamWaitEvent(s, t->pev[kPevBase + c - 1], 0));
@@ -297,8 +300,9 @@
     hipLaunchKernelGGL((kg::hit_partition_kernel<false>), dim3(pl.order_grid), dim3(kg::kHThreads), 0, s, v.sortA, v.cused, v.ucur, pb.ucap,
                        v.gbase, n_groups, g0, 6u + gshift, v.gcur2, v.sortB, pb.ucap, v.gtile);
     hipLaunchKernelGGL((kg::group_place_kernel<AA>), dim3(std::min(n_groups, 256u * 8u)), dim3(kg::kHThreads),
-                       kg::group_place_lds(gshift, pl.place_staged), s,
-                       v.sortB, v.gbase, n_groups, g0, gshift, (uint32_t)row_lo, (uint32_t)row_hi, pb.d_geo, (uint64_t)cx.b.n_rows,
+                       kg::group_place_lds<AA>(gshift, pl.place_staged), s,
+                       v.sortB, v.gbase, n_groups, g0, gshift, (uint32_t)row_lo, (uint32_t)row_hi,
+                       reinterpret_cast<const kg::SeqRows *>(pb.d_owners), pb.d_owners + 3 * (size_t)pb.n_listed,
                        pl.place_staged ? 1u : 0u, v.base, res->d_hits, hits_cap, cx.d_offs, res->d_hit_slots);
     HIP_TRY(hipGetLastError());
     return KG_OK;
@@ -318,14 +322,13 @@
     if ((rc = sc.get(&pb.d_next, pl.next_stride * n_chunks))) return rc;
     if ((rc = sc.get(&pb.d_ovfc, kOvfWords * kMaxChunks))) return rc;
     if ((rc = sc.get(&pb.d_lowc, (size_t)cx.b.nblocks + 1))) return rc;
-    if ((rc = sc.get(&pb.d_geo, (size_t)cx.b.n_rows))) return rc;
     if ((rc = sc.get(&pb.d_ghist, (size_t)groups_stride * n_chunks))) return rc;
     if ((rc = sc.get(&pb.d_gbase, (size_t)(groups_stride + 1) * n_chunks))) return rc;
     if ((rc = sc.get(&pb.d_gcur1, (size_t)(kg::kHDigits + 1) * n_chunks))) return rc;
     if ((rc = sc.get(&pb.d_gcur2, (size_t)groups_stride * n_chunks))) return rc;
     if ((rc = sc.get(&pb.d_gtile, (size_t)(kg::kHDigits + 1) * n_chunks))) return rc;
-    if (kg::group_place_lds(pl.gshift, pl.gshift == 10) > t->place_lds[AA ? 1 : 0]) {
-        const size_t want_lds = kg::group_place_lds(pl.gshift, pl.gshift == 10);
+    if (kg::group_place_lds<AA>(pl.gshift, pl.gshift == 10) > t->place_lds[AA ? 1 : 0]) {
+        const size_t want_lds = kg::group_place_lds<AA>(pl.gshift, pl.gshift == 10);
         HIP_TRY(hipFuncSetAttribute((const void *)kg::group_place_kernel<AA>, hipFuncAttributeMaxDynamicSharedMemorySize, (int)want_lds));
         t->place_lds[AA ? 1 : 0] = want_lds;
     }
@@ -350,7 +353,6 @@
 template <bool AA>
 int scan_partitioned(ScanCtx &cx, const PartPlan &pl, bool &done)
 {
-    constexpr uint32_t PER = AA ? 1 : 6;
     kg_table *t = cx.t;
     kg_result *res = cx.res;
     kg_stats &st = res->st;
@@ -359,7 +361,11 @@
     int rc;
     PartBuffers pb;
     if ((rc = part_allocate<AA>(cx, pl, pb))) return rc;
-    BlockGuard<6> lists{cx.sc, {(void **)&pb.d_ulist, (void **)&pb.d_cused, (void **)&pb.d_cand, (void **)&pb.d_candused,
+    std::vector<uint32_t> owners;
+    pb.n_listed = plan_row_owners<AA>(cx.b, cx.offsets, cx.n_seqs, pl.gshift, owners);
+    if ((rc = cx.sc.get(&pb.d_owners, owners.size()))) return rc;
+    HIP_TRY(hipMemcpyAsync(pb.d_owners, owners.data(), owners.size() * 4, hipMemcpyHostToDevice, t->stream));
+    BlockGuard<7> lists{cx.sc, {(void **)&pb.d_ulist, (void **)&pb.d_ukeys, (void **)&pb.d_cused, (void **)&pb.d_cand, (void **)&pb.d_candused,
                                 (void **)&pb.d_sortA, (void **)&pb.d_sortB}};
     pb.ucap = pl.ucap; pb.ccap = pl.ccap;
     HIP_TRY(hipEventRecord(t->ev[kEvScanBegin], t->stream));
@@ -370,6 +376,7 @@
         if ((rc = dalloc(t, (void **)&res->d_hits, hits_cap * sizeof(kg_hit)))) return rc;
         if (cx.progress && (rc = dalloc(t, (void **)&res->d_hit_slots, hits_cap * 4))) return rc;
         if ((rc = dalloc(t, (void **)&pb.d_ulist, ucap * n_chunks * sizeof(kg_hit)))) return rc;
+        if ((rc = dalloc(t, (void **)&pb.d_ukeys, ucap * n_chunks * 4))) return rc;
         if ((rc = dalloc(t, (void **)&pb.d_cused, pb.cused_stride * n_chunks * 4))) return rc;
         if ((rc = dalloc(t, (void **)&pb.d_cand, ccap * n_chunks * sizeof(kg::CandRec)))) return rc;
         if ((rc = dalloc(t, (void **)&pb.d_candused, pb.candused_stride * n_chunks * 4))) return rc;
@@ -388,8 +395,6 @@
         HIP_TRY(hipEventRecord(t->pev[kPevFork], t->stream));
         HIP_TRY(hipStreamWaitEvent(t->stream2, t->pev[kPevFork], 0));
         HIP_TRY(hipStreamWaitEvent(t->stream3, t->pev[kPevFork], 0));
-        hipLaunchKernelGGL((kg::row_geo_kernel<AA>), dim3((uint32_t)((nblocks * PER + 255) / 256)), dim3(256), 0, t->stream3, cx.d_blocks,
-                           (uint32_t)nblocks, pb.d_geo);
         for (uint32_t c = 0; c < n_chunks; c++) {
             if (!cx.seq_uploaded && (rc = upload_seq(cx, cx.offsets[pl.cseq[c]], cx.offsets[pl.cseq[c + 1]]))) return rc;
             if ((rc = chunk_passes<AA>(cx, pl, pb, chunk_view(pl, pb, c)))) return rc;
diff --git a/kmergutsjava_amd/csrc/kg_order.hpp b/kmergutsjava_amd/csrc/kg_order.hpp
--- a/kmergutsjava_amd/csrc/kg_order.hpp
+++ b/kmergutsjava_amd/csrc/kg_order.hpp
@@ -11,24 +11,10 @@
 constexpr uint32_t kHDigits = 128;
 constexpr uint32_t kMaxGroups = kHDigits * kHDigits;
 
-struct RowGeo { uint32_t container; int32_t pos_first; };
-
-template <bool AA>
-__global__ void row_geo_kernel(const BlockDesc *__restrict__ blocks, uint32_t n_blocks, RowGeo *__restrict__ geo)
-{
-    constexpr uint32_t ROWS = AA ? 1 : 6;
-    const uint64_t tl = (uint64_t)blockIdx.x * blockDim.x + threadIdx.x;
-    if (tl >= (uint64_t)n_blocks * ROWS) return;
-    const uint32_t r = (uint32_t)(tl / n_blocks), it = (uint32_t)(tl % n_blocks);
-    const BlockDesc bd = blocks[it];
-    RowGeo g;
-    int32_t pos0;
-    row_record_key<AA>(bd, (int)r, 0, &g.container, &pos0);
-    g.pos_first = (!AA && r >= 3) ? pos0 - 63 : pos0;
-    geo[row_index<AA>(bd, it, (int)r)] = g;
-}
-
-__global__ __launch_bounds__(kHThreads) void hit_hist_kernel(const kg_hit *__restrict__ ulist, const uint32_t *__restrict__ chunk_used,
+constexpr uint32_t kHistPer = 4;
+constexpr uint32_t kHistLanes = kUChunk / kHistPer;
+static_assert(kUChunk % kHistPer == 0 && kHThreads % kHistLanes == 0, "a workgroup takes whole reservation chunks");
+__global__ __launch_bounds__(kHThreads) void hit_hist_kernel(const uint32_t *__restrict__ ukeys, const uint32_t *__restrict__ chunk_used,
                                                              const unsigned long long *__restrict__ cursor, uint64_t ulist_cap,
                                                              uint32_t g0, uint32_t gs , uint32_t n_groups,
                                                              uint32_t *ghist )
@@ -38,11 +24,17 @@
     __syncthreads();
     const unsigned long long cur = *cursor;
     const uint32_t n_chunks = (uint32_t)((cur < ulist_cap ? cur : ulist_cap) / kUChunk);
-    for (uint32_t c = blockIdx.x; c < n_chunks; c += gridDim.x) {
+    constexpr uint32_t kPerRound = kHThreads / kHistLanes;
+    const uint32_t sub = threadIdx.x / kHistLanes, k = (threadIdx.x % kHistLanes) * kHistPer;
+    for (uint32_t c = blockIdx.x * kPerRound + sub; c < n_chunks; c += gridDim.x * kPerRound) {
         const uint32_t used = chunk_used[c];
-        for (uint32_t k = threadIdx.x; k < used; k += kHThreads) {
-            const uint32_t g = (ulist[(uint64_t)c * kUChunk + k].container >> gs) - g0;
-            if (g < n_groups) atomicAdd(&h_lds[g], 1u);
+        if (k >= used) continue;
+        const kg_u32x4 v = __builtin_nontemporal_load(reinterpret_cast<const kg_u32x4 *>(ukeys + (uint64_t)c * kUChunk + k));
+        const uint32_t key[kHistPer] = {v.x, v.y, v.z, v.w};
+#pragma unroll
+        for (uint32_t i = 0; i < kHistPer; i++) {
+            const uint32_t g = (key[i] >> gs) - g0;
+            if (k + i < used && g < n_groups) atomicAdd(&h_lds[g], 1u);
         }
     }
     __syncthreads();
@@ -220,24 +212,33 @@
 }
 
 constexpr uint32_t kPlaceOut = 1536;
+template <bool AA>
+__host__ __device__ inline uint32_t group_place_seqs(uint32_t gshift)
+{
+    return (1u << gshift) / (AA ? 1u : 6u) + 2u;
+}
+template <bool AA>
 __host__ __device__ inline size_t group_place_lds(uint32_t gshift, bool staged)
 {
-    return staged ? ((size_t)20 << gshift) + (size_t)kPlaceOut * sizeof(kg_hit) : ((size_t)12 << gshift);
+    const size_t slice = ((size_t)group_place_seqs<AA>(gshift) * sizeof(SeqRows) + 7u) & ~(size_t)7u;
+    return ((size_t)12 << gshift) + slice + (staged ? (size_t)kPlaceOut * sizeof(kg_hit) : 0u);
 }
 template <bool AA>
 __global__ __launch_bounds__(kHThreads) void group_place_kernel(const kg_hit *__restrict__ in, const uint32_t *__restrict__ gbase, uint32_t n_groups,
                                                                 uint32_t g0, uint32_t gshift, uint32_t row_lo, uint32_t row_hi ,
-                                                                const RowGeo *__restrict__ geo, uint64_t n_rows_all, uint32_t staged,
+                                                                const SeqRows *__restrict__ seqs, const uint32_t *__restrict__ gseq, uint32_t staged,
                                                                 const uint64_t *__restrict__ base,
                                                                 kg_hit *__restrict__ hits, uint64_t hits_cap, uint32_t *__restrict__ offs,
                                                                 uint32_t *__restrict__ hit_slots )
 {
+    constexpr uint32_t PER = AA ? 1u : 6u;
     extern __shared__ __attribute__((aligned(16))) unsigned char p_lds[];
     const uint32_t R = 1u << gshift;
+    const uint32_t slice_cap = group_place_seqs<AA>(gshift);
     unsigned long long *masks = reinterpret_cast<unsigned long long *>(p_lds);
     uint32_t *pre = reinterpret_cast<uint32_t *>(masks + R);
-    RowGeo *lgeo = reinterpret_cast<RowGeo *>(pre + R);
-    uint64_t *lout = reinterpret_cast<uint64_t *>(lgeo + R);
+    uint32_t *lseq = pre + R;
+    uint64_t *lout = reinterpret_cast<uint64_t *>(p_lds + group_place_lds<AA>(gshift, false));
     __shared__ uint32_t wsum[kHThreads / 64];
     const uint32_t tid = threadIdx.x, lane = tid & 63u, wave = tid >> 6;
     const uint64_t chunk_base = *base;
@@ -246,9 +247,13 @@
         const uint32_t lo = gbase[g], n = gbase[g + 1] - lo;
         const uint64_t row0 = (uint64_t)(g0 + g) << gshift;
         const bool to_lds = staged && n <= kPlaceOut;
-        for (uint32_t i = tid; i < R; i += kHThreads) {
-            masks[i] = 0ull;
-            if (staged && n && row0 + i < n_rows_all) lgeo[i] = geo[row0 + i];
+        const uint32_t s_first = gseq[g0 + g];
+        const uint32_t n_slice = n ? min(gseq[g0 + g + 1] - s_first + 1u, slice_cap) : 0u;
+        for (uint32_t i = tid; i < R; i += kHThreads) masks[i] = 0ull;
+        {
+            const uint32_t *src = reinterpret_cast<const uint32_t *>(seqs + s_first);
+#pragma unroll 1
+            for (uint32_t i = tid; i < 3u * n_slice; i += kHThreads) lseq[i] = src[i];
         }
         __syncthreads();
         constexpr uint32_t kKeep = 4;
@@ -273,6 +278,7 @@
         uint32_t mine = 0;
         const uint32_t r_lo = tid * per;
         if (r_lo < R)
+#pragma unroll 1
             for (uint32_t i = 0; i < per; i++) mine += (uint32_t)__popcll(masks[r_lo + i]);
         uint32_t incl = mine;
         for (int off = 1; off < 64; off <<= 1) {
@@ -284,6 +290,7 @@
         uint32_t run = incl - mine;
         for (uint32_t w = 0; w < wave; w++) run += wsum[w];
         if (r_lo < R)
+#pragma unroll 1
             for (uint32_t i = 0; i < per; i++) {
                 pre[r_lo + i] = run;
                 const uint64_t row = row0 + r_lo + i;
@@ -293,12 +300,17 @@
         __syncthreads();
         auto place = [&](kg_hit h) {
             const uint32_t key = h.container, rl = (key >> 6) & (R - 1u), ol = key & 63u;
-            const RowGeo gr = staged ? lgeo[rl] : geo[key >> 6];
+            const uint32_t row = key >> 6;
+            const uint32_t si = row_owner<PER>(n_slice, row, [&](uint32_t i) { return lseq[3u * i + 1u]; });
+            const SeqRows sr{lseq[3u * si], lseq[3u * si + 1u], lseq[3u * si + 2u]};
+            uint32_t container;
+            int32_t pos_first;
+            row_geometry<AA>(sr, row, &container, &pos_first);
             const uint32_t rank = pre[rl] + (uint32_t)__popcll(masks[rl] & ((1ull << ol) - 1ull));
             if (hit_slots && chunk_base + lo + rank < hits_cap)
                 hit_slots[chunk_base + lo + rank] = (uint32_t)h.from0InProt;
-            h.container = gr.container;
-            h.from0InProt = gr.pos_first + (int32_t)ol;
+            h.container = container;
+            h.from0InProt = pos_first + (int32_t)ol;
             if (to_lds) {
                 uint64_t w3[3];
                 __builtin_memcpy(w3, &h, 24);
diff --git a/kmergutsjava_amd/csrc/kg_partition.hpp b/kmergutsjava_amd/csrc/kg_partition.hpp
--- a/kmergutsjava_amd/csrc/kg_partition.hpp
+++ b/kmergutsjava_amd/csrc/kg_partition.hpp
@@ -522,7 +522,7 @@
 
 template <bool AA, int N, bool COUNTERS>
 __device__ __forceinline__ void probe_entries(const TableView &tab, uint32_t b, uint32_t shift, const uint64_t (&e)[N],
-                                              kg_hit *__restrict__ ulist, uint32_t *__restrict__ chunk_used,
+                                              kg_hit *__restrict__ ulist, uint32_t *__restrict__ ukeys, uint32_t *__restrict__ chunk_used,
                                               unsigned long long *cursor, uint64_t ulist_cap, UListState &u,
                                               unsigned long long &ctr_slots, bool &ran_off, int lane, Progress *prog)
 {
@@ -572,7 +572,7 @@
                     h.container = id[k];
                     h.from0InProt = (int32_t)fslot[k];
                     h.oI = pay[k].oI; h.avgOffFromEnd = pay[k].avg; h.fI = pay[k].fI; h.functionWt = pay[k].wt;
-                    ulist[u.base + at + rank[k]] = h;
+                    ulist_append(ulist, ukeys, u.base + at + rank[k], h);
                 }
                 at += cnt[k];
             }
@@ -881,7 +881,7 @@
 __global__ __launch_bounds__(256) void verify_kernel(
     const uint8_t *__restrict__ entries, const uint8_t *__restrict__ tags, uint64_t limit, uint64_t num_sigs, uint64_t magic,
     const CandRec *__restrict__ cand, const uint32_t *__restrict__ cand_used, const unsigned long long *cand_cursor,
-    uint64_t cand_cap, kg_hit *__restrict__ ulist, uint32_t *__restrict__ chunk_used, unsigned long long *cursor,
+    uint64_t cand_cap, kg_hit *__restrict__ ulist, uint32_t *__restrict__ ukeys, uint32_t *__restrict__ chunk_used, unsigned long long *cursor,
     uint64_t ulist_cap, unsigned long long *ctr, Progress *prog ,
     uint32_t prio )
 {
@@ -983,7 +983,7 @@
                     h.container = r.id;
                     h.from0InProt = (int32_t)(uint32_t)s;
                     h.oI = e.oI; h.avgOffFromEnd = e.avg; h.fI = e.fI; h.functionWt = e.wt;
-                    stream_store_hit(ulist + at + (uint32_t)__popcll(m & ((1ull << lane) - 1ull)), h);
+                    ulist_append(ulist, ukeys, at + (uint32_t)__popcll(m & ((1ull << lane) - 1ull)), h);
                 }
             }
         }
@@ -1000,7 +1000,8 @@
 __global__ __launch_bounds__(256) void overflow_probe_kernel(
     const uint8_t *__restrict__ entries, const uint8_t *__restrict__ tags, uint64_t limit, uint64_t num_sigs, uint64_t magic,
     const uint32_t *__restrict__ ovf_bucket, const uint64_t *__restrict__ ovf_ent, const uint32_t *__restrict__ ovf_cursor,
-    uint32_t ovf_cap, uint32_t shift, kg_hit *__restrict__ ulist, uint32_t *__restrict__ chunk_used, unsigned long long *cursor, uint64_t ulist_cap,
+    uint32_t ovf_cap, uint32_t shift, kg_hit *__restrict__ ulist, uint32_t *__restrict__ ukeys, uint32_t *__restrict__ chunk_used,
+    unsigned long long *cursor, uint64_t ulist_cap,
     unsigned long long *ctr, Progress *prog)
 {
     const int lane = threadIdx.x & 63;
@@ -1017,7 +1018,7 @@
         const uint32_t b = ovf_bucket[g];
         uint64_t e[1];
         e[0] = lane < (int)kGroup ? ovf_ent[(uint64_t)g * kGroup + lane] : kEntInvalid;
-        probe_entries<AA, 1, COUNTERS || PROG>(tab, b, shift, e, ulist, chunk_used, cursor, ulist_cap, u, ctr_slots, ran_off, lane, prog);
+        probe_entries<AA, 1, COUNTERS || PROG>(tab, b, shift, e, ulist, ukeys, chunk_used, cursor, ulist_cap, u, ctr_slots, ran_off, lane, prog);
     }
     if (lane == 0 && u.have && u.base + kUChunk <= ulist_cap) chunk_used[u.base / kUChunk] = u.used;
     flush_ran_off(ran_off, ctr, lane);
diff --git a/kmergutsjava_amd/csrc/kg_rows.hpp b/kmergutsjava_amd/csrc/kg_rows.hpp
--- /dev/null
+++ b/kmergutsjava_amd/csrc/kg_rows.hpp
@@ -0,0 +1,133 @@
+#pragma once
+
+#include <stdint.h>
+
+#include <vector>
+
+#if defined(__HIPCC__)
+#define KG_HD __host__ __device__ __forceinline__
+#else
+#define KG_HD inline
+#endif
+
+namespace kg {
+
+constexpr int kRowDnaPos = 192;
+constexpr int kRowAaWin = 64;
+
+struct BlockDesc {
+    uint64_t soff;
+    uint32_t len;
+    uint32_t j;
+    uint32_t nk;
+    uint32_t ibase;
+    uint32_t seq;
+    uint32_t pad;
+};
+static_assert(sizeof(BlockDesc) == 32, "BlockDesc must be 32 bytes");
+
+template <bool AA>
+KG_HD uint32_t row_index(const BlockDesc &bd, uint32_t it, int r)
+{
+    if (AA) return it;
+    const uint32_t vbase = 6u * bd.ibase;
+    if (r < 3) return vbase + (uint32_t)r * bd.nk + bd.j;
+    return vbase + (3u + (bd.len - (uint32_t)(r - 3)) % 3u) * bd.nk + (bd.nk - 1u - bd.j);
+}
+
+template <bool AA>
+KG_HD void row_record_key(const BlockDesc &bd, int r, int lane, uint32_t *container, int32_t *pos)
+{
+    if (AA) {
+        *container = bd.seq;
+        *pos = (int32_t)(bd.j * kRowAaWin + lane);
+    } else if (r < 3) {
+        *container = bd.seq * 6u + (uint32_t)r;
+        *pos = (int32_t)(bd.j * 64u + lane);
+    } else {
+        const uint32_t f = (uint32_t)(r - 3);
+        *container = bd.seq * 6u + 3u + (bd.len - f) % 3u;
+        *pos = (int32_t)((bd.len - 24u - f - bd.j * kRowDnaPos) / 3u) - (int32_t)lane;
+    }
+}
+
+struct SeqRows { uint32_t seq, ibase, len; };
+
+template <bool AA>
+KG_HD uint32_t seq_blocks(uint32_t len)
+{
+    if (AA) return len >= 9u ? (len - 8u + (uint32_t)kRowAaWin - 1u) / (uint32_t)kRowAaWin : 0u;
+    return len >= 24u ? (uint32_t)(((uint64_t)len - 23u + (uint64_t)kRowDnaPos - 1u) / (uint64_t)kRowDnaPos) : 0u;
+}
+
+template <bool AA>
+KG_HD BlockDesc row_block(const SeqRows &s, uint32_t row, int *r_out)
+{
+    BlockDesc bd;
+    bd.soff = 0; bd.len = s.len; bd.ibase = s.ibase; bd.seq = s.seq; bd.pad = 0;
+    bd.nk = seq_blocks<AA>(s.len);
+    if (AA) {
+        bd.j = row - s.ibase;
+        *r_out = 0;
+        return bd;
+    }
+    const uint32_t rel = row - 6u * s.ibase;
+    uint32_t kind = 0, idx = rel;
+    for (int c = 0; c < 5; c++)
+        if (idx >= bd.nk) { idx -= bd.nk; kind++; }
+    if (kind < 3u) {
+        bd.j = idx;
+        *r_out = (int)kind;
+    } else {
+        bd.j = bd.nk - 1u - idx;
+        *r_out = 3 + (int)((s.len % 3u + 6u - kind) % 3u);
+    }
+    return bd;
+}
+
+template <bool AA>
+KG_HD void row_geometry(const SeqRows &s, uint32_t row, uint32_t *container, int32_t *pos_first)
+{
+    int r;
+    const BlockDesc bd = row_block<AA>(s, row, &r);
+    int32_t pos0;
+    row_record_key<AA>(bd, r, 0, container, &pos0);
+    *pos_first = (!AA && r >= 3) ? pos0 - 63 : pos0;
+}
+
+template <uint32_t PER, typename F>
+KG_HD uint32_t row_owner(uint32_t n, uint32_t row, F &&ibase)
+{
+    uint32_t lo = 0, hi = n;
+    while (hi - lo > 1u) {
+        const uint32_t mid = lo + (hi - lo) / 2u;
+        if (PER * ibase(mid) <= row) lo = mid; else hi = mid;
+    }
+    return lo;
+}
+
+template <bool AA>
+inline uint32_t row_owner_words(const uint32_t *ibase, const int64_t *offsets, int64_t n_seqs, uint32_t gshift, std::vector<uint32_t> &words)
+{
+    constexpr uint32_t PER = AA ? 1 : 6;
+    words.clear();
+    for (int64_t k = 0; k < n_seqs; k++)
+        if (ibase[k + 1] != ibase[k]) {
+            words.push_back((uint32_t)k);
+            words.push_back(ibase[k]);
+            words.push_back((uint32_t)(offsets[k + 1] - offsets[k]));
+        }
+    const uint32_t n_listed = (uint32_t)(words.size() / 3);
+    const uint64_t n_rows = (uint64_t)PER * ibase[n_seqs];
+    const uint64_t n_groups = n_rows ? ((n_rows - 1) >> gshift) + 1 : 0;
+    uint32_t k = 0;
+    for (uint64_t g = 0; g < n_groups; g++) {
+        const uint64_t row0 = g << gshift;
+        while (k + 1 < n_listed && (uint64_t)PER * words[3 * (size_t)(k + 1) + 1] <= row0) k++;
+        words.push_back(k);
+    }
+    words.push_back(n_listed ? n_listed - 1 : 0u);
+    return n_listed;
+}
+
+}
```

Result: no change. 130.4 billion residues/s (-0.7%).
